# ithakis/Option-Replicating-Portfolio-with-Neural-Networks

Measured on AMD Instinct MI355X. Metric: MC paths/sec training 30-step hedge-MLP + terminal P&L std-dev, 1/2/4/8 MI355X, higher is better.
Workload: dtype fp32

## Files before the change

### csrc/hedge_mlp.hip

```cpp
#include "hedge_core.h"
#include "hedge_fit.h"
#include "hedge_lag.h"
#include "hedge_narrow.h"

#include <type_traits>

namespace rph {

template <int NIN, int H, int NO, int HEAD>
__global__ __launch_bounds__(256) void k_hedge_train_step(const TrainDesc d, const int step, const int epoch,
                                                          const Perm perm) {
  using B = NarrowBody<NIN, H, NO, HEAD>;
  constexpr int R = B::R;
  constexpr int P = B::P;
  prefetch_kernarg<sizeof(TrainDesc) + 2 * sizeof(int) + sizeof(Perm)>();
  __shared__ __attribute__((aligned(16))) float lds[B::SCRATCH_FLOATS];
  __shared__ __attribute__((aligned(16))) float wl[P + 4];
  __shared__ int s_last;

  RPH_DASSERT(d.batch > 0 && d.n_local >= d.batch && d.num_wgs == (int)gridDim.x);
  RPH_STAMP(0);
  const float stopped = d.fit->stopped;
  const float wv = threadIdx.x < P ? d.wts->w[0][threadIdx.x] : 0.f;
  UpdPre<P> up;
  if (d.fused_update) prefetch_update<P>(up, d.wts, d.opt, d.fit, d.lr_sched, epoch, step);
  const int lane = threadIdx.x & 63, wid = threadIdx.x >> 6;
  typename B::Pre pre;
  pre.valid = false;
  if (B::first(wid) < d.batch) B::load(d, step, perm, B::first(wid), lane, pre);

  if (stopped != 0.f) return;
  if (threadIdx.x < P) wl[threadIdx.x] = wv;
  if (d.fused_update) {
    asm volatile("" ::"v"(up.m[0]), "v"(up.v[0]), "v"(up.w[0]), "v"(up.wbest[0]), "s"(up.t), "s"(up.lr), "s"(up.loss_sum),
                 "s"(up.wait), "s"(up.best_loss), "s"(up.lr_sched_e));
  }
  __syncthreads();
  RPH_STAMP(1);
  float vv[1];
  B::partial(d, step, perm, wl, typename B::Frags{}, lds, pre, vv);
  float val = vv[0];
  float* red = lds;
  RPH_STAMP(3);

  if (gridDim.x > 1) {
    const int G = gridDim.x;
    if (threadIdx.x < R) {
      if (d.deterministic) st_agent(d.slab + (size_t)blockIdx.x * R + threadIdx.x, val);
      else __hip_atomic_fetch_add(d.acc + (blockIdx.x % ACC_REPLICAS) * R + threadIdx.x, val, __ATOMIC_RELAXED,
                                  __HIP_MEMORY_SCOPE_AGENT);
    }
    asm volatile("s_waitcnt vmcnt(0)" ::: "memory");
    __syncthreads();
    RPH_STAMP(4);
    if (threadIdx.x == 0) {
      const uint32_t ticket = __hip_atomic_fetch_add(d.counter, 1u, __ATOMIC_RELAXED, __HIP_MEMORY_SCOPE_AGENT);
      s_last = (ticket == (uint32_t)G - 1u) ? 1 : 0;
    }
    __syncthreads();
    RPH_STAMP(5);
    if (!s_last) return;
    if (d.deterministic) {
      constexpr int GROUPS = 256 / R;
      const int col = threadIdx.x % R;
      const int grp = threadIdx.x / R;
      float a = 0.f;
#pragma unroll 8
      for (int r = grp; r < G; r += GROUPS) a += ld_agent(d.slab + (size_t)r * R + col);
      lds[grp * R + col] = a;
      __syncthreads();
      if (threadIdx.x < R) {
        float s2 = 0.f;
        for (int gi = 0; gi < GROUPS; ++gi) s2 += lds[gi * R + threadIdx.x];
        val = s2;
      }
      __syncthreads();
    } else {
      if (threadIdx.x < R) {
        float* a = d.acc + threadIdx.x;
        float r0, r1, r2, r3, r4, r5, r6, r7;
        if (R == 128) {
          asm volatile(
              "global_load_dword %0, %8, off sc1\n\t"
              "global_load_dword %1, %8, off offset:512 sc1\n\t"
              "global_load_dword %2, %8, off offset:1024 sc1\n\t"
              "global_load_dword %3, %8, off offset:1536 sc1\n\t"
              "global_load_dword %4, %8, off offset:2048 sc1\n\t"
              "global_load_dword %5, %8, off offset:2560 sc1\n\t"
              "global_load_dword %6, %8, off offset:3072 sc1\n\t"
              "global_load_dword %7, %8, off offset:3584 sc1\n\t"
              "s_waitcnt vmcnt(0)"
              : "=&v"(r0), "=&v"(r1), "=&v"(r2), "=&v"(r3), "=&v"(r4), "=&v"(r5), "=&v"(r6), "=&v"(r7)
              : "v"(a)
              : "memory");
        } else {
          float* b = a + 4 * R;
          asm volatile(
              "global_load_dword %0, %8, off sc1\n\t"
              "global_load_dword %1, %8, off offset:1024 sc1\n\t"
              "global_load_dword %2, %8, off offset:2048 sc1\n\t"
              "global_load_dword %3, %8, off offset:3072 sc1\n\t"
              "global_load_dword %4, %9, off sc1\n\t"
              "global_load_dword %5, %9, off offset:1024 sc1\n\t"
              "global_load_dword %6, %9, off offset:2048 sc1\n\t"
              "global_load_dword %7, %9, off offset:3072 sc1\n\t"
              "s_waitcnt vmcnt(0)"
              : "=&v"(r0), "=&v"(r1), "=&v"(r2), "=&v"(r3), "=&v"(r4), "=&v"(r5), "=&v"(r6), "=&v"(r7)
              : "v"(a), "v"(b)
              : "memory");
        }
        val = ((r0 + r1) + (r2 + r3)) + ((r4 + r5) + (r6 + r7));
#pragma unroll
        for (int rp = 0; rp < ACC_REPLICAS; ++rp) st_agent(a + rp * R, 0.f);
      }
    }
    if (threadIdx.x == 0) __hip_atomic_store(d.counter, 0u, __ATOMIC_RELAXED, __HIP_MEMORY_SCOPE_AGENT);
  }
  if (threadIdx.x < R) red[threadIdx.x] = val;
  __syncthreads();
  RPH_STAMP(6);

  if (d.dp_world > 1) {
    dp_allreduce<R>(d, red);
    RPH_STAMP(7);
  }
  if (d.fused_update) {
    apply_update<P>(red, up, d.wts, d.opt, d.fit, epoch, step, d.steps_per_epoch);
  } else if (threadIdx.x < R) {
    d.grad_out[threadIdx.x] = red[threadIdx.x];
  }
  if (d.dp_world <= 1) RPH_STAMP(7);
}

template <int NIN, int H, int NO, int HEAD, bool PA, bool EX = false>
__global__ __launch_bounds__(256) void k_hedge_eval(const EvalDesc d) {
  using S = NetShape<NIN, H, NO, HEAD>;
  constexpr int NHOLD = S::NHOLD;
  static_assert(!PA || NIN >= NHOLD - 1, "price alias needs a feature per traded asset");
  prefetch_kernarg<sizeof(EvalDesc)>();
  RPH_DASSERT(d.n_local > 0 && d.num_wgs == (int)gridDim.x && d.wa != nullptr && d.stats != nullptr);
  __shared__ double sst[4][EVAL_NSTAT];
  constexpr int WBOFF = (S::P + 3) / 4 * 4;
  __shared__ __attribute__((aligned(16))) float wl[WBOFF + S::P + 4];
  const bool has_b = d.wb != nullptr;
  for (int i = threadIdx.x; i < S::P; i += 256) {
    wl[i] = d.wa->w[0][i];
    if (has_b) wl[WBOFF + i] = d.wb->w[0][i];
  }
  __syncthreads();
  if (blockIdx.x == 0) {
    for (int i = threadIdx.x; i < S::P; i += 256) {
      if (d.snap_a) d.snap_a->w[0][i] = wl[i];
      if (d.snap_b) d.snap_b->w[0][i] = has_b ? wl[WBOFF + i] : wl[i];
    }
  }
  const float* __restrict__ WA = wl;
  const float* __restrict__ WB = has_b ? wl + WBOFF : wl;
  const int lane = threadIdx.x & 63, wid = threadIdx.x >> 6;

  constexpr int NS = 64;
  float st[NS];
#pragma unroll
  for (int i = 0; i < NS; ++i) st[i] = 0.f;
  float rmin = INFINITY, rmax = -INFINITY;

  struct In {
    float x[NIN], pt[NHOLD], pt1[NHOLD], tgt, gb;
    int p;
    bool valid;
  };
  constexpr int EPF = 4;
  const int stride = (int)gridDim.x * 256;
  const bool has1 = d.price_t1[0] != nullptr;
  auto load_in = [&](int p, In& in) {
    in.p = p;
    in.valid = p < d.n_local;
    const int pp = in.valid ? p : 0;
#pragma unroll
    for (int f = 0; f < NIN; ++f) in.x[f] = d.feat[f][pp];
#pragma unroll
    for (int k = 0; k < NHOLD - 1; ++k) {
      if constexpr (PA) in.pt[k] = in.x[PA ? k : 0];
      else in.pt[k] = d.price_t[k][pp];
      in.pt1[k] = has1 ? d.price_t1[k][pp] : 0.f;
    }
    in.tgt = (has1 && d.target) ? d.target[pp] : 0.f;
    in.gb = d.g_base ? d.g_base[pp] : 0.f;
  };
  In q[EPF];
  const int p_first = blockIdx.x * 256 + threadIdx.x;
#pragma unroll
  for (int i = 0; i < EPF; ++i) load_in(p_first + i * stride, q[i]);

  for (int p0 = blockIdx.x * 256; p0 < d.n_local; p0 += stride) {
    const In cur = q[0];
#pragma unroll
    for (int i = 0; i + 1 < EPF; ++i) q[i] = q[i + 1];
    if (p0 + EPF * stride < d.n_local) load_in(cur.p + EPF * stride, q[EPF - 1]);
    const int p = cur.p;
    const bool valid = cur.valid;
    uint32_t zo = 0;
    asm volatile("" : "+v"(zo));
    const float* __restrict__ WAi = (const float*)__builtin_assume_aligned(WA + (zo & ~3u), 16);
    const float* __restrict__ WBi = (const float*)__builtin_assume_aligned(WB + (zo & ~3u), 16);
    float z1[H], a1[H], z2[H], a2[H], hold[NHOLD], holdv[NHOLD], xn[NIN];
#pragma unroll
    for (int f = 0; f < NIN; ++f) xn[f] = (cur.x[f] - d.fmu[f]) * d.fisd[f];
    net_forward<NIN, H, NO, HEAD>(WAi, xn, d.alpha, z1, a1, z2, a2, hold);
#pragma unroll
    for (int k = 0; k < NHOLD; ++k) holdv[k] = hold[k];
    if (has_b) {
      net_forward<NIN, H, NO, HEAD>(WBi, xn, d.alpha, z1, a1, z2, a2, holdv);
#pragma unroll
      for (int k = 0; k < NHOLD; ++k) hold[k] = hold[k] + d.hold_c * (holdv[k] - hold[k]);
    }
    float V = 0.f;
#pragma unroll
    for (int k = 0; k < NHOLD - 1; ++k) V = fmaf(holdv[k], cur.pt[k], V);
    V = fmaf(holdv[NHOLD - 1], d.bond_t, V);
    if (d.g_base) V = cur.gb + d.blend_c * (V - cur.gb);
    [[maybe_unused]] float cont = V, xval = 0.f;
    [[maybe_unused]] bool exer = false;
    if constexpr (EX) {
      xval = d.ex_kind == EX_PUT ? fmaxf(d.ex_strike - cur.pt[0], 0.f) : fmaxf(cur.pt[0] - d.ex_strike, 0.f);
      exer = xval > 0.f && xval >= cont;
      V = exer ? xval : cont;
    }
    float res = 0.f, pred1 = 0.f;
    const float tgt = cur.tgt;
    if (has1) {
#pragma unroll
      for (int k = 0; k < NHOLD - 1; ++k) pred1 = fmaf(hold[k], cur.pt1[k], pred1);
      pred1 = fmaf(hold[NHOLD - 1], d.bond_t1, pred1);
      if (d.target) res = tgt - pred1;
    }
    if (valid) {
      if (d.v_out) d.v_out[p] = V;
#pragma unroll
      for (int k = 0; k < NHOLD; ++k)
        if (d.hold_out[k]) d.hold_out[k][p] = hold[k];
      if (d.resid_out) d.resid_out[p] = res;
      if (d.pred1_out) d.pred1_out[p] = pred1;
      st[ES_V] += V;
      st[ES_V2] += V * V;
      st[ES_RES] += res;
      st[ES_RES2] += res * res;
      st[ES_ABSRES] += fabsf(res);
      st[ES_APE] += d.target ? fabsf(res) * __frcp_rn(fmaxf(fabsf(tgt), 1e-7f)) : 0.f;
      st[ES_PRED1] += pred1;
      st[ES_COUNT] += 1.f;
      if constexpr (EX) {
        st[ES_EXER] += exer ? 1.f : 0.f;
        st[ES_EXVAL] += exer ? xval : 0.f;
        st[ES_CONT] += cont;
      }
#pragma unroll
      for (int k = 0; k < NHOLD; ++k) {
        st[ES_HOLD + k] += hold[k];
        st[ES_HOLD2 + k] += hold[k] * hold[k];
      }
      rmin = fminf(rmin, res);
      rmax = fmaxf(rmax, res);
    }
  }
  wave_reduce_scatter<NS>(st, lane);
#pragma unroll
  for (int o = 1; o < 64; o <<= 1) {
    rmin = fminf(rmin, __shfl_xor(rmin, o, 64));
    rmax = fmaxf(rmax, __shfl_xor(rmax, o, 64));
  }
  if (lane < EVAL_NSTAT) sst[wid][lane] = (double)st[0];
  if (lane == 0) {
    sst[wid][ES_RESMIN] = rmin;
    sst[wid][ES_RESMAX] = rmax;
  }
  __syncthreads();
  if (threadIdx.x < EVAL_NSTAT) {
    const int i = threadIdx.x;
    double v;
    if (i == ES_RESMIN) v = fmin(fmin(sst[0][i], sst[1][i]), fmin(sst[2][i], sst[3][i]));
    else if (i == ES_RESMAX) v = fmax(fmax(sst[0][i], sst[1][i]), fmax(sst[2][i], sst[3][i]));
    else v = sst[0][i] + sst[1][i] + sst[2][i] + sst[3][i];
    d.stats[(size_t)blockIdx.x * EVAL_NSTAT + i] = v;
  }
}

constexpr int PNL_PPT = 4;

template <int NIN, int H, int NO, int HEAD, bool EX = false>
__global__ __launch_bounds__(256) void k_hedge_pnl(const PnlDesc d) {
  using S = NetShape<NIN, H, NO, HEAD>;
  constexpr int NHOLD = S::NHOLD;
  constexpr int NA = NHOLD - 1;
  constexpr int WBOFF = (S::P + 3) / 4 * 4;
  prefetch_kernarg<sizeof(PnlDesc)>();
  RPH_DASSERT(d.n_local > 0 && d.num_wgs == (int)gridDim.x && d.snap != nullptr && d.stats != nullptr);
  __shared__ __attribute__((aligned(16))) float wl[WBOFF + S::P + 4];
  __shared__ double sred[4][EX ? 12 : 8];
  const int tid = threadIdx.x, lane = tid & 63, wid = tid >> 6;
  const long long base = (long long)blockIdx.x * 256 * PNL_PPT + tid;
  const bool has_b = d.has_b != 0;
  float wealth[PNL_PPT], s_cur[PNL_PPT][NA > 0 ? NA : 1];
  long long pidx[PNL_PPT];
#pragma unroll
  for (int j = 0; j < PNL_PPT; ++j) {
    const long long p = base + (long long)j * 256;
    const bool ok = p < d.n_local;
    pidx[j] = ok ? p : 0;
    wealth[j] = ok ? (d.w0 ? d.w0[p] : d.wealth0) : 0.f;
#pragma unroll
    for (int a = 0; a < NA; ++a) s_cur[j][a] = d.price[a][pidx[j]];
  }
  float xr[PNL_PPT][NIN], s_nxt[PNL_PPT][NA > 0 ? NA : 1];
  auto load_date = [&](int t) {
#pragma unroll
    for (int j = 0; j < PNL_PPT; ++j) {
#pragma unroll
      for (int f = 0; f < NIN; ++f) xr[j][f] = d.feat[f][(long long)t * d.feat_ts[f] + pidx[j]];
#pragma unroll
      for (int a = 0; a < NA; ++a) s_nxt[j][a] = d.price[a][(long long)(t + 1) * d.price_ts[a] + pidx[j]];
    }
  };
  [[maybe_unused]] int tau[PNL_PPT];
  [[maybe_unused]] float pnl_ex[PNL_PPT];
  [[maybe_unused]] double paid[PNL_PPT];
  if constexpr (EX) {
#pragma unroll
    for (int j = 0; j < PNL_PPT; ++j) {
      tau[j] = d.n_dates;
      pnl_ex[j] = 0.f;
      paid[j] = 0.0;
    }
  }
  if (d.n_dates > 0) load_date(0);
  for (int t = 0; t < d.n_dates; ++t) {
    float xc[PNL_PPT][NIN], sc_nxt[PNL_PPT][NA > 0 ? NA : 1];
#pragma unroll
    for (int j = 0; j < PNL_PPT; ++j) {
#pragma unroll
      for (int f = 0; f < NIN; ++f) xc[j][f] = xr[j][f];
#pragma unroll
      for (int a = 0; a < NA; ++a) sc_nxt[j][a] = s_nxt[j][a];
    }
    if (t + 1 < d.n_dates) load_date(t + 1);
    __syncthreads();
    const NetWeights* wt = d.snap + (size_t)t * 2;
    for (int i = tid; i < S::P; i += 256) {
      wl[i] = wt[0].w[0][i];
      if (has_b) wl[WBOFF + i] = wt[1].w[0][i];
    }
    float mu[NIN], isd[NIN];
#pragma unroll
    for (int f = 0; f < NIN; ++f) {
      mu[f] = d.fmu[t * MAXIN + f];
      isd[f] = d.fisd[t * MAXIN + f];
    }
    const float grow = (float)(d.bond[t + 1] / d.bond[t]);
    [[maybe_unused]] bool ex_date = false;
    [[maybe_unused]] float bond_t = 0.f, to_end = 0.f;
    [[maybe_unused]] double disc = 0.0;
    if constexpr (EX) {
      ex_date = t % d.ex_every == 0;
      bond_t = (float)d.bond[t];
      to_end = (float)(d.bond[d.n_dates] / d.bond[t]);
      disc = d.bond[0] / d.bond[t];
    }
    __syncthreads();
#pragma unroll
    for (int j = 0; j < PNL_PPT; ++j) {
      uint32_t zo = 0;
      asm volatile("" : "+v"(zo));
      const float* __restrict__ WA = (const float*)__builtin_assume_aligned(wl + (zo & ~3u), 16);
      const float* __restrict__ WB = (const float*)__builtin_assume_aligned(wl + WBOFF + (zo & ~3u), 16);
      float x[NIN];
#pragma unroll
      for (int f = 0; f < NIN; ++f) x[f] = (xc[j][f] - mu[f]) * isd[f];
      float z1[H], a1[H], z2[H], a2[H], hold[NHOLD], hb[NHOLD];
      net_forward<NIN, H, NO, HEAD>(WA, x, d.alpha, z1, a1, z2, a2, hold);
      if (has_b) {
        net_forward<NIN, H, NO, HEAD>(WB, x, d.alpha, z1, a1, z2, a2, hb);
#pragma unroll
        for (int k = 0; k < NHOLD; ++k) hold[k] = hold[k] + d.hold_c * (hb[k] - hold[k]);
      }
      if constexpr (EX) {
        if (ex_date && tau[j] == d.n_dates) {
          float c = 0.f;
#pragma unroll
          for (int a = 0; a < NA; ++a) c = fmaf(hold[a], s_cur[j][a], c);
          c = fmaf(hold[NHOLD - 1], bond_t, c);
          const float s0 = s_cur[j][0];
          const float xv = d.ex_kind == EX_PUT ? fmaxf(d.ex_strike - s0, 0.f) : fmaxf(s0 - d.ex_strike, 0.f);
          if (xv > 0.f && xv >= c) {
            tau[j] = t;
            pnl_ex[j] = (wealth[j] - xv) * to_end;
            paid[j] = (double)xv * disc;
            wealth[j] = wealth[j] * to_end;
          }
        }
      }
      float w = wealth[j] * grow;
#pragma unroll
      for (int a = 0; a < NA; ++a) {
        w = fmaf(hold[a], sc_nxt[j][a] - s_cur[j][a] * grow, w);
        s_cur[j][a] = sc_nxt[j][a];
      }
      if constexpr (EX) wealth[j] = tau[j] == d.n_dates ? w : wealth[j];
      else wealth[j] = w;
    }
  }
  double sv = 0, sv2 = 0, sp = 0, sp2 = 0, sa = 0, cnt = 0;
  float pmin = INFINITY, pmax = -INFINITY;
  [[maybe_unused]] double sx = 0, sxv = 0, stau = 0;
#pragma unroll
  for (int j = 0; j < PNL_PPT; ++j) {
    const long long p = base + (long long)j * 256;
    if (p >= d.n_local) continue;
    float pnl = wealth[j] - d.payoff[p];
    if constexpr (EX) {
      const bool exd = tau[j] < d.n_dates;
      if (exd) pnl = pnl_ex[j];
      if (d.tau_out) d.tau_out[p] = tau[j];
      sx += exd ? 1.0 : 0.0;
      sxv += exd ? paid[j] : (double)d.payoff[p] * (d.bond[0] / d.bond[d.n_dates]);
      stau += (double)tau[j];
    }
    if (d.pnl_out) d.pnl_out[p] = pnl;
    sv += wealth[j];
    sv2 += (double)wealth[j] * wealth[j];
    sp += pnl;
    sp2 += (double)pnl * pnl;
    sa += fabsf(pnl);
    cnt += 1.0;
    pmin = fminf(pmin, pnl);
    pmax = fmaxf(pmax, pnl);
  }
#pragma unroll
  for (int o = 1; o < 64; o <<= 1) {
    sv += __shfl_xor(sv, o, 64);
    sv2 += __shfl_xor(sv2, o, 64);
    sp += __shfl_xor(sp, o, 64);
    sp2 += __shfl_xor(sp2, o, 64);
    sa += __shfl_xor(sa, o, 64);
    cnt += __shfl_xor(cnt, o, 64);
    pmin = fminf(pmin, __shfl_xor(pmin, o, 64));
    pmax = fmaxf(pmax, __shfl_xor(pmax, o, 64));
    if constexpr (EX) {
      sx += __shfl_xor(sx, o, 64);
      sxv += __shfl_xor(sxv, o, 64);
      stau += __shfl_xor(stau, o, 64);
    }
  }
  if constexpr (EX) {
    if (lane == 0) {
      sred[wid][8] = sx; sred[wid][9] = sxv; sred[wid][10] = stau;
    }
  }
  if (lane == 0) {
    sred[wid][0] = sv; sred[wid][1] = sv2; sred[wid][2] = sp; sred[wid][3] = sp2;
    sred[wid][4] = sa; sred[wid][5] = cnt; sred[wid][6] = pmin; sred[wid][7] = pmax;
  }
  __syncthreads();
  if (tid < EVAL_NSTAT) {
    double v = 0.0;
    auto sum4 = [&](int k) { return (sred[0][k] + sred[1][k]) + (sred[2][k] + sred[3][k]); };
    if (tid == ES_V) v = sum4(0);
    else if (tid == ES_V2) v = sum4(1);
    else if (tid == ES_RES) v = sum4(2);
    else if (tid == ES_RES2) v = sum4(3);
    else if (tid == ES_ABSRES) v = sum4(4);
    else if (tid == ES_COUNT) v = sum4(5);
    else if (tid == ES_RESMIN) v = fmin(fmin(sred[0][6], sred[1][6]), fmin(sred[2][6], sred[3][6]));
    else if (tid == ES_RESMAX) v = fmax(fmax(sred[0][7], sred[1][7]), fmax(sred[2][7], sred[3][7]));
    if constexpr (EX) {
      if (tid == ES_EXER) v = sum4(8);
      else if (tid == ES_EXVAL) v = sum4(9);
      else if (tid == ES_TAU) v = sum4(10);
    }
    d.stats[(size_t)blockIdx.x * EVAL_NSTAT + tid] = v;
  }
}

}

using namespace rph;

extern "C" int rph_net_nparams(int nin, int h, int nout, int head, int* p_out, int* r_out) {
  int rc = -1;
  match_shape(AllShapes{}, nin, h, nout, head, &rc, [&](auto t) {
    using S = typename decltype(t)::S;
    *p_out = S::P;
    *r_out = S::R;
    return 0;
  });
  return rc;
}

static Perm step_perm(const TrainDesc* d, int epoch) {
  const uint32_t n_chunks = (uint32_t)((d->n_local + (1 << d->chunk_log2) - 1) >> d->chunk_log2);
  return make_perm(n_chunks, d->seed, (uint32_t)epoch, d->shuffle != 0);
}

extern "C" int rph_train_step(const TrainDesc* d, int step, int epoch, void* stream) {
  if (int rc = validate_train(d, 0, "rph_train_step")) return rc;
  hipStream_t s = (hipStream_t)stream;
  const Perm perm = step_perm(d, epoch);
  int rc = 0;
  if (match_shape(NarrowShapes{}, d->nin, d->h, d->nout, d->head, &rc, [&](auto t) {
        using T = decltype(t);
        hipLaunchKernelGGL((k_hedge_train_step<T::NIN, T::H, T::NO, T::HEAD>), dim3(d->num_wgs), dim3(256), 0, s, *d,
                           step, epoch, perm);
        return (int)hipGetLastError();
      }))
    return rc;
  return launch_wide_step(d, step, epoch, perm, s);
}

extern "C" int rph_train_fit(const TrainDesc* d, int epochs, void* stream) {
  if (int rc = validate_train(d, 2, "rph_train_fit")) return rc;
  hipStream_t s = (hipStream_t)stream;
  int rc = 0;
  if (match_shape(NarrowShapes{}, d->nin, d->h, d->nout, d->head, &rc, [&](auto t) {
        using T = decltype(t);
        return launch_fit<NarrowBody<T::NIN, T::H, T::NO, T::HEAD>>(d, epochs, s);
      }))
    return rc;
  return launch_wide_fit(d, epochs, s);
}

extern "C" int rph_train_lag_step(const TrainDesc* d, int k, int epoch, void* stream) {
  if (int rc = validate_train(d, 1, "rph_train_lag_step")) return rc;
  hipStream_t s = (hipStream_t)stream;
  const Perm perm = step_perm(d, epoch);
  int rc = 0;
  if (match_shape(NarrowShapes{}, d->nin, d->h, d->nout, d->head, &rc, [&](auto t) {
        constexpr int A = decltype(t)::NIN, B = decltype(t)::H, C = decltype(t)::NO, E = decltype(t)::HEAD;
        switch (d->variant) {
          case 1: return launch_step_lag<NarrowBody<A, B, C, E, 2>>(d, k, epoch, perm, s);
          case 2: return launch_step_lag<NarrowBody<A, B, C, E, 1, 3>>(d, k, epoch, perm, s);
          case 3: return launch_step_lag<NarrowBody<A, B, C, E, 2, 3>>(d, k, epoch, perm, s);
          case 4: return launch_step_lag<NarrowBody<A, B, C, E, 1, 1, true>>(d, k, epoch, perm, s);
          case 5: return launch_step_lag<NarrowBody<A, B, C, E, 1, 1, false, true>>(d, k, epoch, perm, s);
          default: return launch_step_lag<NarrowBody<A, B, C, E>>(d, k, epoch, perm, s);
        }
      }))
    return rc;
  return launch_wide_lag_step(d, k, epoch, perm, s);
}

extern "C" int rph_train_lag_finalize(const TrainDesc* d, int K, void* stream) {
  if (int rc = validate_train(d, 1, "rph_train_lag_finalize")) return rc;
  hipStream_t s = (hipStream_t)stream;
  return with_shape(AllShapes{}, d->nin, d->h, d->nout, d->head, "rph_train_lag_finalize", [&](auto t) {
    using T = decltype(t);
    constexpr int NREP = T::H == 8 ? NARROW_NREP : WIDE_NREP;
    hipLaunchKernelGGL((k_hedge_lag_finalize<T::S::P, T::S::R, NREP>), dim3(1), dim3(256), 0, s, *d, K);
    return (int)hipGetLastError();
  });
}

extern "C" int rph_train_lag_fit(const TrainDesc* d, int epochs, void* stream) {
  if (int rc = validate_train(d, 1, "rph_train_lag_fit")) return rc;
  int k = 0;
  for (int e = 0; e < epochs; ++e)
    for (int s = 0; s < d->steps_per_epoch; ++s, ++k)
      if (int rc = rph_train_lag_step(d, k, e, stream)) return rc;
  return rph_train_lag_finalize(d, k, stream);
}

extern "C" int rph_train_ticket_fit(const TrainDesc* d, int epochs, void* stream) {
  if (int rc = validate_train(d, 0, "rph_train_ticket_fit")) return rc;
  if (!d->fused_update) return rph_report("rph_train_ticket_fit", "needs the fused (in-kernel) update");
  for (int e = 0; e < epochs; ++e)
    for (int s = 0; s < d->steps_per_epoch; ++s)
      if (int rc = rph_train_step(d, s, e, stream)) return rc;
  return 0;
}


extern "C" int rph_train_update(const TrainDesc* d, int step, int epoch, void* stream) {
  if (!d->grad_out || !d->wts || !d->opt || !d->fit) return rph_report("rph_train_update", "null pointer");
  hipStream_t s = (hipStream_t)stream;
  return with_shape(AllShapes{}, d->nin, d->h, d->nout, d->head, "rph_train_update", [&](auto t) {
    using S = typename decltype(t)::S;
    hipLaunchKernelGGL((k_hedge_update<S::P, S::R>), dim3(1), dim3(256), 0, s, *d, step, epoch);
    return (int)hipGetLastError();
  });
}

extern "C" int rph_eval(const EvalDesc* d, void* stream) {
  if (!d->wa || !d->stats || d->n_local < 1 || d->num_wgs < 1 || d->nin < 1 || d->nin > MAXIN)
    return rph_report("rph_eval", "bad eval descriptor");
  if (!(d->alpha >= 0.f && d->alpha <= 1.f)) return rph_report("rph_eval", "LeakyReLU slope must be in [0, 1]");
  for (int f = 0; f < d->nin; ++f)
    if (!(d->fisd[f] > 0.f && d->fisd[f] < 3.0e38f && d->fmu[f] == d->fmu[f]))
      return rph_report("rph_eval", "feature standardisation must be finite with fisd > 0");
  for (int f = 0; f < d->nin; ++f)
    if (!d->feat[f]) return rph_report("rph_eval", "null feature pointer");
  hipStream_t s = (hipStream_t)stream;
  const int nhold = d->head == HEAD_COMPLEMENT ? 2 : d->nout;
  bool alias = d->nin >= nhold - 1;
  for (int k = 0; alias && k < nhold - 1; ++k) alias = d->price_t[k] == d->feat[k];
  const bool ex = d->ex_kind != EX_NONE;
  if (ex) {
    if (d->ex_kind != EX_PUT && d->ex_kind != EX_CALL) return rph_report("rph_eval", "ex_kind must be 0, 1 (put) or 2 (call)");
    if (d->wb) return rph_report("rph_eval", "wb with ex_kind (early exercise takes one network)");
    if (d->g_base) return rph_report("rph_eval", "g_base with ex_kind (early exercise takes one network)");
    if (nhold < 2 || !d->price_t[0]) return rph_report("rph_eval", "price_t[0] is null with ex_kind");
    if (!(d->ex_strike == d->ex_strike) || d->ex_strike < 0.f || d->ex_strike > 3.0e38f)
      return rph_report("rph_eval", "ex_strike must be finite and >= 0");
  }
  return with_shape(AllShapes{}, d->nin, d->h, d->nout, d->head, "rph_eval", [&](auto t) {
    using T = decltype(t);
    auto launch = [&](auto pa, auto exv) {
      hipLaunchKernelGGL((k_hedge_eval<T::NIN, T::H, T::NO, T::HEAD, decltype(pa)::value, decltype(exv)::value>),
                         dim3(d->num_wgs), dim3(256), 0, s, *d);
      return (int)hipGetLastError();
    };
    if constexpr (T::NIN >= T::S::NHOLD - 1) {
      if (alias) return ex ? launch(std::true_type{}, std::true_type{}) : launch(std::true_type{}, std::false_type{});
    }
    return ex ? launch(std::false_type{}, std::true_type{}) : launch(std::false_type{}, std::false_type{});
  });
}

extern "C" int rph_pnl(const PnlDesc* d, void* stream) {
  const int nhold = d->head == HEAD_COMPLEMENT ? 2 : d->nout;
  if (!d->snap || !d->stats || !d->payoff || !d->fmu || !d->fisd || !d->bond || d->n_local < 1 || d->n_dates < 1 ||
      d->nin < 1 || d->nin > MAXIN || nhold < 2 || nhold > MAXHOLD)
    return rph_report("rph_pnl", "bad P&L descriptor");
  if (!(d->alpha >= 0.f && d->alpha <= 1.f)) return rph_report("rph_pnl", "LeakyReLU slope must be in [0, 1]");
  for (int f = 0; f < d->nin; ++f)
    if (!d->feat[f] || d->feat_ts[f] < 0) return rph_report("rph_pnl", "null feature pointer / negative stride");
  for (int k = 0; k < nhold - 1; ++k)
    if (!d->price[k] || d->price_ts[k] < d->n_local) return rph_report("rph_pnl", "null price pointer / bad stride");
  const long long per_wg = 256LL * PNL_PPT;
  if ((long long)d->num_wgs * per_wg < d->n_local || (long long)(d->num_wgs - 1) * per_wg >= d->n_local)
    return rph_report("rph_pnl", "num_wgs does not match n_local / (256 * PNL_PPT)");
  const bool ex = d->ex_kind != EX_NONE;
  if (ex) {
    if (d->ex_kind != EX_PUT && d->ex_kind != EX_CALL) return rph_report("rph_pnl", "ex_kind must be 0, 1 (put) or 2 (call)");
    if (d->has_b) return rph_report("rph_pnl", "has_b with ex_kind (early exercise takes one network)");
    if (d->ex_every < 1) return rph_report("rph_pnl", "ex_every must be >= 1 with ex_kind");
    if (!(d->ex_strike == d->ex_strike) || d->ex_strike < 0.f || d->ex_strike > 3.0e38f)
      return rph_report("rph_pnl", "ex_strike must be finite and >= 0");
  } else if (d->tau_out) {
    return rph_report("rph_pnl", "tau_out without ex_kind");
  }
  hipStream_t s = (hipStream_t)stream;
  return with_shape(AllShapes{}, d->nin, d->h, d->nout, d->head, "rph_pnl", [&](auto t) {
    using T = decltype(t);
    if (ex) hipLaunchKernelGGL((k_hedge_pnl<T::NIN, T::H, T::NO, T::HEAD, true>), dim3(d->num_wgs), dim3(256), 0, s, *d);
    else hipLaunchKernelGGL((k_hedge_pnl<T::NIN, T::H, T::NO, T::HEAD, false>), dim3(d->num_wgs), dim3(256), 0, s, *d);
    return (int)hipGetLastError();
  });
}
```

### csrc/paths.hip

```cpp
#include "rph_common.h"
#include "rph_types.h"

namespace rph {
int rph_report(const char* what, const char* msg);
}

namespace rph {

template <typename Real>
RPH_INLINE Real ndtri_u30(uint32_t x);
template <>
RPH_INLINE float ndtri_u30<float>(uint32_t x) {
  x = x == 0u ? 1u : x;
  return ndtri_u30_f32(x);
}
template <>
RPH_INLINE double ndtri_u30<double>(uint32_t x) {
  return ndtri_u30_f64(x);
}

template <typename Real, bool ALIGNED>
__global__ __launch_bounds__(256) void k_sobol_normal(Real* __restrict__ out, int n, int d,
                                                      const uint32_t* __restrict__ sv,
                                                      const uint32_t* __restrict__ shift,
                                                      long long offset, int raw) {
  const int i = blockIdx.x * 256 + threadIdx.x;
  if (ALIGNED == false && i >= n) return;
  const uint32_t g = gray_code((uint64_t)(offset + i));
  for (int j = 0; j < d; ++j) {
    const uint32_t x = sobol_point<ALIGNED>(sv + (size_t)j * 32, shift[j], g);
    Real v;
    if (raw) v = (Real)x * (Real)9.313225746154785e-10;
    else v = ndtri_u30<Real>(x);
    if (i < n) out[(size_t)i * d + j] = v;
  }
}

RPH_INLINE long long sim_gidx(const SimDesc& d, int p) {
  return d.map_blk > 0 ? d.path_offset + ((long long)p / d.map_blk) * d.map_stride + (long long)p % d.map_blk
                       : d.path_offset + p;
}

template <typename Real, bool ALIGNED, int MODEL, int STAT = 0>
__global__ __launch_bounds__(256) void k_sim_scan(const SimDesc d) {
  const int p = blockIdx.x * 256 + threadIdx.x;
  if (!ALIGNED && p >= d.n_local) return;
  const long long gp = sim_gidx(d, p);
  const uint32_t g = gray_code((uint64_t)gp);
  const Real dt = (Real)d.dt;
  const Real sdt = sqrt(dt);
  const Real mu = (Real)d.mu[0], sig = (Real)d.sigma[0];
  const float inv0 = (float)d.inv_norm[0];
  const size_t n = (size_t)d.n_local;

  if (MODEL == SIM_GBM_ARITH || MODEL == SIM_GBM_LOG) {
    Real y = (MODEL == SIM_GBM_LOG) ? log((Real)d.s0[0]) : (Real)d.s0[0];
    const Real drift = (MODEL == SIM_GBM_LOG) ? (mu - (Real)0.5 * sig * sig) * dt : mu * dt;
    const Real vol = sig * sdt;
    d.out[p] = (float)d.s0[0] * inv0;
    Real acc = (STAT == STAT_MEAN || STAT == STAT_GEOMEAN) ? (Real)0 : (Real)d.s0[0];
    Real stat = (Real)d.s0[0];
    Real sf = (Real)d.s0[0];
    if (STAT != STAT_NONE) d.out2[p] = (float)d.s0[0] * inv0;
    for (int t = 1; t < d.n_fine; ++t) {
      const Real z = ndtri_u30<Real>(sobol_point<ALIGNED>(d.sv1 + (size_t)t * 32, d.shift1[t], g));
      if (MODEL == SIM_GBM_LOG) y += drift + vol * z;
      else y = y + y * (drift + vol * z);
      if (STAT == STAT_GEOMEAN) {
        acc += y;
      } else if (STAT != STAT_NONE) {
        sf = (MODEL == SIM_GBM_LOG) ? exp(y) : y;
        if (STAT == STAT_MEAN) acc += sf;
        else if (STAT == STAT_MAX) acc = sf > acc ? sf : acc;
        else acc = sf < acc ? sf : acc;
      }
      if (t % d.reduction == 0 || (STAT != STAT_NONE && t == d.n_fine - 1)) {
        if (STAT == STAT_MEAN) stat = acc / (Real)t;
        else if (STAT == STAT_GEOMEAN) stat = exp(acc / (Real)t);
        else if (STAT != STAT_NONE) stat = acc;
      }
      if (t % d.reduction == 0) {
        const int c = t / d.reduction;
        const Real s = (STAT != STAT_NONE && STAT != STAT_GEOMEAN) ? sf : ((MODEL == SIM_GBM_LOG) ? exp(y) : y);
        if (c < d.n_coarse) {
          d.out[(size_t)c * n + p] = (float)s * inv0;
          if (STAT != STAT_NONE) d.out2[(size_t)c * n + p] = (float)stat * inv0;
        }
      }
    }
    const Real s = (STAT != STAT_NONE && STAT != STAT_GEOMEAN) ? sf : ((MODEL == SIM_GBM_LOG) ? exp(y) : y);
    if (d.final_out) d.final_out[p] = (float)s * inv0;
    if (STAT != STAT_NONE && d.final2_out) d.final2_out[p] = (float)stat * inv0;
  } else if (MODEL == SIM_SV_REF || MODEL == SIM_HESTON) {
    Real ly = log((Real)d.s0[0]);
    Real v = (Real)d.v0;
    d.out[p] = (float)d.s0[0] * inv0;
    if (d.out2) d.out2[p] = (float)v;
    const Real rho = (Real)d.rho, rhoc = sqrt((Real)1 - rho * rho);
    const Real kap = (Real)d.kappa, th = (Real)d.theta, xi = (Real)d.xi;
    const Real ekd = exp(-kap * dt);
    const Real qc1 = xi * xi * ekd * ((Real)1 - ekd) / kap;
    const Real qc2 = th * xi * xi * ((Real)1 - ekd) * ((Real)1 - ekd) / ((Real)2 * kap);
    const Real qK1 = (Real)0.5 * dt * (kap * rho / xi - (Real)0.5) - rho / xi;
    const Real qK2 = (Real)0.5 * dt * (kap * rho / xi - (Real)0.5) + rho / xi;
    const Real qK3 = (Real)0.5 * dt * ((Real)1 - rho * rho);
    const Real qA = qK2 + (Real)0.5 * qK3;
    const Real qK0u = -rho * kap * th * dt / xi;
    const bool qe = MODEL == SIM_HESTON && d.scheme == HESTON_QE;
    const Real tau = (Real)d.sv_tscale * dt;
    for (int t = 1; t < d.n_fine; ++t) {
      const Real z1 = ndtri_u30<Real>(sobol_point<ALIGNED>(d.sv1 + (size_t)t * 32, d.shift1[t], g));
      const uint32_t x2 = sobol_point<ALIGNED>(d.sv2 + (size_t)t * 32, d.shift2[t], g);
      if (MODEL == SIM_SV_REF) {
        const Real z2 = ndtri_u30<Real>(x2);
        if (d.sv_tscale > 0.0) {
          const Real vp = v > (Real)0 ? v : (Real)0;
          ly += (mu - (Real)0.5 * vp * vp) * dt + vp * sdt * z1;
          v = v + (Real)d.a * ((Real)d.b - vp) * tau + (Real)d.c * sqrt(vp * tau) * z2;
        } else {
          const Real arg = v * dt;
          const Real sq = d.parity ? sqrt(arg) : sqrt(arg > (Real)0 ? arg : (Real)0);
          v = v + (Real)d.a * ((Real)d.b - v) + (Real)d.c * sq * z2;
          ly += (mu - (Real)0.5 * v * v) * dt + v * sdt * z1;
        }
      } else if (qe) {
        const Real m = th + (v - th) * ekd;
        const Real s2 = v * qc1 + qc2;
        const Real psi = s2 / (m * m);
        Real vn, k0;
        if (psi <= (Real)1.5) {
          const Real z2 = ndtri_u30<Real>(x2);
          const Real ip = (Real)2 / psi;
          const Real b2 = ip - (Real)1 + sqrt(ip) * sqrt(ip - (Real)1);
          const Real qa = m / ((Real)1 + b2);
          const Real bz = sqrt(b2) + z2;
          vn = qa * bz * bz;
          const Real den = (Real)1 - (Real)2 * qA * qa;
          k0 = den > (Real)0 ? -qA * b2 * qa / den + (Real)0.5 * log(den) - (qK1 + (Real)0.5 * qK3) * v : qK0u;
        } else {
          const Real p = (psi - (Real)1) / (psi + (Real)1);
          const Real beta = ((Real)1 - p) / m;
          const Real u = (Real)x2 * (Real)9.313225746154785e-10;
          vn = u <= p ? (Real)0 : log(((Real)1 - p) / ((Real)1 - u)) / beta;
          k0 = beta > qA ? -log(p + beta * ((Real)1 - p) / (beta - qA)) - (qK1 + (Real)0.5 * qK3) * v : qK0u;
        }
        const Real var = qK3 * (v + vn);
        ly += mu * dt + k0 + qK1 * v + qK2 * vn + sqrt(var > (Real)0 ? var : (Real)0) * z1;
        v = vn;
      } else {
        const Real z2 = ndtri_u30<Real>(x2);
        const Real vp = v > (Real)0 ? v : (Real)0;
        const Real sv = sqrt(vp * dt);
        ly += (mu - (Real)0.5 * vp) * dt + sv * (rho * z2 + rhoc * z1);
        v = v + (Real)d.kappa * ((Real)d.theta - vp) * dt + (Real)d.xi * sv * z2;
      }
      if (t % d.reduction == 0) {
        const int c = t / d.reduction;
        if (c < d.n_coarse) {
          d.out[(size_t)c * n + p] = (float)exp(ly) * inv0;
          if (d.out2) d.out2[(size_t)c * n + p] = (float)v;
        }
      }
    }
    if (d.final_out) d.final_out[p] = (float)exp(ly) * inv0;
  } else if (MODEL == SIM_MORTALITY) {
    Real lam = (Real)d.l0;
    int N = d.n0;
    const float invn = 1.0f / (float)d.n0;
    d.out2[p] = 1.0f;
    if (d.out3) d.out3[p] = (float)lam;
    const Real lc = (Real)d.lc, eta_sdt = (Real)d.eta * sdt;
    for (int t = 1; t < d.n_fine; ++t) {
      const Real z = ndtri_u30<Real>(sobol_point<ALIGNED>(d.sv2 + (size_t)t * 32, d.shift2[t], g));
      lam = lam + (lc * lam * dt + eta_sdt * z);
      double q = 1.0 - exp(-(double)lam * (double)dt);
      q = q < 0.0 ? 0.0 : (q > 1.0 ? 1.0 : q);
      if (N > 0 && q > 0.0) {
        const u32x4 r = philox4x32_10({(uint32_t)gp, (uint32_t)(gp >> 32),
                                       (uint32_t)t, 0xB1A0u},
                                      d.seed, 0x1234u);
        const double u = u01d(r.x, r.y);
        const double mean = (double)N * q;
        int D;
        if (mean < 200.0 && q < 1.0) {
          double f = exp((double)N * log1p(-q));
          double F = f;
          const double ratio = q / (1.0 - q);
          D = 0;
          while (u > F && D < N) {
            f *= (double)(N - D) / (double)(D + 1) * ratio;
            ++D;
            F += f;
            if (f < 1e-300 && F < u) { break; }
          }
        } else {
          const double z2n = ndtri_u30<double>((uint32_t)(u * 1073741824.0) | 1u);
          double dd = mean + sqrt(mean * (1.0 - q)) * z2n + 0.5;
          dd = dd < 0.0 ? 0.0 : (dd > (double)N ? (double)N : dd);
          D = (int)dd;
        }
        N -= D;
      }
      if (d.parity) {
        if (t < d.n_coarse && d.out3) d.out3[(size_t)t * n + p] = (float)lam;
      }
      if (t % d.reduction == 0) {
        const int c = t / d.reduction;
        if (c < d.n_coarse) {
          d.out2[(size_t)c * n + p] = (float)N * invn;
          if (!d.parity && d.out3) d.out3[(size_t)c * n + p] = (float)lam;
        }
      }
    }
    if (d.final2_out) d.final2_out[p] = (float)N * invn;
  }
}

template <int NA, bool ALIGNED>
__global__ __launch_bounds__(256) void k_sim_basket(const SimDesc d) {
  const int p = blockIdx.x * 256 + threadIdx.x;
  if (!ALIGNED && p >= d.n_local) return;
  const uint32_t g = gray_code((uint64_t)sim_gidx(d, p));
  const float dt = (float)d.dt, sdt = sqrtf(dt);
  float ly[NA], drift[NA], vol[NA], inv[NA], ch[NA * (NA + 1) / 2];
  const size_t n = (size_t)d.n_local;
#pragma unroll
  for (int a = 0, i = 0; a < NA; ++a)
#pragma unroll
    for (int b = 0; b <= a; ++b, ++i) ch[i] = (float)d.chol[a * MAXIN + b];
#pragma unroll
  for (int a = 0; a < NA; ++a) {
    ly[a] = logf((float)d.s0[a]);
    drift[a] = (float)((d.mu[a] - 0.5 * d.sigma[a] * d.sigma[a]) * d.dt);
    vol[a] = (float)d.sigma[a] * sdt;
    inv[a] = (float)d.inv_norm[a];
    d.out[(size_t)a * n + p] = (float)d.s0[a] * inv[a];
  }
  for (int t = 1; t < d.n_fine; ++t) {
    float w[NA];
#pragma unroll
    for (int a = 0; a < NA; ++a) {
      const int dim = a * d.n_fine + t;
      w[a] = ndtri_u30<float>(sobol_point<ALIGNED>(d.sv1 + (size_t)dim * 32, d.shift1[dim], g));
    }
#pragma unroll
    for (int a = 0; a < NA; ++a) {
      float z = 0.f;
#pragma unroll
      for (int b = 0; b <= a; ++b) z = fmaf(ch[a * (a + 1) / 2 + b], w[b], z);
      ly[a] += drift[a] + vol[a] * z;
    }
    if (t % d.reduction == 0) {
      const int c = t / d.reduction;
      if (c < d.n_coarse) {
#pragma unroll
        for (int a = 0; a < NA; ++a) d.out[((size_t)c * NA + a) * n + p] = __expf(ly[a]) * inv[a];
      }
    }
  }
  if (d.final_out) {
#pragma unroll
    for (int a = 0; a < NA; ++a) d.final_out[(size_t)a * n + p] = __expf(ly[a]) * inv[a];
  }
}

__global__ __launch_bounds__(256) void k_payoff(int kind, int n, int na, const float* __restrict__ s,
                                                const float* __restrict__ nfrac, float strike,
                                                const float* __restrict__ wts, const float* __restrict__ x,
                                                float* __restrict__ out) {
  const int p = blockIdx.x * 256 + threadIdx.x;
  if (p >= n) return;
  float v;
  if (kind == 0) {
    const float y = s[p];
    v = (y > strike ? y : strike) * (nfrac ? nfrac[p] : 1.f);
  } else if (kind == 1) {
    v = fmaxf(s[p] - strike, 0.f);
  } else if (kind == 2) {
    v = fmaxf(strike - s[p], 0.f);
  } else if (kind == 4) {
    v = fmaxf(s[p] - x[p], 0.f);
  } else if (kind == 5) {
    v = fmaxf(x[p] - s[p], 0.f);
  } else {
    float b = 0.f;
    for (int a = 0; a < na; ++a) b = fmaf(wts[a], s[(size_t)a * n + p], b);
    v = fmaxf(b - strike, 0.f);
  }
  out[p] = v;
}

RPH_INLINE uint32_t fkey(float x) {
  const uint32_t b = __float_as_uint(x);
  return (b & 0x80000000u) ? ~b : (b | 0x80000000u);
}

__global__ __launch_bounds__(256) void k_radix_hist(const float* __restrict__ x, long long n, uint32_t pmask,
                                                    uint32_t prefix, int shift, int nbins,
                                                    unsigned int* __restrict__ hist) {
  extern __shared__ __attribute__((aligned(16))) unsigned int h[];
  for (int i = threadIdx.x; i < nbins; i += 256) h[i] = 0u;
  __syncthreads();
  for (long long i = (long long)blockIdx.x * 256 + threadIdx.x; i < n; i += (long long)gridDim.x * 256) {
    const uint32_t k = fkey(x[i]);
    if ((k & pmask) == prefix) atomicAdd(&h[(k >> shift) & (uint32_t)(nbins - 1)], 1u);
  }
  __syncthreads();
  for (int i = threadIdx.x; i < nbins; i += 256)
    if (h[i]) atomicAdd(&hist[i], h[i]);
}

}

using namespace rph;

static inline int grid_for(int n) { return (n + 255) / 256; }

extern "C" int rph_sobol_normal(void* out, int n, int d, const uint32_t* sv, const uint32_t* shift,
                                long long offset, int fp64, int raw, void* stream) {
  hipStream_t s = (hipStream_t)stream;
  const bool aligned = (n % 256 == 0) && (offset % 64 == 0);
  if (fp64) {
    if (aligned) hipLaunchKernelGGL((k_sobol_normal<double, true>), dim3(grid_for(n)), dim3(256), 0, s, (double*)out, n, d, sv, shift, offset, raw);
    else hipLaunchKernelGGL((k_sobol_normal<double, false>), dim3(grid_for(n)), dim3(256), 0, s, (double*)out, n, d, sv, shift, offset, raw);
  } else {
    if (aligned) hipLaunchKernelGGL((k_sobol_normal<float, true>), dim3(grid_for(n)), dim3(256), 0, s, (float*)out, n, d, sv, shift, offset, raw);
    else hipLaunchKernelGGL((k_sobol_normal<float, false>), dim3(grid_for(n)), dim3(256), 0, s, (float*)out, n, d, sv, shift, offset, raw);
  }
  return (int)hipGetLastError();
}

template <typename Real, bool AL, int MODEL>
static int launch_scan_stat(const SimDesc* d, hipStream_t s) {
  const dim3 grid(grid_for(d->n_local)), block(256);
  switch (d->path_stat) {
    case STAT_MEAN: hipLaunchKernelGGL((k_sim_scan<Real, AL, MODEL, STAT_MEAN>), grid, block, 0, s, *d); break;
    case STAT_GEOMEAN: hipLaunchKernelGGL((k_sim_scan<Real, AL, SIM_GBM_LOG, STAT_GEOMEAN>), grid, block, 0, s, *d); break;
    case STAT_MAX: hipLaunchKernelGGL((k_sim_scan<Real, AL, MODEL, STAT_MAX>), grid, block, 0, s, *d); break;
    case STAT_MIN: hipLaunchKernelGGL((k_sim_scan<Real, AL, MODEL, STAT_MIN>), grid, block, 0, s, *d); break;
    default: return -1;
  }
  return (int)hipGetLastError();
}

template <typename Real, bool AL>
static int launch_scan(const SimDesc* d, hipStream_t s) {
  const dim3 grid(grid_for(d->n_local)), block(256);
  if (d->path_stat != STAT_NONE)
    return d->model == SIM_GBM_LOG ? launch_scan_stat<Real, AL, SIM_GBM_LOG>(d, s)
                                   : launch_scan_stat<Real, AL, SIM_GBM_ARITH>(d, s);
  switch (d->model) {
    case SIM_GBM_ARITH: hipLaunchKernelGGL((k_sim_scan<Real, AL, SIM_GBM_ARITH>), grid, block, 0, s, *d); break;
    case SIM_GBM_LOG: hipLaunchKernelGGL((k_sim_scan<Real, AL, SIM_GBM_LOG>), grid, block, 0, s, *d); break;
    case SIM_SV_REF: hipLaunchKernelGGL((k_sim_scan<Real, AL, SIM_SV_REF>), grid, block, 0, s, *d); break;
    case SIM_HESTON: hipLaunchKernelGGL((k_sim_scan<Real, AL, SIM_HESTON>), grid, block, 0, s, *d); break;
    case SIM_MORTALITY: hipLaunchKernelGGL((k_sim_scan<Real, AL, SIM_MORTALITY>), grid, block, 0, s, *d); break;
    default: return -1;
  }
  return (int)hipGetLastError();
}

template <bool AL>
static int launch_basket(const SimDesc* d, hipStream_t s) {
  const dim3 grid(grid_for(d->n_local)), block(256);
  switch (d->na) {
    case 1: hipLaunchKernelGGL((k_sim_basket<1, AL>), grid, block, 0, s, *d); break;
    case 2: hipLaunchKernelGGL((k_sim_basket<2, AL>), grid, block, 0, s, *d); break;
    case 3: hipLaunchKernelGGL((k_sim_basket<3, AL>), grid, block, 0, s, *d); break;
    case 4: hipLaunchKernelGGL((k_sim_basket<4, AL>), grid, block, 0, s, *d); break;
    case 5: hipLaunchKernelGGL((k_sim_basket<5, AL>), grid, block, 0, s, *d); break;
    case 6: hipLaunchKernelGGL((k_sim_basket<6, AL>), grid, block, 0, s, *d); break;
    default: return -1;
  }
  return (int)hipGetLastError();
}

extern "C" int rph_simulate(const SimDesc* d, void* stream) {
  hipStream_t s = (hipStream_t)stream;
  if (d->map_blk < 0 || (d->map_blk > 0 && d->map_stride < d->map_blk)) return rph_report("rph_simulate", "bad path-index map");
  if (d->path_stat < STAT_NONE || d->path_stat > STAT_MIN) return rph_report("rph_simulate", "path_stat outside 0..4");
  if (d->path_stat != STAT_NONE) {
    if (d->model != SIM_GBM_ARITH && d->model != SIM_GBM_LOG)
      return rph_report("rph_simulate", "path statistics need a GBM model");
    if (!d->out2) return rph_report("rph_simulate", "path statistic without an out2 buffer");
    if (d->path_stat == STAT_GEOMEAN && d->model != SIM_GBM_LOG)
      return rph_report("rph_simulate", "geomean needs the log scheme (SIM_GBM_LOG)");
  }
  const bool aligned = (d->n_local % 256 == 0) && (d->path_offset % 64 == 0) &&
                       (d->map_blk == 0 || (d->map_blk % 64 == 0 && d->map_stride % 64 == 0));
  if (d->model == SIM_BASKET) return aligned ? launch_basket<true>(d, s) : launch_basket<false>(d, s);
  if (d->fp64) return aligned ? launch_scan<double, true>(d, s) : launch_scan<double, false>(d, s);
  return aligned ? launch_scan<float, true>(d, s) : launch_scan<float, false>(d, s);
}

extern "C" int rph_payoff(int kind, int n, int na, const float* s, const float* nfrac, float strike,
                          const float* wts, const float* x, float* out, void* stream) {
  if ((kind == 4 || kind == 5) && !x) return rph_report("rph_payoff", "floating-strike payoff without the x array");
  hipLaunchKernelGGL(k_payoff, dim3(grid_for(n)), dim3(256), 0, (hipStream_t)stream, kind, n, na, s, nfrac,
                     strike, wts, x, out);
  return (int)hipGetLastError();
}

extern "C" int rph_radix_hist(const float* x, long long n, uint32_t pmask, uint32_t prefix, int shift,
                              int nbins, unsigned int* hist, void* stream) {
  long long blocks = (n + 255) / 256;
  if (blocks > 2048) blocks = 2048;
  if (blocks < 1) blocks = 1;
  hipLaunchKernelGGL(k_radix_hist, dim3((unsigned)blocks), dim3(256), nbins * sizeof(unsigned int),
                     (hipStream_t)stream, x, n, pmask, prefix, shift, nbins, hist);
  return (int)hipGetLastError();
}
```

### csrc/rph_types.h

```cpp
#pragma once
#include <stdint.h>

namespace rph {

constexpr int PMAX = 2048;
constexpr int MAXIN = 8;
constexpr int MAXHOLD = 8;
constexpr int MAXHIST = 1024;
constexpr int EVAL_NSTAT = 32;
constexpr int LAG_SLOTS = 16;

enum Head : int { HEAD_FREE = 0, HEAD_COMPLEMENT = 1 };
enum Loss : int { LOSS_MSE = 0, LOSS_PINBALL = 1 };

struct NetWeights {
  float w[2][PMAX];
  float cur;
  float pad[3];
};

struct OptState {
  float m[PMAX];
  float v[PMAX];
  float t;
  float lr;
  float beta1, beta2, eps;
  float nan_steps;
  float pad0, pad1;
};

struct FitState {
  float w_best[PMAX];
  float best_loss;
  float wait;
  float stopped;
  float epoch;
  float patience;
  float max_epochs;
  float restore_best;
  float has_best;
  float loss_sum, loss_cnt, abs_sum, ape_sum;
  float last_loss, last_mae, last_mape;
  float restore_at_end;
  float hist[MAXHIST];
};

constexpr int NETW_FLOATS = (int)(sizeof(NetWeights) / 4);
constexpr int OPT_FLOATS = (int)(sizeof(OptState) / 4);
constexpr int FIT_FLOATS = (int)(sizeof(FitState) / 4);

struct TrainDesc {
  const float* feat[MAXIN];
  const float* price[MAXHOLD];
  const float* target;
  NetWeights* wts;
  OptState* opt;
  FitState* fit;
  const float* lr_sched;
  float* slab;
  uint32_t* counter;
  float* grad_out;
  float bond;
  float alpha;
  float quantile;
  float inv_batch;
  int loss;
  int n_local;
  int batch;
  int steps_per_epoch;
  int chunk_log2;
  int shuffle;
  uint32_t seed;
  int fused_update;
  int num_wgs;
  int nin, h, nout, head;
  float* acc;
  int deterministic;
  unsigned long long* stamps;
  int dp_world;
  int dp_rank;
  float* dp_mbox[8];
  uint32_t* dp_flags[8];
  uint32_t* dp_counter;
  uint32_t* dp_error;
  int mfma_fp32;
  float* lag;
  int variant;
  const FitState* fit_init;
  float fmu[MAXIN];
  float fisd[MAXIN];
};

constexpr int DP_SLOTS = 4;

struct EvalDesc {
  const float* feat[MAXIN];
  const float* price_t[MAXHOLD];
  const float* price_t1[MAXHOLD];
  const float* target;
  const NetWeights* wa;
  const NetWeights* wb;
  const float* g_base;
  float* v_out;
  float* hold_out[MAXHOLD];
  float* resid_out;
  float* pred1_out;
  double* stats;
  float bond_t, bond_t1;
  float alpha;
  float blend_c;
  float hold_c;
  int n_local;
  int num_wgs;
  int nin, h, nout, head;
  float fmu[MAXIN];
  float fisd[MAXIN];
  NetWeights* snap_a;
  NetWeights* snap_b;
  int ex_kind;
  float ex_strike;
};

struct PnlDesc {
  const float* feat[MAXIN];
  long long feat_ts[MAXIN];
  const float* price[MAXHOLD];
  long long price_ts[MAXHOLD];
  const NetWeights* snap;
  const float* fmu;
  const float* fisd;
  const double* bond;
  const float* w0;
  const float* payoff;
  float* pnl_out;
  double* stats;
  float alpha, hold_c, wealth0;
  int has_b;
  int n_local, n_dates, num_wgs;
  int nin, h, nout, head;
  int ex_kind;
  int ex_every;
  float ex_strike;
  int* tau_out;
};

constexpr int LM_NPMAX = 192;
constexpr int LM_TILE = 64;
constexpr int LM_GBLK_MAX = 21 * 1024;
constexpr int LM_OUTG = 64 * 65 / 2;
constexpr int LM_OUTG_TAIL = 1;
constexpr int LM_RED_OUTG = LM_GBLK_MAX + LM_NPMAX + 8;
constexpr int LM_RED = LM_RED_OUTG + LM_OUTG;
constexpr int LM_PASS_WGS_MAX = 512;
constexpr int LM_OG_MAX = 64;
constexpr int LM_SPEC = 4;
enum LmState : int {
  LMS_W = 0,
  LMS_RED = 2 * LM_NPMAX,
  LMS_BEST = LMS_RED + 2 * LM_RED,
  LMS_LAM,
  LMS_NACC,
  LMS_FAIL,
  LMS_LFIN,
  LMS_FAILTOT,
  LMS_SPEC_LAM = LMS_FAIL + 8,
  LMS_SPEC_PRED = LMS_SPEC_LAM + LM_SPEC,
  LMS_SPEC_OK = LMS_SPEC_PRED + LM_SPEC,
  LMS_SPEC_W = LMS_SPEC_OK + LM_SPEC,
  LMS_SLOTS = LMS_SPEC_W + LM_SPEC * LM_NPMAX,
  LMS_FLOATS = LMS_SLOTS + 16
};
constexpr int LM_SLOT = 8;
enum LmSlot : int {
  LSS_BEST = 0,
  LSS_LAM,
  LSS_NU,
  LSS_PRED,
  LSS_COPY,
  LSS_SPEC_IDX,
  LSS_LBEST,
  LSS_STOP,
};

constexpr int LM_DP_WGS = 16;
constexpr int LM_DP_FLAGS = 128;
constexpr int LM_DP_PITCH = LM_RED + LM_DP_FLAGS;
struct LmDpDesc {
  double* mbox[8];
  unsigned* counter;
  unsigned* error;
  int world, rank;
  int pitch;
  int fault;
};

struct LmDesc {
  double* state;
  float* slab_b;
  float* slab_g;
  int num_wgs;
  int gram_wgs;
  int red_wgs;
  int passes;
  int gram_blk;
  int gram_blk_stride;
  float inv_ns;
  float inv_n;
  float lam0, lam_up, lam_down, lam_min, lam_max, ridge;
  int bias_index;
  int weights_only;
  int damping;
  int stop_min;
  float stop_tol;
  int gram_skip;
  int inst;
  int explore;
  float lam_carry;
  float diag_floor;
  const float* w0;
  int renorm;
  int pad1;
  float ren_mu[MAXIN];
  float ren_isd[MAXIN];
  int out_n;
  float out_mu;
  int out_gram;
  float out_tr;
  float* slab_o;
  const float* gfeat[MAXIN];
  const float* gprice[MAXIN];
  int gram_side;
  float q_delta;
  float q_kappa;
  LmDpDesc dp;
  int dp_fused;
  int leaf_blocks;
  const float* gtarget;
  int gram_base;
  int pad4;
};

constexpr int LM_SEL_W = LM_NPMAX + 2;
constexpr int LM_SEL_MAX = 64;


enum EvalStat : int {
  ES_V = 0, ES_V2 = 1, ES_RES = 2, ES_RES2 = 3, ES_ABSRES = 4, ES_APE = 5, ES_PRED1 = 6,
  ES_COUNT = 7, ES_HOLD = 8 , ES_HOLD2 = 16 , ES_RESMIN = 24,
  ES_RESMAX = 25,
  ES_EXER = 26, ES_EXVAL = 27, ES_CONT = 28, ES_TAU = 29
};

enum ExKind : int { EX_NONE = 0, EX_PUT = 1, EX_CALL = 2 };

struct SimDesc {
  int model;
  int n_local;
  long long path_offset;
  int n_fine;
  int reduction;
  int n_coarse;
  int na;
  int fp64;
  int parity;
  const uint32_t* sv1; const uint32_t* shift1; int dims1;
  const uint32_t* sv2; const uint32_t* shift2; int dims2;
  double s0[MAXIN], mu[MAXIN], sigma[MAXIN];
  double chol[MAXIN * MAXIN];
  double dt;
  double inv_norm[MAXIN];
  double v0, a, b, c, kappa, theta, xi, rho;
  double l0, lc, eta; int n0; uint32_t seed;
  float* out;
// ... 32 lines not shown
```

### csrc/runtime.cpp

```cpp
#include <hip/hip_runtime.h>
#include <rccl/rccl.h>
#include <stddef.h>
#include <stdio.h>
#include <string.h>

#include "rph_types.h"

using namespace rph;

static thread_local char g_err[512];

static int set_err(const char* what, int code, const char* msg) {
  snprintf(g_err, sizeof(g_err), "%s failed (%d): %s", what, code, msg ? msg : "");
  return code == 0 ? -1 : code;
}

#define HIP_TRY(expr)                                                              \
  do {                                                                             \
    hipError_t _e = (expr);                                                        \
    if (_e != hipSuccess) return set_err(#expr, (int)_e, hipGetErrorString(_e));   \
  } while (0)

#define NCCL_TRY(expr)                                                             \
  do {                                                                             \
    ncclResult_t _r = (expr);                                                      \
    if (_r != ncclSuccess) return set_err(#expr, (int)_r, ncclGetErrorString(_r)); \
  } while (0)

extern "C" const char* rph_last_error() { return g_err; }

namespace rph {
int rph_report(const char* what, const char* msg) { return set_err(what, -22, msg); }
int rph_report_shape(const char* what, int nin, int h, int nout, int head) {
  char msg[128];
  snprintf(msg, sizeof(msg), "unsupported network shape (nin %d, h %d, nout %d, head %d)", nin, h, nout, head);
  return rph_report(what, msg);
}
}

#define OFF(T, f) (long long)offsetof(T, f)
extern "C" int rph_layout(long long* out, int cap) {
  long long v[] = {
      (long long)sizeof(NetWeights), (long long)sizeof(OptState), (long long)sizeof(FitState),
      OFF(NetWeights, cur), OFF(OptState, t), OFF(OptState, lr), OFF(OptState, nan_steps),
      OFF(FitState, best_loss), OFF(FitState, stopped), OFF(FitState, epoch), OFF(FitState, last_loss),
      OFF(FitState, restore_at_end), OFF(FitState, hist),
      (long long)sizeof(TrainDesc), OFF(TrainDesc, price), OFF(TrainDesc, target), OFF(TrainDesc, wts),
      OFF(TrainDesc, lr_sched), OFF(TrainDesc, slab), OFF(TrainDesc, counter), OFF(TrainDesc, grad_out),
      OFF(TrainDesc, bond), OFF(TrainDesc, inv_batch), OFF(TrainDesc, loss), OFF(TrainDesc, seed),
      OFF(TrainDesc, num_wgs), OFF(TrainDesc, head), OFF(TrainDesc, acc), OFF(TrainDesc, deterministic), OFF(TrainDesc, stamps),
      OFF(TrainDesc, dp_world), OFF(TrainDesc, dp_mbox), OFF(TrainDesc, dp_flags), OFF(TrainDesc, dp_counter), OFF(TrainDesc, dp_error),
      OFF(TrainDesc, fit_init), OFF(TrainDesc, fmu), OFF(TrainDesc, fisd),
      (long long)sizeof(EvalDesc), OFF(EvalDesc, price_t), OFF(EvalDesc, price_t1), OFF(EvalDesc, target),
      OFF(EvalDesc, wa), OFF(EvalDesc, g_base), OFF(EvalDesc, v_out), OFF(EvalDesc, hold_out),
      OFF(EvalDesc, resid_out), OFF(EvalDesc, pred1_out), OFF(EvalDesc, stats), OFF(EvalDesc, bond_t),
      OFF(EvalDesc, hold_c), OFF(EvalDesc, n_local), OFF(EvalDesc, head), OFF(EvalDesc, fmu), OFF(EvalDesc, fisd),
      OFF(EvalDesc, snap_a), OFF(EvalDesc, snap_b), OFF(EvalDesc, ex_kind), OFF(EvalDesc, ex_strike),
      (long long)sizeof(PnlDesc), OFF(PnlDesc, feat_ts), OFF(PnlDesc, price), OFF(PnlDesc, price_ts),
      OFF(PnlDesc, snap), OFF(PnlDesc, bond), OFF(PnlDesc, pnl_out), OFF(PnlDesc, stats), OFF(PnlDesc, alpha),
      OFF(PnlDesc, has_b), OFF(PnlDesc, n_dates), OFF(PnlDesc, head),
      OFF(PnlDesc, ex_kind), OFF(PnlDesc, ex_every), OFF(PnlDesc, ex_strike), OFF(PnlDesc, tau_out),
      (long long)ES_EXER, (long long)ES_EXVAL, (long long)ES_CONT, (long long)ES_TAU, (long long)EVAL_NSTAT,
      (long long)sizeof(LmDesc), OFF(LmDesc, slab_b), OFF(LmDesc, slab_g), OFF(LmDesc, num_wgs),
      OFF(LmDesc, passes), OFF(LmDesc, gram_blk), OFF(LmDesc, inv_ns), OFF(LmDesc, lam0), OFF(LmDesc, ridge), OFF(LmDesc, bias_index), OFF(LmDesc, weights_only), OFF(LmDesc, damping), OFF(LmDesc, stop_tol), OFF(LmDesc, gram_skip),
      OFF(LmDesc, inst), OFF(LmDesc, lam_carry), OFF(LmDesc, w0), OFF(LmDesc, renorm), OFF(LmDesc, ren_isd), OFF(LmDesc, out_n), OFF(LmDesc, gfeat), OFF(LmDesc, gprice), OFF(LmDesc, gram_side), OFF(LmDesc, q_delta), OFF(LmDesc, dp), OFF(LmDesc, dp_fused), OFF(LmDesc, gtarget), OFF(LmDesc, gram_base), (long long)sizeof(LmDesc), (long long)LMS_LFIN, (long long)LMS_FAILTOT, (long long)LM_SEL_W, (long long)LM_DP_PITCH,
      (long long)sizeof(LmDpDesc), OFF(LmDpDesc, counter), OFF(LmDpDesc, world), OFF(LmDpDesc, pitch),
      (long long)LM_NPMAX, (long long)LM_RED, (long long)LMS_BEST, (long long)LMS_FLOATS,
      (long long)LM_SPEC, (long long)LMS_SPEC_W, (long long)LMS_SLOTS, (long long)LM_SLOT, (long long)LSS_LBEST, (long long)LSS_STOP,
      (long long)sizeof(SimDesc), OFF(SimDesc, path_offset), OFF(SimDesc, sv1), OFF(SimDesc, dims1),
      OFF(SimDesc, sv2), OFF(SimDesc, dims2), OFF(SimDesc, s0), OFF(SimDesc, chol), OFF(SimDesc, dt),
      OFF(SimDesc, inv_norm), OFF(SimDesc, v0), OFF(SimDesc, rho), OFF(SimDesc, l0), OFF(SimDesc, n0),
      OFF(SimDesc, seed), OFF(SimDesc, out), OFF(SimDesc, final2_out), OFF(SimDesc, sv_tscale),
      OFF(SimDesc, scheme), OFF(SimDesc, path_stat), OFF(SimDesc, map_blk), OFF(SimDesc, map_stride),
      (long long)LAG_SLOTS,
  };
  const int n = (int)(sizeof(v) / sizeof(v[0]));
  for (int i = 0; i < n && i < cap; ++i) out[i] = v[i];
  return n;
}

extern "C" int rph_device_info(int dev, int* cus, int* lds_per_cu, long long* hbm_bytes, char* name, int name_cap) {
  hipDeviceProp_t p;
  HIP_TRY(hipGetDeviceProperties(&p, dev));
  *cus = p.multiProcessorCount;
  *lds_per_cu = (int)p.maxSharedMemoryPerMultiProcessor;
  *hbm_bytes = (long long)p.totalGlobalMem;
  snprintf(name, name_cap, "%s", p.gcnArchName);
  return 0;
}

extern "C" int rph_memset_async(void* ptr, int value, long long bytes, void* stream) {
  HIP_TRY(hipMemsetAsync(ptr, value, (size_t)bytes, (hipStream_t)stream));
  return 0;
}

extern "C" int rph_stream_sync(void* stream) {
  HIP_TRY(hipStreamSynchronize((hipStream_t)stream));
  return 0;
}

extern "C" int rph_graph_begin(void* stream) {
  HIP_TRY(hipStreamBeginCapture((hipStream_t)stream, hipStreamCaptureModeThreadLocal));
  return 0;
}

extern "C" int rph_graph_end(void* stream, void** exec_out, long long* num_nodes) {
  hipGraph_t g = nullptr;
  HIP_TRY(hipStreamEndCapture((hipStream_t)stream, &g));
  size_t nn = 0;
  HIP_TRY(hipGraphGetNodes(g, nullptr, &nn));
  *num_nodes = (long long)nn;
  hipGraphExec_t ex = nullptr;
  HIP_TRY(hipGraphInstantiate(&ex, g, nullptr, nullptr, 0));
  HIP_TRY(hipGraphDestroy(g));
  *exec_out = (void*)ex;
  return 0;
}

extern "C" int rph_graph_launch(void* exec, void* stream) {
  HIP_TRY(hipGraphLaunch((hipGraphExec_t)exec, (hipStream_t)stream));
  return 0;
}

extern "C" int rph_graph_destroy(void* exec) {
  HIP_TRY(hipGraphExecDestroy((hipGraphExec_t)exec));
  return 0;
}

extern "C" int rph_nccl_unique_id(char* out128) {
  ncclUniqueId id;
  NCCL_TRY(ncclGetUniqueId(&id));
  memcpy(out128, &id, sizeof(id));
  return (int)sizeof(id);
}

extern "C" int rph_nccl_init(const char* id128, int nranks, int rank, void** comm_out) {
  ncclUniqueId id;
  memcpy(&id, id128, sizeof(id));
  ncclComm_t c = nullptr;
  NCCL_TRY(ncclCommInitRank(&c, nranks, id, rank));
  *comm_out = (void*)c;
  return 0;
}

extern "C" int rph_nccl_allreduce_f32(void* comm, void* buf, long long count, void* stream) {
  NCCL_TRY(ncclAllReduce(buf, buf, (size_t)count, ncclFloat32, ncclSum, (ncclComm_t)comm, (hipStream_t)stream));
  return 0;
}

extern "C" int rph_nccl_allreduce_f64(void* comm, void* buf, long long count, void* stream) {
  NCCL_TRY(ncclAllReduce(buf, buf, (size_t)count, ncclFloat64, ncclSum, (ncclComm_t)comm, (hipStream_t)stream));
  return 0;
}

extern "C" int rph_nccl_allreduce_u32(void* comm, void* buf, long long count, void* stream) {
  NCCL_TRY(ncclAllReduce(buf, buf, (size_t)count, ncclUint32, ncclSum, (ncclComm_t)comm, (hipStream_t)stream));
  return 0;
}

extern "C" int rph_nccl_destroy(void* comm) {
  NCCL_TRY(ncclCommDestroy((ncclComm_t)comm));
  return 0;
}

static int g_ipc_finegrained = -1;

extern "C" int rph_ipc_alloc(long long bytes, void** ptr_out, char* handle_out ) {
  void* p = nullptr;
  hipIpcMemHandle_t h;
  bool done = false;
  if (g_ipc_finegrained != 0 && hipExtMallocWithFlags(&p, (size_t)bytes, hipDeviceMallocFinegrained) == hipSuccess) {
    if (hipIpcGetMemHandle(&h, p) == hipSuccess) {
      done = true;
      g_ipc_finegrained = 1;
    } else {
      (void)hipGetLastError();
      (void)hipFree(p);
      p = nullptr;
      g_ipc_finegrained = 0;
    }
  } else {
    (void)hipGetLastError();
  }
  if (!done) {
    HIP_TRY(hipMalloc(&p, (size_t)bytes));
    HIP_TRY(hipIpcGetMemHandle(&h, p));
  }
  HIP_TRY(hipMemset(p, 0, (size_t)bytes));
  HIP_TRY(hipDeviceSynchronize());
  memcpy(handle_out, &h, sizeof(h));
  *ptr_out = p;
  return 0;
}

extern "C" int rph_ipc_is_finegrained() { return g_ipc_finegrained; }

extern "C" int rph_ipc_open(const char* handle , void** ptr_out) {
  hipIpcMemHandle_t h;
  memcpy(&h, handle, sizeof(h));
  void* p = nullptr;
  HIP_TRY(hipIpcOpenMemHandle(&p, h, hipIpcMemLazyEnablePeerAccess));
  *ptr_out = p;
  return 0;
}

extern "C" int rph_ipc_close(void* p) {
  HIP_TRY(hipIpcCloseMemHandle(p));
  return 0;
}

// ... 7 lines not shown
```

### rphedge/api.py

```python
from __future__ import annotations

import math
import time
from dataclasses import dataclass, field

import numpy as np
import torch

from . import risk
from .config import RunConfig, parse_params
from .driver import BackwardInduction, InductionConfig, InductionResult, error_history, expected_value_trajectory
from .engine import Exercise, TrainConfig, gram_subsample, make_backend, set_weights
from .models import hedge_mlp as hm
from .ops import layout as L
from .ops import paths as P
from .parallel import dist as D
from .utils.logging import get_logger
from .utils.profiling import PhaseTimer


@dataclass
class RunResult:
    phi: float
    psi: float
    v0: float
    scale: float
    holdings0: np.ndarray
    induction: InductionResult
    errors: np.ndarray
    p_e_values: np.ndarray
    terminal_pnl: dict
    var: dict = field(default_factory=dict)
    summary: dict = field(default_factory=dict)
    timings: dict = field(default_factory=dict)
    config: dict = field(default_factory=dict)
    paths: object = None
    terminal_residual: dict = field(default_factory=dict)
    self_financing_pnl: dict | None = None
    exercise_share: float | None = None
    mean_exercise_date: float | None = None
    policy_value: float | None = None
    tree_price: float | None = None

    def as_tuple(self):
        return self.phi, self.psi


class HedgeRun:

    def __init__(self, cfg: RunConfig, dist_info: D.DistInfo | None = None, stream=None):
        self.cfg = cfg
        self.log = get_logger()
        if dist_info is None:
            dist_info = D.init(device=cfg.device) if D.env_world() > 1 else D.DistInfo(
                device=torch.device(cfg.device) if cfg.device else
                (torch.device("cuda", torch.cuda.current_device()) if torch.cuda.is_available() else
                 torch.device("cpu")))
        self.di = dist_info
        self.device = dist_info.device
        self.backend_kind = cfg.backend or ("hip" if self.device.type == "cuda" else "torch")
        if self.backend_kind == "hip" and self.device.type != "cuda":
            raise ValueError("hip backend needs a GPU device")
        self.stream = stream
        self.grid = P.Grid(cfg.T, cfg.dt, cfg.rebalancing)
        t_end = float(self.grid.times()[-1])
        if t_end - cfg.T > 1e-6 * max(cfg.T, 1.0):
            import warnings

            warnings.warn(f"time grid ends at {t_end:.10g}, beyond T={cfg.T:g} (dt={cfg.dt!r}, "
                          f"rebalancing={cfg.rebalancing!r}); pass dt / rebalancing at full precision", stacklevel=2)
        self.n_total = 2 ** int(cfg.n_paths)
        self.offset, self.n_local = D.shard(self.n_total, dist_info.world, dist_info.rank)
        self.timer = PhaseTimer(enabled=True, device=self.device)
        self.path_stat = None
        self.kind = self._kind()
        self.exercise = self._exercise()
        self.spec = self._spec()
        self.paths = None
        self.gpaths = None
        self.gv_terminal = None
        self.xpaths = None
        self.induction = None
        self.graph = None

    def _kind(self) -> str:
        c = self.cfg
        if c.payoff in ("call", "put"):
            return "european"
        if c.payoff in P.PATH_PAYOFFS:
            self.path_stat = P.PATH_PAYOFFS[c.payoff][0]
            bad = None
            if c.model in ("heston", "basket", "sv_ref"):
                bad = f"model {c.model!r} (path statistics run on the GBM models: gbm | gbm_log)"
            elif c.parity.complement_head:
                bad = "parity.complement_head (the psi = 1 - phi head takes one input)"
            elif c.mortality:
                bad = "mortality=True (a pension liability)"
            elif self.path_stat == "geomean" and c.model == "gbm":
                bad = "model 'gbm' (the arithmetic scheme; the geometric mean needs model='gbm_log')"
            if bad:
                raise ValueError(f"payoff {c.payoff!r} is not available with {bad}")
            return "european"
        if c.payoff == "basket_call" or c.model == "basket":
            return "basket"
        return "pension"

    def _exercise(self) -> Exercise | None:
        c = self.cfg
        mode = str(c.exercise).lower()
        if mode not in ("european", "bermudan", "american"):
            raise ValueError(f"exercise must be european | bermudan | american, got {c.exercise!r}")
        if mode == "european":
            return None
        every = int(c.exercise_every)
        if every < 1:
            raise ValueError(f"exercise_every must be >= 1, got {c.exercise_every!r}")
        if mode == "american" and every != 1:
            raise ValueError(f"exercise='american' is exercise='bermudan' with exercise_every=1, got {every}")
        what = f"exercise={mode!r}"
        if c.payoff in P.PATH_PAYOFFS:
            raise ValueError(f"{what} is not available with the path-dependent payoff {c.payoff!r} "
                             f"(the intrinsic value must depend on S_t alone: call | put)")
        if self.kind != "european" or c.mortality:
            raise ValueError(f"{what} is not available with a basket, pension or mortality liability (payoff "
                             f"{c.payoff!r}, model {c.model!r}, mortality={c.mortality}): call | put on one asset")
        if c.model not in ("gbm", "gbm_log", "heston"):
            raise ValueError(f"{what} is not available with model {c.model!r} (gbm | gbm_log | heston)")
        if c.train.q99:
            raise ValueError(f"{what} is not available with q99=True (a second network, wts_b / g_base: the exercise "
                             f"decision compares the intrinsic value with ONE network's continuation value)")
        if c.parity.complement_head or c.parity.local_residual_pnl or c.parity.raw_features:
            raise ValueError(f"{what} is not available with parity=True (the reference has no early exercise)")
        return Exercise(kind=c.option_type.lower(), strike=float(c.K) / float(c.Y), every=every)

    def _spec(self) -> hm.NetSpec:
        c = self.cfg
        alpha = c.train.leaky_alpha
        hid = int(c.train.hidden)
        if self.kind == "european":
            if self.path_stat is not None:
                return hm.NetSpec(nin=2 if c.path_feature else 1, hidden=hid, nout=2, head=L.HEAD_FREE, alpha=alpha)
            if c.model == "heston":
                return hm.NetSpec(nin=2, hidden=hid, nout=2, head=L.HEAD_FREE, alpha=alpha)
            if c.parity.complement_head:
                return hm.NetSpec(nin=1, hidden=hid, nout=1, head=L.HEAD_COMPLEMENT, alpha=alpha,
                                  layer_names=("LeakyReLU_1", "LeakyReLU_2", "Phi"))
            return hm.NetSpec(nin=1, hidden=hid, nout=2, head=L.HEAD_FREE, alpha=alpha)
        if self.kind == "basket":
            return hm.NetSpec(nin=c.n_assets, hidden=hid, nout=c.n_assets + 1, head=L.HEAD_FREE, alpha=alpha)
        if c.model in ("sv_ref", "heston") and not c.mortality:
            return hm.NetSpec(nin=2, hidden=hid, nout=2, head=L.HEAD_FREE, alpha=alpha)
        return hm.NetSpec(nin=3, hidden=hid, nout=2, head=L.HEAD_FREE, alpha=alpha)

    @property
    def scale(self) -> float:
        c = self.cfg
        return float(c.N * c.P) if self.kind == "pension" else float(c.Y)

    def simulate(self, into: P.Paths | None = None):
        c = self.cfg
        vt_out = self.v_terminal if into is not None else None
        with self.timer.phase("simulate"):
            p = self._simulate_paths(self.n_local, self.offset, None, into)
            v_t = self._payoff(p, vt_out)
            tr = c.train
            if str(tr.optimizer).lower() == "lm":
                ns, blk, stride = gram_subsample(self.n_total, tr.lm_gram_paths)
                self.gpaths = self._simulate_paths(ns, 0, (blk, stride), self.gpaths if into is not None else None)
                if self._q_lm():
                    self.gv_terminal = self._payoff(self.gpaths, self.gv_terminal if into is not None else None)
                if self.di.world > 1 and (int(tr.lm_starts) > 1 or bool(getattr(tr, "lm_explore_one", False))):
                    nx = min(1 << int(tr.lm_explore_log2), self.n_total)
                    xp = self._simulate_paths(nx, 0, None, self.xpaths[0] if into is not None else None)
                    xv = self._payoff(xp, self.xpaths[1] if into is not None else None)
                    self.xpaths = (xp, xv)
        self.paths, self.v_terminal = p, v_t
        return p, v_t

    def _q_lm(self) -> bool:
        tr, pf = self.cfg.train, self.cfg.parity
        return bool(tr.q99) and not pf.shared_q99_model and str(getattr(tr, "q99_optimizer", "adam")).lower() == "lm"

    def _payoff(self, p: P.Paths, out=None) -> torch.Tensor:
        c = self.cfg
        if self.path_stat is not None:
            return P.payoff(c.payoff, p, c.K / c.Y, stream=self.stream, out=out)
        if self.kind == "european":
            return P.payoff(c.option_type.lower(), p, c.K / c.Y, stream=self.stream, out=out)
        if self.kind == "basket":
            w = c.basket_weights or tuple([1.0 / c.n_assets] * c.n_assets)
            return P.payoff("basket_call", p, c.K / c.Y, weights=w, stream=self.stream, out=out)
        return P.payoff("guarantee", p, c.K, stream=self.stream, out=out)

    def _simulate_paths(self, n: int, offset: int, index_map, into: P.Paths | None) -> P.Paths:
        c, g, dev = self.cfg, self.grid, self.device
        fp64 = c.dtype == "fp64"
        kw = dict(device=dev, offset=offset, stream=self.stream, out=into, index_map=index_map)
        if self.kind == "european":
            if c.model == "heston":
                p = P.simulate_sv(g, n, c.Y, c.r, c.v0, model="heston", kappa=c.kappa, theta=c.theta, xi=c.xi,
                                  rho=c.rho, norm=c.Y, fp64=fp64, scheme=c.heston_scheme,
                                  joint=not c.parity.paired_sobol, **kw)
            else:
                scheme = "arith" if c.model == "gbm" else "log"
                p = P.simulate_gbm(g, n, c.Y, c.r, c.sigma, scheme=scheme, norm=c.Y, fp64=fp64,
                                   path_stat=self.path_stat, **kw)
                p.stat_feature = bool(c.path_feature)
            p.bond = g.bond(c.r, norm=c.Y if c.parity.complement_head else 1.0)
            return p
        if self.kind == "basket":
            na = c.n_assets
            corr = np.full((na, na), c.basket_corr) + np.eye(na) * (1 - c.basket_corr)
            s0 = [c.Y] * na
            p = P.simulate_basket(g, n, s0, [c.r] * na, [c.sigma] * na, corr, norm=s0, **kw)
            p.bond = g.bond(c.r)
            return p
        if c.model in ("sv_ref", "heston"):
            p = P.simulate_sv(g, n, c.Y, c.mu, c.s0, model=c.model, a=c.a, b=c.b, c=c.sv_c, kappa=c.kappa,
                              theta=c.theta, xi=c.xi, rho=c.rho, fp64=fp64, parity_nan=c.parity.sv_sqrt_nan,
                              scheme=c.heston_scheme,
                              sv_tscale=0.0 if c.parity.sv_reference_dynamics else c.sv_days_per_year,
                              joint=not c.parity.paired_sobol, **kw)
        else:
            p = P.simulate_gbm(g, n, c.Y, c.mu, c.sigma, scheme=("log" if c.model == "gbm_log" else "arith"),
                               fp64=fp64, **kw)
        if c.mortality:
            if into is not None and c.parity.numpy_binomial:
                raise NotImplementedError("numpy binomial (Q20 parity) runs on the host: not graph-safe")
            P.simulate_mortality(p, c.l0, c.c, c.ita, c.N, lambda_fine_index=c.parity.lambda_fine_index,
                                 fp64=fp64, numpy_binomial=c.parity.numpy_binomial, stream=self.stream)
        else:
            p.kind = "pension_nomort"
        p.bond = g.bond(c.r)
        if not c.parity.fine_terminal_payoff:
            if into is None:
                p.S_final = p.S[-1].clone()
            else:
                p.S_final.copy_(p.S[-1])
        if p.nfrac is not None:
            p.nfrac_final = p.nfrac[-1]
        return p

    def summary_stats(self) -> dict:
        c, p, w = self.cfg, self.paths, self.di.world
        n = float(self.n_total)
        yT = p.S_final if p.S_final.dim() == 1 else p.S_final[0]
        if self.kind == "pension":
            p_oom = D.all_reduce_scalar(float((yT < c.Y).double().sum()), device=self.device) / n if w > 1 else \
                float((yT < c.Y).double().mean())
        elif self.path_stat is not None:
            zero = self.v_terminal == 0
            p_oom = D.all_reduce_scalar(float(zero.double().sum()), device=self.device) / n if w > 1 else \
                float(zero.double().mean())
        else:
            strike = c.K / c.Y
            p_oom = D.all_reduce_scalar(float((yT < strike).double().sum()), device=self.device) / n if w > 1 else \
                float((yT < strike).double().mean())
        e_pay = float(self.v_terminal.double().sum())
        e_pay = (D.all_reduce_scalar(e_pay, device=self.device) if w > 1 else e_pay) / n
        out = {"p_oom": p_oom, "E_payoff": e_pay}
        if p.nfrac_final is not None:
            en = float(p.nfrac_final.double().sum())
            out["E_N_T"] = (D.all_reduce_scalar(en, device=self.device) if w > 1 else en) / n * c.N
        out["mean_Y_T"] = (D.all_reduce_scalar(float(yT.double().sum()), device=self.device) if w > 1
                           else float(yT.double().sum())) / n * (c.Y if self.kind != "pension" else 1.0)
        return out

    def init_align(self) -> tuple | None:
        c = self.cfg
        if str(getattr(c.train, "init", "reference")) != "aligned" or self.kind != "basket":
            return None
        return tuple(c.basket_weights or [1.0 / c.n_assets] * c.n_assets)

    def feature_centers(self) -> tuple | None:
        c = self.cfg
        if self.kind == "pension" or c.payoff not in ("call", "put", "basket_call"):
            return None
        k = float(c.K) / float(c.Y)
        nin = self.spec.nin
        return tuple([k] * nin) if self.kind == "basket" else (k,) + (None,) * (nin - 1)

    def init_weights(self, stats: dict) -> np.ndarray:
        c, spec = self.cfg, self.spec
        if self.kind == "pension":
            bias = [1.0 - stats["p_oom"], stats["p_oom"]]
        elif spec.head == L.HEAD_COMPLEMENT:
            bias = [stats["E_payoff"]]
        else:
            p_itm = 1.0 - stats["p_oom"]
            bias = [p_itm, stats["E_payoff"] - p_itm] + [0.0] * (spec.nout - 2)
            if self.kind == "basket":
                bias = [p_itm / c.n_assets] * c.n_assets + [stats["E_payoff"] - p_itm]
        return hm.init_weights(spec, bias[: spec.nout], seed=c.train.seed,
                               spread=str(getattr(c.train, "init", "reference")) in ("spread", "aligned"),
                               align=self.init_align(),
                               shared_stream=bool(c.parity.shared_initializer))

    def build(self, w0: np.ndarray | None = None):
        c = self.cfg
        if self.paths is None:
            self.simulate()
        self.stats0 = self.summary_stats()
        self.w0 = self.init_weights(self.stats0) if w0 is None else w0
        tr = c.train
        tcfg = TrainConfig(batch_size=tr.batch_size, shuffle=tr.shuffle, chunk_log2=tr.chunk_log2, seed=tr.seed,
                           lr=tr.lr, deterministic=tr.deterministic, max_wgs=tr.max_wgs,
                           mfma_fp32=str(tr.mfma_precision).lower() == "fp32", step_mode=tr.step_mode,
                           lm_gram_paths=int(tr.lm_gram_paths), lm_damping=str(tr.lm_damping),
                           lm_leaf_paths=int(getattr(tr, "lm_leaf_paths", -1)),
                           lm_lam0=float(tr.lm_lam0), lm_lam_up=float(tr.lm_lam_up),
                           lm_lam_down=float(tr.lm_lam_down), lm_out_fix=bool(tr.lm_out_fix),
                           lm_out_mu=float(tr.lm_out_mu), lm_out_tr=float(getattr(tr, "lm_out_tr", 0.0)),
                           lm_ridge=float(getattr(tr, "lm_ridge", 1e-10)),
                           lm_diag_floor=float(tr.lm_diag_floor))
        if int(tr.variant) >= 0:
            tcfg.variant = int(tr.variant)
        kw = {}
        if self.backend_kind == "hip" and self.di.world > 1:
            if self.di.probe is None and self.di.dp_mode == "xgmi":
                D.select_transport(self.di)
            self.mailbox = D.make_mailbox(self.di, self.spec.red_width)
            kw["mailbox"] = self.mailbox
            self.lm_mailbox = D.make_mailbox(self.di, L.LM_DP_PITCH, tag="rph_lmbox",
                                             mode=self.di.lm_dp_mode)
            kw["lm_mailbox"] = self.lm_mailbox
            kw["lm_comm"] = self.di.lm_comm
        self.backend = make_backend(self.backend_kind, self.spec, self.n_local, tcfg, device=self.device,
                                    comm=self.di.comm, world=self.di.world, rank=self.di.rank, stream=self.stream,
                                    **kw)
        pf = c.parity
        icfg = InductionConfig(epochs_first=tr.epochs_first, epochs_rest=tr.epochs_rest,
                               patience_first=tr.patience_first, patience_rest=tr.patience_rest,
                               early_stopping=tr.early_stopping,
                               lr_schedule_first=tr.lr_schedule_first and pf.lr_schedule_first_only,
                               lr=tr.lr, lr_rest=tr.lr_rest, lr_decay=tr.lr_decay,
                               q99=tr.q99, quantile=tr.quantile, cost_of_capital=tr.cost_of_capital,
                               shared_q99_model=pf.shared_q99_model,
                               holdings_blend_sign_rp=pf.holdings_blend_sign_rp, warm_start=pf.warm_start, carry_optimizer=pf.carry_optimizer,
                               restore_best_at_end=pf.restore_best_at_end, keep_paths=c.keep_paths,
                               poll_every=tr.poll_every, seed=tr.seed,
                               feature_norm="none" if pf.raw_features else tr.feature_norm,
                               feature_centers=self.feature_centers(),
                               feature_norm_floor=float(getattr(tr, "feature_norm_floor", 0.0)),
                               optimizer=str(tr.optimizer).lower(), lm_passes_first=int(tr.lm_passes_first),
                               q99_optimizer=str(getattr(tr, "q99_optimizer", "adam")).lower(),
                               lm_q_passes_first=int(getattr(tr, "lm_q_passes_first", 40)),
                               lm_q_passes_rest=int(getattr(tr, "lm_q_passes_rest", 4)),
                               lm_q_delta=float(getattr(tr, "lm_q_delta", 1e-4)),
                               lm_q_kappa=float(getattr(tr, "lm_q_kappa", 3.0)),
                               lm_q_start=str(getattr(tr, "lm_q_start", "mse")),
# ... 309 lines not shown
```

### rphedge/driver.py

```python
from __future__ import annotations

import math
from dataclasses import dataclass, field

import numpy as np
import torch

from .engine import (MAXIN, DateData, Exercise, FitConfig, PnlData, TrainConfig, fit_seed, fit_summary,
                     geometric_lr_schedule, keras_lr_schedule, reduce_stats)
from .models.hedge_mlp import NetSpec
from .ops import layout as L
from .ops.paths import Paths


@dataclass
class InductionConfig:
    epochs_first: int = 500
    epochs_rest: int = 100
    patience_first: int = 50
    patience_rest: int = 7
    early_stopping: bool = True
    lr_schedule_first: bool = True
    lr: float = 1e-3
    lr_rest: float = 0.0
    lr_decay: float = 1.0
    q99: bool = True
    quantile: float = 0.99
    cost_of_capital: float = 0.1
    shared_q99_model: bool = False
    holdings_blend_sign_rp: bool = False
    warm_start: bool = True
    carry_optimizer: bool = True
    restore_best_at_end: bool = False
    keep_paths: bool = True
    poll_every: int = 0
    seed: int = 1234
    feature_norm: str = "none"
    feature_centers: tuple | None = None
    feature_norm_floor: float = 0.0
    optimizer: str = "adam"
    q99_optimizer: str = "adam"
    lm_q_passes_first: int = 40
    lm_q_passes_rest: int = 4
    lm_q_delta: float = 1e-4
    lm_q_kappa: float = 3.0
    lm_q_start: str = "mse"
    lm_passes_first: int = 80
    lm_passes_rest: int = 3
    lm_stop_tol: float = 0.0
    lm_stop_min: int = 2
    lm_lam0_rest: float = 0.0
    lm_lam0_first: float = 0.0
    lm_lam_carry: float = 0.0
    lm_renorm: bool = False
    lm_starts: int = 1
    lm_explore_passes: int = 45
    lm_explore_log2: int = 16
    lm_explore_one: bool = False
    init_spread: bool = False
    init_align: tuple | None = None
    init_shared_stream: bool = False
    mean_refit: bool = False
    exercise: Exercise | None = None


@dataclass
class DateResult:
    index: int
    time: float
    fit_mse: dict | None = None
    fit_q99: dict | None = None
    stats: np.ndarray | None = None
    stats_mse: np.ndarray | None = None

    @property
    def count(self) -> float:
        return float(self.stats[L.ES_COUNT])

    def mean_holdings(self, nhold: int) -> np.ndarray:
        return self.stats[L.ES_HOLD:L.ES_HOLD + nhold] / self.count

    @property
    def mean_value(self) -> float:
        return float(self.stats[L.ES_V] / self.count)

    @property
    def residual_mean(self) -> float:
        return float(self.stats[L.ES_RES] / self.count)

    @property
    def residual_std(self) -> float:
        n = self.count
        m = self.stats[L.ES_RES] / n
        return float(math.sqrt(max(self.stats[L.ES_RES2] / n - m * m, 0.0) * n / max(n - 1, 1)))

    @property
    def exercise_share(self) -> float:
        return float(self.stats[L.ES_EXER] / self.count)

    @property
    def mean_continuation(self) -> float:
        return float(self.stats[L.ES_CONT] / self.count)

    @property
    def mean_exercise_value(self) -> float:
        n = self.stats[L.ES_EXER]
        return float(self.stats[L.ES_EXVAL] / n) if n > 0 else 0.0

    @property
    def policy_value(self) -> float:
        return float(self.stats[L.ES_EXVAL] / self.count)

    @property
    def errors(self) -> tuple[float, float]:
        s = self.stats_mse if self.stats_mse is not None else self.stats
        n = s[L.ES_COUNT]
        return float(s[L.ES_ABSRES] / n), float(100.0 * s[L.ES_APE] / n)


@dataclass
class InductionResult:
    dates: list = field(default_factory=list)
    values: torch.Tensor | None = None
    holdings: torch.Tensor | None = None
    residuals: torch.Tensor | None = None
    weights_snapshots: torch.Tensor | None = None
    v0: float = float("nan")
    holdings0: np.ndarray | None = None
    terminal: DateResult | None = None
    pnl: DateResult | None = None
    pnl_paths: torch.Tensor | None = None
    tau: torch.Tensor | None = None


class BackwardInduction:

    def __init__(self, paths: Paths, v_terminal: torch.Tensor, spec: NetSpec, w0: np.ndarray, backend,
                 icfg: InductionConfig, world: int = 1, rank: int = 0, backend_q=None, gram_paths: Paths | None = None,
                 explore_paths: tuple | None = None, gram_terminal: torch.Tensor | None = None):
        self.paths, self.spec, self.backend, self.cfg = paths, spec, backend, icfg
        self.gram_paths = gram_paths
        self.explore_paths = explore_paths
        self.backend_q = backend_q if (backend_q is not None and icfg.q99 and not icfg.shared_q99_model) else None
        self._side = None
        self.world, self.rank = world, rank
        n, nc = paths.n_local, paths.n_coarse
        dev = paths.S.device
        self.n_dates = nc - 1
        self.values = torch.empty(nc, n, dtype=torch.float32, device=dev)
        self.values[nc - 1].copy_(v_terminal)
        self.v_terminal = v_terminal
        self.gbuf = torch.empty(n, dtype=torch.float32, device=dev)
        keep = icfg.keep_paths
        self.holdings = torch.empty(nc - 1, spec.nhold, n, dtype=torch.float32, device=dev) if keep else None
        self.residuals = torch.empty(nc - 1, n, dtype=torch.float32, device=dev) if keep else None
        self.w_mse = backend.new_weights(w0)
        self.opt_mse = backend.new_opt()
        if icfg.q99:
            self.w_q = self.w_mse if icfg.shared_q99_model else backend.new_weights(w0)
            self.opt_q = backend.new_opt()
        self.w_init = backend.new_weights(w0)
        self.lm_w0s = None
        if icfg.optimizer == "lm" and (icfg.lm_starts > 1 or icfg.lm_explore_one):
            from .models import hedge_mlp as hm
            o = spec.offsets
            b3 = np.asarray(w0, np.float32)[o["b3"]:o["P"]]
            rows = [np.asarray(w0, np.float32)] + [hm.init_weights(spec, b3, seed=icfg.seed + 1000 * c,
                                                                   spread=icfg.init_spread, align=icfg.init_align,
                                                                   shared_stream=icfg.init_shared_stream)
                                                   for c in range(1, icfg.lm_starts)]
            self.lm_w0s = np.stack(rows)
        self.opt_init = backend.new_opt()
        self.fits = [[backend.new_fit(), backend.new_fit()] for _ in range(self.n_dates)]
        self.stats = [[backend.new_stats(), backend.new_stats()] for _ in range(self.n_dates)]
        self.snap = torch.zeros(self.n_dates, 2, L.NETW_FLOATS, dtype=torch.float32, device=dev)
        if icfg.lr_schedule_first:
            self.lr_first = tuple(keras_lr_schedule(icfg.epochs_first))
        else:
            self.lr_first = geometric_lr_schedule(icfg.lr, icfg.epochs_first, icfg.lr_decay) \
                if icfg.lr_decay != 1.0 else None
        self.lr_rest = geometric_lr_schedule(icfg.lr_rest or icfg.lr, icfg.epochs_rest, icfg.lr_decay) \
            if (icfg.lr_rest > 0 or icfg.lr_decay != 1.0) else None
        self.norms = feature_norms(paths, icfg.feature_norm, world, centers=icfg.feature_centers,
                                   floor=icfg.feature_norm_floor)
        self.gvalues = None
        q_lm_side = (icfg.q99 and not icfg.shared_q99_model and str(icfg.q99_optimizer).lower() == "lm"
                     and gram_paths is not None and gram_terminal is not None)
        if q_lm_side:
            ns = gram_terminal.numel()
            self.gvalues = torch.full((nc, ns), float("nan"), dtype=torch.float32, device=dev)
            self.gvalues[nc - 1].copy_(gram_terminal)
            self.g_terminal = gram_terminal
            self.ggbuf = torch.empty(ns, dtype=torch.float32, device=dev)
            self.gstats = [backend.new_stats(), backend.new_stats()]
        self.q_lm = icfg.q99 and not icfg.shared_q99_model and str(icfg.q99_optimizer).lower() == "lm"
        self.q_delta = 0.0
        if self.q_lm:
            vs = torch.stack([v_terminal.double().abs().sum(),
                              torch.tensor(float(v_terminal.numel()), dtype=torch.float64, device=dev)])
            if world > 1:
                from .parallel import dist as D

                D.all_reduce_(vs)
            vs = vs.cpu().numpy()
            self.q_delta = float(icfg.lm_q_delta) * float(vs[0] / max(vs[1], 1.0))
        nd, nin = self.n_dates, spec.nin
        fmu = np.zeros((nd, MAXIN), np.float32)
        fisd = np.ones((nd, MAXIN), np.float32)
        for t, (mu, isd) in enumerate(self.norms):
            fmu[t, :nin], fisd[t, :nin] = mu, isd
        self.pnl_data = PnlData(n_dates=nd, features=paths.features, prices=paths.prices,
                                bond=torch.tensor(np.asarray(paths.bond, np.float64), device=dev),
                                fmu=torch.from_numpy(fmu).to(dev), fisd=torch.from_numpy(fisd).to(dev),
                                w0=self.values[0], payoff=self.values[nc - 1])
        self.pnl_stats = backend.new_pnl_stats()
        self.pnl_paths = torch.empty(n, dtype=torch.float32, device=dev) if keep else None
        self.pnl_done = False
        ex = icfg.exercise
        if ex is not None and icfg.q99:
            raise ValueError("early exercise takes one network per date: q99=True (wts_b / g_base) is not available")
        self.tau = torch.full((n,), self.n_dates, dtype=torch.int32, device=dev) if ex is not None else None

    def exercise_at(self, t: int) -> Exercise | None:
        ex = self.cfg.exercise
        return ex if (ex is not None and t % int(ex.every) == 0) else None

    @property
    def hold_c(self) -> float:
        c = self.cfg
        return -c.cost_of_capital if c.holdings_blend_sign_rp else c.cost_of_capital

    def _fcfg(self, first: bool, loss: int, t: int | None = None) -> FitConfig:
        c = self.cfg
        if loss == L.LOSS_PINBALL and self.q_lm:
            return FitConfig(epochs=c.lm_q_passes_first if first else c.lm_q_passes_rest, loss=loss,
                             quantile=c.quantile, optimizer="lm", early_stopping=False,
                             lm_lam0=(c.lm_lam0_first if (first and c.lm_lam0_first > 0) else None),
                             lm_lam_carry=0.0 if first else c.lm_lam_carry, lm_q_delta=self.q_delta,
                             lm_q_kappa=c.lm_q_kappa)
        if c.optimizer == "lm" and loss == L.LOSS_MSE:
            ms = first and (c.lm_starts > 1 or c.lm_explore_one)
            ren = (self.norms[t + 1] if (c.lm_renorm and not first and c.warm_start and t is not None and self.norms
                                         and t + 1 < len(self.norms)) else None)
            return FitConfig(epochs=c.lm_passes_first if first else c.lm_passes_rest, loss=loss,
                             optimizer="lm", early_stopping=False, lm_stop_tol=0.0 if first else c.lm_stop_tol,
                             lm_stop_min=c.lm_stop_min,
                             lm_lam0=((c.lm_lam0_first if c.lm_lam0_first > 0 else None) if first else
                                      (c.lm_lam0_rest if c.lm_lam0_rest > 0 else None)),
                             lm_lam_carry=0.0 if first else c.lm_lam_carry,
                             lm_starts=c.lm_starts if ms else 1,
                             lm_explore_passes=c.lm_explore_passes if ms else 0,
                             lm_explore_paths=(1 << int(c.lm_explore_log2)) if ms else 0,
                             lm_w0s=self.lm_w0s if ms else None, lm_renorm=ren,
                             lm_explore_data=self.explore_data(t) if (ms and t is not None) else None)
        return FitConfig(epochs=c.epochs_first if first else c.epochs_rest,
                         patience=c.patience_first if first else c.patience_rest,
                         loss=loss, quantile=c.quantile, lr_schedule=self.lr_first if first else self.lr_rest,
                         restore_best=True, restore_at_end=c.restore_best_at_end, early_stopping=c.early_stopping)

    def explore_data(self, t: int) -> DateData | None:
        if self.explore_paths is None:
            return None
        if t != self.paths.n_coarse - 2:
            raise ValueError(f"explore_data(t={t}): the exploration prefix holds the terminal payoff, the target of "
                             f"the first fitted date t = {self.paths.n_coarse - 2} only")
        xp, xv = self.explore_paths
        mu, isd = self.norms[t] if self.norms else ((), ())
        return DateData(feats=xp.features(t), prices_next=xp.prices(t + 1), bond_next=float(xp.bond[t + 1]),
                        target=xv, prices_now=xp.prices(t), bond_now=float(xp.bond[t]), fmu=mu, fisd=isd)

    def date_data(self, t: int) -> DateData:
        p = self.paths
        mu, isd = self.norms[t] if self.norms else ((), ())
        gp = self.gram_paths
        return DateData(feats=p.features(t), prices_next=p.prices(t + 1), bond_next=float(p.bond[t + 1]),
                        target=self.values[t + 1], prices_now=p.prices(t), bond_now=float(p.bond[t]),
                        fmu=mu, fisd=isd, gram_feats=gp.features(t) if gp is not None else None,
                        gram_prices_next=gp.prices(t + 1) if gp is not None else None,
                        gram_target=self.gvalues[t + 1] if self.gvalues is not None else None)

    def gram_date_data(self, t: int) -> DateData:
        gp = self.gram_paths
        mu, isd = self.norms[t] if self.norms else ((), ())
        return DateData(feats=gp.features(t), prices_next=gp.prices(t + 1), bond_next=float(gp.bond[t + 1]),
                        target=self.gvalues[t + 1], prices_now=gp.prices(t), bond_now=float(gp.bond[t]),
                        fmu=mu, fisd=isd)

    def eval_gram_values(self, t: int, with_target: bool = True):
        c, be = self.cfg, self.backend
        gd = self.gram_date_data(t)
        if not with_target:
            gd.target = None
        ns = self.ggbuf.numel()
        be.eval(self.w_mse, gd, self.gstats[0], v_out=self.ggbuf, n_local=ns)
        be.eval(self.w_mse, gd, self.gstats[1], wts_b=self.w_q, g_base=self.ggbuf,
                blend_c=c.cost_of_capital, hold_c=self.hold_c, v_out=self.gvalues[t], n_local=ns)

    def restore_gram_values(self, date: int):
        if self.gvalues is None:
            return
        if date >= self.paths.n_coarse - 1:
            self.gvalues[date].copy_(self.g_terminal)
        else:
            self.eval_gram_values(date, with_target=False)

    def enqueue(self, start: int | None = None):
        c, be = self.cfg, self.backend
        nc = self.paths.n_coarse
        start = nc - 2 if start is None else int(start)
        self.ran = list(range(start, -1, -1))
        for t in self.ran:
            first = t == nc - 2
            data = self.date_data(t)
            if not c.carry_optimizer and c.warm_start and not first:
                self.opt_mse.copy_(self.opt_init)
                if c.q99:
                    self.opt_q.copy_(self.opt_init)
            if not c.warm_start and not first:
                self.w_mse.copy_(self.w_init)
                self.opt_mse.copy_(self.opt_init)
                if c.q99:
                    if not c.shared_q99_model:
                        self.w_q.copy_(self.w_init)
                    self.opt_q.copy_(self.opt_init)
            f_m, f_q = self.fits[t]
            s_m, s_q = self.stats[t]
            join = None
            q_from_mse = self.q_lm and str(c.lm_q_start).lower() == "mse"
            if self.backend_q is not None and not q_from_mse:
                main = torch.cuda.current_stream(self.values.device)
                if self._side is None:
                    self._side = torch.cuda.Stream(self.values.device)
                fork = torch.cuda.Event()
                fork.record(main)
                self._side.wait_event(fork)
                with torch.cuda.stream(self._side):
                    self.backend_q.fit(self.w_q, self.opt_q, f_q, data, self._fcfg(first, L.LOSS_PINBALL),
                                       seed=fit_seed(c.seed, t, 1), poll_every=0)
                    join = torch.cuda.Event()
                    join.record(self._side)
            be.fit(self.w_mse, self.opt_mse, f_m, data, self._fcfg(first, L.LOSS_MSE, t),
                   seed=fit_seed(c.seed, t, 0), poll_every=c.poll_every)
            if c.mean_refit and c.optimizer != "lm":
                be.bias_refit(self.w_mse, self.opt_mse, f_m, data, self._fcfg(first, L.LOSS_MSE))
            hold_out = [self.holdings[t, k] for k in range(self.spec.nhold)] if self.holdings is not None else None
            resid_out = self.residuals[t] if self.residuals is not None else None
            if c.q99:
                be.eval(self.w_mse, data, s_m, v_out=self.gbuf)
                if join is not None:
                    torch.cuda.current_stream(self.values.device).wait_event(join)
                else:
                    if q_from_mse:
                        self.w_q.copy_(self.w_mse)
                    be.fit(self.w_q, self.opt_q, f_q, data, self._fcfg(first, L.LOSS_PINBALL),
                           seed=fit_seed(c.seed, t, 1), poll_every=c.poll_every)
                be.eval(self.w_mse, data, s_q, wts_b=self.w_q, g_base=self.gbuf, blend_c=c.cost_of_capital,
                        hold_c=self.hold_c, v_out=self.values[t], hold_out=hold_out, resid_out=resid_out,
                        snap_a=self.snap[t, 0], snap_b=self.snap[t, 1])
                if self.gvalues is not None:
                    self.eval_gram_values(t)
            else:
                be.eval(self.w_mse, data, s_q, v_out=self.values[t], hold_out=hold_out, resid_out=resid_out,
                        snap_a=self.snap[t, 0], exercise=self.exercise_at(t))
        self.pnl_done = start == nc - 2
        if self.pnl_done:
            be.pnl(self.snap, self.pnl_data, self.pnl_stats, has_b=c.q99, hold_c=self.hold_c,
                   pnl_out=self.pnl_paths, exercise=c.exercise, tau_out=self.tau)

    def collect(self) -> InductionResult:
        c = self.cfg
        nc = self.paths.n_coarse
        dtc = self.paths.grid.dt_coarse
        res = InductionResult(values=self.values, holdings=self.holdings, residuals=self.residuals,
                              weights_snapshots=self.snap)
        for t in getattr(self, "ran", range(nc - 2, -1, -1)):
            f_m, f_q = self.fits[t]
            s_m, s_q = self.stats[t]
            d = DateResult(index=t, time=t * dtc, fit_mse=fit_summary(f_m),
                           fit_q99=fit_summary(f_q) if c.q99 else None,
                           stats=reduce_stats(s_q, self.world),
                           stats_mse=reduce_stats(s_m, self.world) if c.q99 else None)
            res.dates.append(d)
        d0 = res.dates[-1]
        res.terminal = res.dates[0]
        res.v0 = d0.mean_value
        res.holdings0 = d0.mean_holdings(self.spec.nhold)
        if self.pnl_done:
            res.pnl = DateResult(index=-1, time=float(self.paths.grid.times()[-1]),
                                 stats=reduce_stats(self.pnl_stats, self.world))
            res.pnl_paths = self.pnl_paths
            res.tau = self.tau
        return res


def price_features(paths: Paths) -> list:
    nin = len(paths.features(0))
    return list(range(nin)) if paths.kind not in ("pension", "heston", "sv", "gbm_stat") else [0]


def feature_norms(paths: Paths, mode: str, world: int = 1, centers=None, floor: float = 0.0) -> list:
    mode = (mode or "none").lower()
    if mode == "none":
        return []
    if mode not in ("global", "date", "horizon"):
        raise ValueError(f"feature_norm must be none | global | date | horizon, got {mode!r}")
    nd = paths.n_coarse - 1
    nin = len(paths.features(0))
    s1, s2 = [], []
    for t in range(nd):
        for x in paths.features(t):
            s1.append(x.sum(dtype=torch.float64))
            s2.append((x * x).sum(dtype=torch.float64))
    cnt = float(paths.features(0)[0].numel())
    mom = torch.stack([torch.stack(s1).view(nd, nin), torch.stack(s2).double().view(nd, nin),
                       torch.full((nd, nin), cnt, dtype=torch.float64, device=paths.S.device)], dim=-1)
    if world > 1:
        from .parallel import dist as D

        D.all_reduce_(mom)
    m = mom.cpu().numpy()
    if mode == "global":
        m = np.broadcast_to(m.sum(axis=0, keepdims=True), m.shape)
    out = []
    for t in range(nd):
        cnt = np.maximum(m[t, :, 2], 1.0)
        mu = m[t, :, 0] / cnt
        var = np.maximum(m[t, :, 1] / cnt - mu * mu, 0.0)
        sd = np.sqrt(var)
        ok = sd > 1e-6 * (np.abs(mu) + 1.0)
        isd = np.where(ok, 1.0 / np.where(ok, sd, 1.0), 1.0)
        out.append([mu, isd, sd])
    if mode == "horizon":
        _horizon_norms(paths, out, world, centers, floor)
    return [(tuple(float(v) for v in mu), tuple(float(v) for v in isd)) for mu, isd, _ in out]


def _horizon_norms(paths: Paths, out: list, world: int, centers, floor: float):
    nd = paths.n_coarse - 1
    pf = price_features(paths)
    nin = len(paths.features(0))
    last = paths.features(nd)
    lT = [torch.log(last[i].double()) for i in pf]
    s = []
    q = float(2 ** 32)
    for t in range(nd):
        ft = paths.features(t)
        for k, i in enumerate(pf):
            r = lT[k] - torch.log(ft[i].double())
            s.append(torch.round(r * q).to(torch.int64).sum())
            s.append(torch.round(r * r * q).to(torch.int64).sum())
    mom = torch.stack(s).view(nd, len(pf), 2)
    if world > 1:
        from .parallel import dist as D

        D.all_reduce_(mom)
    m = mom.cpu().numpy().astype(np.float64) / q
    cnt = float(paths.features(0)[0].numel()) * world
    for t in range(nd):
        mu, isd, sd = out[t]
        mu, isd = np.array(mu, dtype=np.float64), np.array(isd, dtype=np.float64)
        for k, i in enumerate(pf):
            rm = m[t, k, 0] / cnt
            rsd = math.sqrt(max(m[t, k, 1] / cnt - rm * rm, 0.0))
            scale = max(abs(mu[i]) * rsd, float(floor) * float(sd[i]))
            if scale > 1e-12 * (abs(mu[i]) + 1.0):
                c = centers[i] if (centers is not None and i < len(centers) and centers[i] is not None) else mu[i]
                mu[i], isd[i] = float(c), 1.0 / scale
        out[t] = [mu, isd, sd]
    assert len(out) == nd and all(len(o[0]) == nin for o in out)


def expected_value_trajectory(result: InductionResult, e_payoff: float, mu: float, r: float, dt: float) -> np.ndarray:
    rows = [[e_payoff, e_payoff, e_payoff]]
    for its, d in enumerate(result.dates, start=1):
        rows.append([d.mean_value, e_payoff * math.exp(-mu * dt * its), e_payoff * math.exp(-r * dt * its)])
    return np.asarray(rows)


def error_history(result: InductionResult) -> np.ndarray:
    rows = [[0.0, 0.0]] + [list(d.errors) for d in result.dates]
    return np.asarray(rows)
```

### rphedge/engine/__init__.py

```python
from ..models.hedge_mlp import NetSpec
from ..ops.native import MAXIN
from .config import (DateData, Exercise, FitConfig, PnlData, TrainConfig, fit_seed, geometric_lr_schedule,
                     keras_lr_schedule)
from .lm_geometry import (GRAM_BLOCKS, _lm_bias_index, _lm_out_n, gram_subsample, lm_gram_geometry,
                          lm_og_wgs, lm_out_gram, lm_out_nu, lm_pass_schedule, lm_pass_wgs, lm_tpack_image, lm_tpack_len)
from .state import (_normalise, current_weights, fit_summary, fit_template, make_opt, make_weights,
                    reduce_stats, set_weights)
from .torch_ref import TorchBackend


def __getattr__(name):
    if name in ("HipBackend", "PERSISTENT_MAX_WGS", "PNL_PPT"):
        from . import hip
        return getattr(hip, name)
    raise AttributeError(f"module {__name__!r} has no attribute {name!r}")


def make_backend(kind: str, spec: NetSpec, n_local: int, tcfg: TrainConfig, **kw):
    if kind == "hip":
        from .hip import HipBackend
        return HipBackend(spec, n_local, tcfg, **kw)
    for k in ("stream", "mailbox", "lm_mailbox", "lm_comm"):
        kw.pop(k, None)
    return TorchBackend(spec, n_local, tcfg, **kw)
```

### rphedge/engine/config.py

```python
from __future__ import annotations

from dataclasses import dataclass, field

import torch

from ..ops import layout as L


def keras_lr_schedule(epochs: int) -> list:
    return [1e-2 if e < 100 else 1e-3 if e < 200 else 5e-4 if e < 400 else float("nan") for e in range(epochs)]


def geometric_lr_schedule(lr0: float, epochs: int, decay: float = 1.0) -> tuple:
    n = max(int(epochs), 1)
    if n == 1 or decay == 1.0:
        return tuple([float(lr0)] * n)
    return tuple(float(lr0) * decay ** (e / (n - 1)) for e in range(n))


@dataclass
class FitConfig:
    epochs: int = 100
    patience: int = 7
    loss: int = L.LOSS_MSE
    quantile: float = 0.99
    lr_schedule: tuple | None = None
    restore_best: bool = True
    restore_at_end: bool = False
    early_stopping: bool = True
    optimizer: str = "adam"
    lm_stop_tol: float = 0.0
    lm_stop_min: int = 2
    lm_lam0: float | None = None
    lm_lam_carry: float = 0.0
    lm_renorm: tuple | None = None
    lm_starts: int = 1
    lm_explore_passes: int = 0
    lm_explore_paths: int = 0
    lm_w0s: object = None
    lm_explore_data: object = None
    lm_q_delta: float = 0.0
    lm_q_kappa: float = 3.0

    def key(self):
        return (self.epochs, self.patience if self.early_stopping else 1 << 30, self.restore_best,
                self.restore_at_end, tuple(self.lr_schedule) if self.lr_schedule is not None else None)


@dataclass
class TrainConfig:
    batch_size: int = 512
    shuffle: bool = True
    chunk_log2: int = 0
    seed: int = 1234
    lr: float = 1e-3
    beta1: float = 0.9
    beta2: float = 0.999
    eps: float = 1e-7
    max_wgs: int = 0
    paths_per_thread: int = 1
    deterministic: bool = False
    split_update: bool = False
    mfma_fp32: bool = False
    lm_gram_paths: int = 4096
    lm_lam0: float = 1e-3
    lm_lam_up: float = 4.0
    lm_lam_down: float = 1.0 / 3.0
    lm_lam_min: float = 1e-9
    lm_lam_max: float = 1e10
    lm_ridge: float = 1e-10
    lm_diag_floor: float = 0.0
    lm_damping: str = "simple"
    lm_bias_fix: bool = True
    lm_gram_skip: int = 3
    lm_leaf_paths: int = -1
    lm_gram_overlap: bool | None = None
    lm_out_fix: bool = False
    lm_out_mu: float = 1e-5
    lm_out_tr: float = 0.0
    lm_split: bool = False
    expose_packet: bool = False
    step_mode: str = "auto"
    variant: int = -1


@dataclass
class DateData:

    feats: list
    prices_next: list
    bond_next: float
    target: torch.Tensor
    prices_now: list = field(default_factory=list)
    bond_now: float = 1.0
    fmu: tuple = ()
    fisd: tuple = ()
    gram_feats: list | None = None
    gram_prices_next: list | None = None
    gram_target: torch.Tensor | None = None


@dataclass
class PnlData:

    n_dates: int
    features: object
    prices: object
    bond: torch.Tensor
    fmu: torch.Tensor
    fisd: torch.Tensor
    w0: torch.Tensor
    payoff: torch.Tensor


@dataclass(frozen=True)
class Exercise:

    kind: str
    strike: float
    every: int = 1

    def __post_init__(self):
        if self.kind not in ("put", "call"):
            raise ValueError(f"exercise kind must be 'put' or 'call', got {self.kind!r}")
        if int(self.every) < 1:
            raise ValueError(f"exercise_every must be >= 1, got {self.every!r}")

    def intrinsic(self, s: torch.Tensor) -> torch.Tensor:
        k = torch.tensor(float(self.strike), dtype=s.dtype, device=s.device)
        return torch.clamp(k - s, min=0) if self.kind == "put" else torch.clamp(s - k, min=0)


def fit_seed(seed: int, date: int, net: int) -> int:
    return (int(seed) * 1000003 + int(date) * 7919 + int(net) * 104729) & 0xFFFFFFFF
```

### rphedge/engine/hip.py

```python
from __future__ import annotations

import os
from dataclasses import replace

import numpy as np
import torch

from ..models.hedge_mlp import NetSpec
from ..ops import layout as L
from .config import DateData, Exercise, FitConfig, PnlData, TrainConfig
from .lm_geometry import (_lm_bias_index, _lm_out_n, gram_subsample, lm_explore_nsub, lm_gram_geometry, lm_og_wgs,
                          lm_out_nu, lm_pass_schedule, lm_shard_gram_wgs, lm_tpack_len)
from .state import StateBlocks, _Cache, _check_eval_data, _set_norm, _steps, fit_template

PNL_PPT = 4
PERSISTENT_MAX_WGS = 64


def _env(name: str, default) -> int:
    return int(os.environ.get("RPH_" + name, default))


_clone = lambda desc: type(desc).from_buffer_copy(desc)

# ... 334 lines not shown
                raise RuntimeError("multi-start start points changed inside a graph capture")
            w0 = torch.zeros(K, L.LM_NPMAX, dtype=torch.float32)
            w0[:, :P] = torch.from_numpy(rows)
            if self.device.type == "cuda" and self.stream is not None:
                with torch.cuda.stream(self.stream):
                    x["w0"].copy_(w0)
            else:
                x["w0"].copy_(w0)
            x["w0_rows"] = rows.tobytes()
        n, main_state = self.native, self._lm_buffers()["state"]
        n.lm_fit(d, lm, x["red"], self.stream)
        n.lm_select(d, lm, x["sel"], main_state, 1, 0, P, 0, self.stream)
        n.lm_select(d, lm, x["sel"], main_state, 1, 0, P, 1, self.stream)
        self.lm_explore_last = x

    def _lm_allreduce(self, red: torch.Tensor, gram: bool = True, og: bool = False):
        P, _, nblk = self._lm_shape
        if self.lm_mailbox is not None:
            x = self._cache.get(("lm_dp",), self.lm_mailbox.lm_desc)
            if gram:
                self.native.lm_dp_exchange(x, red, nblk * 1024 + lm_tpack_len(P, nblk), P, self.stream)
            else:
                self.native.lm_dp_exchange(x, red, 0, self._lm_greg(og), self.stream)
            return
        if gram:
            self._lm_comm().allreduce_(red, self.stream)
        else:
            self._lm_comm().allreduce_(red[L.LM_GBLK_MAX:L.LM_GBLK_MAX + self._lm_greg(og)], self.stream)

    def bias_refit(self, wts, opt, fit, data: DateData, fcfg: FitConfig):
        bi = _lm_bias_index(self.spec, self.tcfg)
        if bi < 0:
            return
        if not self.lm_supported():
            c = self._cache.get(("refit",), self._refit_buffers)
            st, red = c["stats"], c["red"]
            G, S = L.LM_GBLK_MAX, L.LM_GBLK_MAX + L.LM_NPMAX
            self.eval(wts, data, st)
            torch.sum(st[:, L.ES_RES], dim=0, out=red[G])
            torch.sum(st[:, L.ES_COUNT], dim=0, out=red[S])
            if self.world > 1:
                if self.lm_mailbox is not None:
                    x = self._cache.get(("lm_dp",), self.lm_mailbox.lm_desc)
                    self.native.lm_dp_exchange(x, red, 0, L.LM_RED_OUTG - L.LM_GBLK_MAX, self.stream)
                else:
                    self._lm_comm().allreduce_(red[G:S + 1], self.stream)
            torch.clamp_min(red[S:S + 1], 1.0, out=c["cnt"])
            torch.div(red[G:G + 1], c["cnt"], out=c["delta"])
            c["delta"].mul_(1.0 / float(data.bond_next))
            wts[bi:bi + 1].add_(c["delta"])
            fit[L.F_WBEST + bi:L.F_WBEST + bi + 1].copy_(wts[bi:bi + 1])
            return
        d, lm = self._lm_refit_prepare(wts, opt, fit, data, fcfg)
        self._lm_launch(d, lm, self._lm_buffers()["red"], self.world <= 1, True)

    def _lm_refit_prepare(self, wts, opt, fit, data: DateData, fcfg: FitConfig):
        def make():
            lm = _clone(self._lm_buffers()["base"])
            lm.weights_only, lm.gram_wgs, lm.out_n, lm.out_gram = 1, 1, 0, 0
            lm.gram_blk, lm.gram_blk_stride = lm_gram_geometry(self.n_local, L.LM_TILE, self.world)
            lm.inv_ns = 1.0 / float(L.LM_TILE * max(self.world, 1))
            return lm
        return self._full_batch_desc(wts, opt, fit, data, fcfg, L.LOSS_MSE), self._cache.get(("lm_refit",), make)

    def _refit_buffers(self) -> dict:
        dev = self.device
        return {"stats": self.new_stats(), "red": torch.zeros(L.LM_RED, dtype=torch.float64, device=dev),
                "cnt": torch.zeros(1, dtype=torch.float64, device=dev),
                "delta": torch.zeros(1, dtype=torch.float64, device=dev)}

    def _lm_comm(self):
        if self._lm_nccl is not None:
            return self._lm_nccl
        if self.comm is not None:
            return self.comm
        raise RuntimeError("LM reduced-block exchange without an xGMI mailbox or an RCCL communicator: build "
                           "data-parallel backends through rphedge.parallel.dist.select_transport (or pass lm_comm)")

    def lm_state(self) -> dict:
        st = self._lm_buffers()["state"].cpu().numpy()
        return {"accepted": int(st[L.LMS_NACC]), "chol_failures": int(st[L.LMS_FAIL]), "lam": float(st[L.LMS_LAM]),
                "chol_failures_total": int(st[L.LMS_FAILTOT])}

    def step_mode(self, poll_every: int = 0) -> str:
        t = self.tcfg
        atomic = not t.deterministic and not t.split_update
        dp_fused = self.mailbox is not None and self.comm is None
        if (t.step_mode == "persistent" and atomic and not poll_every and (self.world == 1 or dp_fused)
                and self.persistent_supported()):
            return "persistent"
        shared = dp_fused and getattr(self.mailbox, "shared_device", False)
        if t.step_mode == "lag" and atomic and (self.world == 1 or dp_fused):
            return "lag"
        if (t.step_mode == "auto" and atomic and self.world == 1 and not poll_every
                and self.spec.hidden == 8 and self.num_wgs <= PERSISTENT_MAX_WGS):
            return "persistent"
        if t.step_mode == "persistent" and atomic and (self.world == 1 or dp_fused):
            return "lag"
        if t.step_mode == "auto" and atomic and (self.world == 1 or (dp_fused and not shared)):
            return "lag"
        return "ticket"

    def concurrent_with(self, other: "HipBackend") -> bool:
        a, b = self.step_mode(), other.step_mode()
        cus = 256
        try:
            cus = int(torch.cuda.get_device_properties(self.device).multi_processor_count)
        except Exception:
            pass
        need = (self.num_wgs if a == "persistent" else 0) + (other.num_wgs if b == "persistent" else 0)
        if ("persistent" in (a, b)) and need > cus:
            return False
        return self.world == 1 and other.world == 1

    def persistent_supported(self) -> bool:
        return self.spec.hidden == 8 or self.spec.nin <= 3

    def check(self):
        if int(self.fit_ctl[1].item()) != 0:
            raise RuntimeError("persistent fit kernel: workgroups not co-resident (wait timed out); "
                               "use TrainConfig.step_mode='lag' or 'ticket'")

    def pnl_wgs(self) -> int:
        return (self.n_local + 256 * PNL_PPT - 1) // (256 * PNL_PPT)

    def pnl(self, snap, data: PnlData, stats, has_b: bool = False, hold_c: float = 0.0, pnl_out=None,
            exercise: Exercise | None = None, tau_out=None):
        n = self.native
        d = n.PnlDesc()
        f0, p0, p1 = data.features(0), data.prices(0), data.prices(1)
        f1 = data.features(1) if data.n_dates >= 1 else f0
        n.fill_ptrs(d.feat, f0)
        n.fill_ptrs(d.price, p0)
        for i, (a, b) in enumerate(zip(f0, f1)):
            d.feat_ts[i] = (b.data_ptr() - a.data_ptr()) // 4
        for k, (a, b) in enumerate(zip(p0, p1)):
            d.price_ts[k] = (b.data_ptr() - a.data_ptr()) // 4
        d.snap = snap.data_ptr()
        d.fmu, d.fisd, d.bond = data.fmu.data_ptr(), data.fisd.data_ptr(), data.bond.data_ptr()
        d.w0, d.payoff = data.w0.data_ptr(), data.payoff.data_ptr()
        d.pnl_out = n.ptr(pnl_out)
        d.stats = stats.data_ptr()
        d.alpha, d.hold_c, d.wealth0, d.has_b = float(self.spec.alpha), float(hold_c), 0.0, 1 if has_b else 0
        d.n_local, d.n_dates, d.num_wgs = self.n_local, int(data.n_dates), self.pnl_wgs()
        d.nin, d.h, d.nout, d.head = self.shape
        if exercise is not None:
            d.ex_kind, d.ex_every, d.ex_strike = L.EX_KINDS[exercise.kind], int(exercise.every), float(exercise.strike)
        if tau_out is not None:
            assert tau_out.dtype == torch.int32 and tau_out.numel() == self.n_local
            d.tau_out = tau_out.data_ptr()
        assert stats.shape[0] == d.num_wgs and snap.shape[0] >= data.n_dates
        n.pnl(d, self.stream)

    def eval(self, wts, data: DateData, stats, wts_b=None, g_base=None, blend_c=0.0, hold_c=0.0,
             v_out=None, hold_out=None, resid_out=None, pred1_out=None, snap_a=None, snap_b=None,
             n_local: int | None = None, exercise: Exercise | None = None):
        _check_eval_data(self.spec, data)
        n = self.native
        d = n.EvalDesc()
        d.snap_a, d.snap_b = n.ptr(snap_a), n.ptr(snap_b)
        n.fill_ptrs(d.feat, data.feats)
        n.fill_ptrs(d.price_t, data.prices_now)
        n.fill_ptrs(d.price_t1, data.prices_next)
        d.target = n.ptr(data.target)
        d.wa, d.wb, d.g_base, d.v_out = wts.data_ptr(), n.ptr(wts_b), n.ptr(g_base), n.ptr(v_out)
        if hold_out is not None:
            n.fill_ptrs(d.hold_out, hold_out)
        d.resid_out, d.pred1_out = n.ptr(resid_out), n.ptr(pred1_out)
        d.stats = stats.data_ptr()
        d.bond_t, d.bond_t1 = float(data.bond_now), float(data.bond_next)
        d.alpha = float(self.spec.alpha)
        d.blend_c, d.hold_c = float(blend_c), float(hold_c)
        d.n_local = self.n_local if n_local is None else int(n_local)
        if d.n_local != int(data.feats[0].numel()):
            raise ValueError(f"eval over {data.feats[0].numel()} paths with n_local {d.n_local}")
        d.num_wgs = self.eval_wgs
        d.nin, d.h, d.nout, d.head = self.shape
        _set_norm(d, data)
        if exercise is not None:
            d.ex_kind, d.ex_strike = L.EX_KINDS[exercise.kind], float(exercise.strike)
        n.eval_(d, self.stream)
```

### rphedge/ops/native.py

```python
from __future__ import annotations

import ctypes as C
import os
from pathlib import Path

import torch

from . import layout as L

_LIB_ENV = os.environ.get("RPH_NATIVE_LIB", "")
_LIB_PATH = Path(_LIB_ENV).resolve() if _LIB_ENV.endswith(".so") else Path(__file__).resolve().parent.parent / "_lib" / (
    {"debug": "librphedge_debug.so", "asan": "librphedge_asan.so"}.get(_LIB_ENV, "librphedge.so"))
_lib = None
_load_error: str | None = None

MAXIN, MAXHOLD = 8, 8
VP = C.c_void_p


class TrainDesc(C.Structure):
    _fields_ = [
        ("feat", VP * MAXIN), ("price", VP * MAXHOLD), ("target", VP),
        ("wts", VP), ("opt", VP), ("fit", VP), ("lr_sched", VP),
        ("slab", VP), ("counter", VP), ("grad_out", VP),
        ("bond", C.c_float), ("alpha", C.c_float), ("quantile", C.c_float), ("inv_batch", C.c_float),
        ("loss", C.c_int), ("n_local", C.c_int), ("batch", C.c_int), ("steps_per_epoch", C.c_int),
        ("chunk_log2", C.c_int), ("shuffle", C.c_int), ("seed", C.c_uint32), ("fused_update", C.c_int),
        ("num_wgs", C.c_int), ("nin", C.c_int), ("h", C.c_int), ("nout", C.c_int), ("head", C.c_int),
        ("acc", VP), ("deterministic", C.c_int), ("stamps", VP),
        ("dp_world", C.c_int), ("dp_rank", C.c_int), ("dp_mbox", VP * 8), ("dp_flags", VP * 8),
        ("dp_counter", VP), ("dp_error", VP), ("mfma_fp32", C.c_int), ("lag", VP), ("variant", C.c_int),
        ("fit_init", VP), ("fmu", C.c_float * MAXIN), ("fisd", C.c_float * MAXIN),
    ]

    def __init__(self, *a, **kw):
        super().__init__(*a, **kw)
        for f in range(MAXIN):
            self.fisd[f] = 1.0


class EvalDesc(C.Structure):
    _fields_ = [
        ("feat", VP * MAXIN), ("price_t", VP * MAXHOLD), ("price_t1", VP * MAXHOLD), ("target", VP),
        ("wa", VP), ("wb", VP), ("g_base", VP), ("v_out", VP), ("hold_out", VP * MAXHOLD),
        ("resid_out", VP), ("pred1_out", VP), ("stats", VP),
        ("bond_t", C.c_float), ("bond_t1", C.c_float), ("alpha", C.c_float), ("blend_c", C.c_float),
        ("hold_c", C.c_float),
        ("n_local", C.c_int), ("num_wgs", C.c_int), ("nin", C.c_int), ("h", C.c_int), ("nout", C.c_int),
        ("head", C.c_int), ("fmu", C.c_float * MAXIN), ("fisd", C.c_float * MAXIN),
        ("snap_a", VP), ("snap_b", VP), ("ex_kind", C.c_int), ("ex_strike", C.c_float),
    ]

    def __init__(self, *a, **kw):
        super().__init__(*a, **kw)
        for f in range(MAXIN):
            self.fisd[f] = 1.0


class PnlDesc(C.Structure):
    _fields_ = [
        ("feat", VP * MAXIN), ("feat_ts", C.c_longlong * MAXIN), ("price", VP * MAXHOLD),
        ("price_ts", C.c_longlong * MAXHOLD), ("snap", VP), ("fmu", VP), ("fisd", VP), ("bond", VP),
        ("w0", VP), ("payoff", VP), ("pnl_out", VP), ("stats", VP),
        ("alpha", C.c_float), ("hold_c", C.c_float), ("wealth0", C.c_float), ("has_b", C.c_int),
        ("n_local", C.c_int), ("n_dates", C.c_int), ("num_wgs", C.c_int),
        ("nin", C.c_int), ("h", C.c_int), ("nout", C.c_int), ("head", C.c_int),
        ("ex_kind", C.c_int), ("ex_every", C.c_int), ("ex_strike", C.c_float), ("tau_out", VP),
    ]


class LmDpDesc(C.Structure):
    _fields_ = [
        ("mbox", VP * 8), ("counter", VP), ("error", VP),
        ("world", C.c_int), ("rank", C.c_int), ("pitch", C.c_int), ("fault", C.c_int),
    ]


class LmDesc(C.Structure):
    _fields_ = [
        ("state", VP), ("slab_b", VP), ("slab_g", VP),
        ("num_wgs", C.c_int), ("gram_wgs", C.c_int), ("red_wgs", C.c_int), ("passes", C.c_int),
        ("gram_blk", C.c_int), ("gram_blk_stride", C.c_int), ("inv_ns", C.c_float), ("inv_n", C.c_float),
        ("lam0", C.c_float), ("lam_up", C.c_float), ("lam_down", C.c_float), ("lam_min", C.c_float),
        ("lam_max", C.c_float), ("ridge", C.c_float), ("bias_index", C.c_int), ("weights_only", C.c_int),
        ("damping", C.c_int), ("stop_min", C.c_int), ("stop_tol", C.c_float), ("gram_skip", C.c_int),
        ("inst", C.c_int), ("explore", C.c_int), ("lam_carry", C.c_float), ("diag_floor", C.c_float), ("w0", VP),
        ("renorm", C.c_int), ("pad1", C.c_int), ("ren_mu", C.c_float * MAXIN), ("ren_isd", C.c_float * MAXIN),
        ("out_n", C.c_int), ("out_mu", C.c_float), ("out_gram", C.c_int), ("out_tr", C.c_float),
        ("slab_o", VP),
        ("gfeat", VP * MAXIN), ("gprice", VP * MAXIN), ("gram_side", C.c_int), ("q_delta", C.c_float), ("q_kappa", C.c_float),
        ("dp", LmDpDesc), ("dp_fused", C.c_int), ("leaf_blocks", C.c_int), ("gtarget", VP),
        ("gram_base", C.c_int), ("pad4", C.c_int),
    ]

    def __init__(self, *a, **kw):
        super().__init__(*a, **kw)
        self.inst = 1


class SimDesc(C.Structure):
    _fields_ = [
        ("model", C.c_int), ("n_local", C.c_int), ("path_offset", C.c_longlong),
        ("n_fine", C.c_int), ("reduction", C.c_int), ("n_coarse", C.c_int), ("na", C.c_int),
        ("fp64", C.c_int), ("parity", C.c_int),
        ("sv1", VP), ("shift1", VP), ("dims1", C.c_int),
        ("sv2", VP), ("shift2", VP), ("dims2", C.c_int),
        ("s0", C.c_double * MAXIN), ("mu", C.c_double * MAXIN), ("sigma", C.c_double * MAXIN),
        ("chol", C.c_double * (MAXIN * MAXIN)), ("dt", C.c_double), ("inv_norm", C.c_double * MAXIN),
        ("v0", C.c_double), ("a", C.c_double), ("b", C.c_double), ("c", C.c_double),
        ("kappa", C.c_double), ("theta", C.c_double), ("xi", C.c_double), ("rho", C.c_double),
        ("l0", C.c_double), ("lc", C.c_double), ("eta", C.c_double), ("n0", C.c_int), ("seed", C.c_uint32),
        ("out", VP), ("out2", VP), ("out3", VP), ("final_out", VP), ("final2_out", VP),
        ("sv_tscale", C.c_double), ("scheme", C.c_int), ("path_stat", C.c_int),
        ("map_blk", C.c_longlong), ("map_stride", C.c_longlong),
    ]


def _expected_layout() -> list[int]:
    f = 4
    T, E, S = TrainDesc, EvalDesc, SimDesc
    return [
        L.NETW_FLOATS * f, L.OPT_FLOATS * f, L.FIT_FLOATS * f,
        L.W_CUR * f, L.O_T * f, L.O_LR * f, L.O_NAN * f,
        L.F_BEST * f, L.F_STOPPED * f, L.F_EPOCH * f, L.F_LAST_LOSS * f, L.F_RESTORE_END * f, L.F_HIST * f,
        C.sizeof(T), T.price.offset, T.target.offset, T.wts.offset, T.lr_sched.offset, T.slab.offset,
        T.counter.offset, T.grad_out.offset, T.bond.offset, T.inv_batch.offset, T.loss.offset, T.seed.offset,
        T.num_wgs.offset, T.head.offset, T.acc.offset, T.deterministic.offset, T.stamps.offset,
        T.dp_world.offset, T.dp_mbox.offset, T.dp_flags.offset, T.dp_counter.offset, T.dp_error.offset,
        T.fit_init.offset, T.fmu.offset, T.fisd.offset,
        C.sizeof(E), E.price_t.offset, E.price_t1.offset, E.target.offset, E.wa.offset, E.g_base.offset,
        E.v_out.offset, E.hold_out.offset, E.resid_out.offset, E.pred1_out.offset, E.stats.offset,
        E.bond_t.offset, E.hold_c.offset, E.n_local.offset, E.head.offset, E.fmu.offset, E.fisd.offset,
        E.snap_a.offset, E.snap_b.offset, E.ex_kind.offset, E.ex_strike.offset,
        C.sizeof(PnlDesc), PnlDesc.feat_ts.offset, PnlDesc.price.offset, PnlDesc.price_ts.offset,
        PnlDesc.snap.offset, PnlDesc.bond.offset, PnlDesc.pnl_out.offset, PnlDesc.stats.offset,
        PnlDesc.alpha.offset, PnlDesc.has_b.offset, PnlDesc.n_dates.offset, PnlDesc.head.offset,
        PnlDesc.ex_kind.offset, PnlDesc.ex_every.offset, PnlDesc.ex_strike.offset, PnlDesc.tau_out.offset,
        L.ES_EXER, L.ES_EXVAL, L.ES_CONT, L.ES_TAU, L.EVAL_NSTAT,
        C.sizeof(LmDesc), LmDesc.slab_b.offset, LmDesc.slab_g.offset, LmDesc.num_wgs.offset,
        LmDesc.passes.offset, LmDesc.gram_blk.offset, LmDesc.inv_ns.offset, LmDesc.lam0.offset,
        LmDesc.ridge.offset, LmDesc.bias_index.offset, LmDesc.weights_only.offset, LmDesc.damping.offset, LmDesc.stop_tol.offset, LmDesc.gram_skip.offset,
        LmDesc.inst.offset, LmDesc.lam_carry.offset, LmDesc.w0.offset, LmDesc.renorm.offset,
        LmDesc.ren_isd.offset, LmDesc.out_n.offset, LmDesc.gfeat.offset, LmDesc.gprice.offset,
        LmDesc.gram_side.offset, LmDesc.q_delta.offset, LmDesc.dp.offset, LmDesc.dp_fused.offset, LmDesc.gtarget.offset, LmDesc.gram_base.offset, C.sizeof(LmDesc),
        L.LMS_LFIN, L.LMS_FAILTOT, L.LM_SEL_W, L.LM_DP_PITCH,
        C.sizeof(LmDpDesc), LmDpDesc.counter.offset, LmDpDesc.world.offset, LmDpDesc.pitch.offset,
        L.LM_NPMAX, L.LM_RED, L.LMS_BEST, L.LMS_FLOATS,
        L.LM_SPEC, L.LMS_SPEC_W, L.LMS_SLOTS, L.LM_SLOT, L.LSS_LBEST, L.LSS_STOP,
        C.sizeof(S), S.path_offset.offset, S.sv1.offset, S.dims1.offset, S.sv2.offset, S.dims2.offset,
        S.s0.offset, S.chol.offset, S.dt.offset, S.inv_norm.offset, S.v0.offset, S.rho.offset, S.l0.offset,
        S.n0.offset, S.seed.offset, S.out.offset, S.final2_out.offset, S.sv_tscale.offset, S.scheme.offset, S.path_stat.offset,
        S.map_blk.offset, S.map_stride.offset,
        L.LAG_SLOTS,
    ]


def _bind(lib):
    sig = {
        "rph_last_error": (C.c_char_p, []),
        "rph_layout": (C.c_int, [C.POINTER(C.c_longlong), C.c_int]),
        "rph_device_info": (C.c_int, [C.c_int, C.POINTER(C.c_int), C.POINTER(C.c_int), C.POINTER(C.c_longlong),
                                      C.c_char_p, C.c_int]),
        "rph_memset_async": (C.c_int, [VP, C.c_int, C.c_longlong, VP]),
        "rph_stream_sync": (C.c_int, [VP]),
        "rph_graph_begin": (C.c_int, [VP]),
        "rph_graph_end": (C.c_int, [VP, C.POINTER(VP), C.POINTER(C.c_longlong)]),
        "rph_graph_launch": (C.c_int, [VP, VP]),
        "rph_graph_destroy": (C.c_int, [VP]),
        "rph_nccl_unique_id": (C.c_int, [C.c_char_p]),
        "rph_nccl_init": (C.c_int, [C.c_char_p, C.c_int, C.c_int, C.POINTER(VP)]),
        "rph_nccl_allreduce_f32": (C.c_int, [VP, VP, C.c_longlong, VP]),
        "rph_nccl_allreduce_f64": (C.c_int, [VP, VP, C.c_longlong, VP]),
        "rph_nccl_allreduce_u32": (C.c_int, [VP, VP, C.c_longlong, VP]),
        "rph_nccl_destroy": (C.c_int, [VP]),
        "rph_net_nparams": (C.c_int, [C.c_int] * 4 + [C.POINTER(C.c_int), C.POINTER(C.c_int)]),
        "rph_train_step": (C.c_int, [C.POINTER(TrainDesc), C.c_int, C.c_int, VP]),
        "rph_train_update": (C.c_int, [C.POINTER(TrainDesc), C.c_int, C.c_int, VP]),
        "rph_train_fit": (C.c_int, [C.POINTER(TrainDesc), C.c_int, VP]),
        "rph_train_lag_step": (C.c_int, [C.POINTER(TrainDesc), C.c_int, C.c_int, VP]),
        "rph_train_lag_finalize": (C.c_int, [C.POINTER(TrainDesc), C.c_int, VP]),
        "rph_train_lag_fit": (C.c_int, [C.POINTER(TrainDesc), C.c_int, VP]),
        "rph_train_ticket_fit": (C.c_int, [C.POINTER(TrainDesc), C.c_int, VP]),
        "rph_eval": (C.c_int, [C.POINTER(EvalDesc), VP]),
        "rph_pnl": (C.c_int, [C.POINTER(PnlDesc), VP]),
        "rph_lm_shape": (C.c_int, [C.c_int] * 4 + [C.POINTER(C.c_int)] * 3),
        "rph_lm_pass_wps": (C.c_int, [C.c_int] * 4),
        "rph_lm_eval": (C.c_int, [C.POINTER(TrainDesc), C.POINTER(LmDesc), VP, C.c_int, VP]),
        "rph_lm_solve": (C.c_int, [C.POINTER(TrainDesc), C.POINTER(LmDesc), VP, C.c_int, VP]),
        "rph_lm_fit": (C.c_int, [C.POINTER(TrainDesc), C.POINTER(LmDesc), VP, VP]),
        "rph_lm_dp_exchange": (C.c_int, [C.POINTER(LmDpDesc), VP, C.c_int, C.c_int, VP]),
        "rph_lm_select": (C.c_int, [C.POINTER(TrainDesc), C.POINTER(LmDesc), VP, VP, C.c_int, C.c_int, C.c_int,
                                    C.c_int, VP]),
        "rph_sobol_normal": (C.c_int, [VP, C.c_int, C.c_int, VP, VP, C.c_longlong, C.c_int, C.c_int, VP]),
        "rph_simulate": (C.c_int, [C.POINTER(SimDesc), VP]),
        "rph_payoff": (C.c_int, [C.c_int, C.c_int, C.c_int, VP, VP, C.c_float, VP, VP, VP, VP]),
        "rph_radix_hist": (C.c_int, [VP, C.c_longlong, C.c_uint32, C.c_uint32, C.c_int, C.c_int, VP, VP]),
        "rph_ipc_alloc": (C.c_int, [C.c_longlong, C.POINTER(VP), C.c_char_p]),
        "rph_ipc_open": (C.c_int, [C.c_char_p, C.POINTER(VP)]),
        "rph_ipc_close": (C.c_int, [VP]),
        "rph_free": (C.c_int, [VP]),
        "rph_ipc_handle_size": (C.c_int, []),
        "rph_ipc_is_finegrained": (C.c_int, []),
    }
    for name, (res, args) in sig.items():
        fn = getattr(lib, name)
        fn.restype = res
        fn.argtypes = args


def load(required: bool | None = None):
    global _lib, _load_error
    if _lib is not None:
        return _lib
    if required is None:
        required = torch.cuda.is_available()
    try:
        if _LIB_ENV.endswith(".so") and not _LIB_PATH.exists():
            raise FileNotFoundError(f"RPH_NATIVE_LIB={_LIB_ENV} does not exist (it is never built implicitly)")
        if not _LIB_PATH.exists() or os.environ.get("RPH_REBUILD"):
            from .. import build as _build

            v = os.environ.get("RPH_NATIVE_LIB", "")
            _build.build(debug=v == "debug", asan=v == "asan")
        lib = C.CDLL(str(_LIB_PATH), mode=C.RTLD_GLOBAL)
        _bind(lib)
        cap = 256
        buf = (C.c_longlong * cap)()
        n = lib.rph_layout(buf, cap)
        got = list(buf[:n])
        exp = _expected_layout()
        if got != exp:
            raise RuntimeError(f"native/ctypes layout mismatch:\n native={got}\n python={exp}")
        _lib = lib
        return lib
    except Exception as e:
        _load_error = f"{type(e).__name__}: {e}"
        if required:
            raise RuntimeError(f"rphedge native library unavailable on a GPU machine: {_load_error}") from e
        return None


def available() -> bool:
    return load(required=False) is not None


def _check(rc: int, what: str):
    if rc != 0:
        msg = _lib.rph_last_error().decode() if _lib is not None else ""
        raise RuntimeError(f"{what} failed with code {rc}: {msg}")


def ptr(t) -> int | None:
    if t is None:
        return None
    return t.data_ptr()


def fill_ptrs(arr, tensors):
    for i, t in enumerate(tensors):
        arr[i] = ptr(t)


def stream_handle(stream=None) -> int:
    if isinstance(stream, int):
        return stream
    s = stream if stream is not None else torch.cuda.current_stream()
    return s.cuda_stream


def net_nparams(nin: int, h: int, nout: int, head: int) -> tuple[int, int]:
    lib = load(required=True)
    p, r = C.c_int(), C.c_int()
    if lib.rph_net_nparams(nin, h, nout, head, C.byref(p), C.byref(r)) != 0:
        raise ValueError(f"unsupported hedge network shape nin={nin} h={h} nout={nout} head={head}")
    return p.value, r.value


def sobol_normal(out: torch.Tensor, table, offset: int = 0, raw: bool = False, stream=None):
    lib = load(required=True)
    sv, sh, dims = table
    n, d = out.shape
    assert d <= dims
    fp64 = 1 if out.dtype == torch.float64 else 0
    _check(lib.rph_sobol_normal(ptr(out), n, d, ptr(sv), ptr(sh), int(offset), fp64, int(raw),
                                stream_handle(stream)), "rph_sobol_normal")


def simulate(desc: SimDesc, stream=None):
    lib = load(required=True)
    _check(lib.rph_simulate(C.byref(desc), stream_handle(stream)), "rph_simulate")


def train_step(desc: TrainDesc, step: int, epoch: int, stream=None):
    _check(_lib.rph_train_step(C.byref(desc), int(step), int(epoch), stream_handle(stream)), "rph_train_step")


def train_fit(desc: TrainDesc, epochs: int, stream=None):
    _check(_lib.rph_train_fit(C.byref(desc), int(epochs), stream_handle(stream)), "rph_train_fit")


def train_lag_step(desc: TrainDesc, k: int, epoch: int, stream=None):
    _check(_lib.rph_train_lag_step(C.byref(desc), int(k), int(epoch), stream_handle(stream)), "rph_train_lag_step")


def train_lag_fit(desc: TrainDesc, epochs: int, stream=None):
    load(required=True)
    _check(_lib.rph_train_lag_fit(C.byref(desc), int(epochs), stream_handle(stream)), "rph_train_lag_fit")


def train_ticket_fit(desc: TrainDesc, epochs: int, stream=None):
    load(required=True)
    _check(_lib.rph_train_ticket_fit(C.byref(desc), int(epochs), stream_handle(stream)), "rph_train_ticket_fit")


def train_lag_finalize(desc: TrainDesc, K: int, stream=None):
    _check(_lib.rph_train_lag_finalize(C.byref(desc), int(K), stream_handle(stream)), "rph_train_lag_finalize")


def train_update(desc: TrainDesc, step: int, epoch: int, stream=None):
    _check(_lib.rph_train_update(C.byref(desc), int(step), int(epoch), stream_handle(stream)), "rph_train_update")


def eval_(desc: EvalDesc, stream=None):
    _check(_lib.rph_eval(C.byref(desc), stream_handle(stream)), "rph_eval")


def lm_shape(nin: int, h: int, nout: int, head: int):
    lib = load(required=True)
    v = [C.c_int() for _ in range(3)]
    if lib.rph_lm_shape(nin, h, nout, head, *[C.byref(x) for x in v]) != 0:
        return None
    return tuple(int(x.value) for x in v)


def lm_pass_wps(nin: int, h: int, nout: int, head: int) -> int:
    return int(load(required=True).rph_lm_pass_wps(nin, h, nout, head))


def lm_eval(desc: TrainDesc, lm: LmDesc, red_new: torch.Tensor, pass_: int, stream=None):
    _check(_lib.rph_lm_eval(C.byref(desc), C.byref(lm), ptr(red_new), int(pass_), stream_handle(stream)),
           "rph_lm_eval")


def lm_solve(desc: TrainDesc, lm: LmDesc, red_new: torch.Tensor, pass_: int, stream=None):
    _check(_lib.rph_lm_solve(C.byref(desc), C.byref(lm), ptr(red_new), int(pass_), stream_handle(stream)),
           "rph_lm_solve")


def lm_fit(desc: TrainDesc, lm: LmDesc, red_new: torch.Tensor, stream=None):
    load(required=True)
    _check(_lib.rph_lm_fit(C.byref(desc), C.byref(lm), ptr(red_new), stream_handle(stream)), "rph_lm_fit")


def lm_select(desc: TrainDesc, lm: LmDesc, sel: torch.Tensor, main_state: torch.Tensor, world: int, rank: int,
              p: int, phase: int, stream=None):
    _check(_lib.rph_lm_select(C.byref(desc), C.byref(lm), ptr(sel), ptr(main_state), int(world), int(rank), int(p),
                              int(phase), stream_handle(stream)), "rph_lm_select")


def lm_dp_exchange(x: LmDpDesc, red: torch.Tensor, ng: int, p: int, stream=None):
    load(required=True)
    _check(_lib.rph_lm_dp_exchange(C.byref(x), ptr(red), int(ng), int(p), stream_handle(stream)),
           "rph_lm_dp_exchange")


def pnl(desc: PnlDesc, stream=None):
    load(required=True)
    _check(_lib.rph_pnl(C.byref(desc), stream_handle(stream)), "rph_pnl")


def payoff(kind: int, s: torch.Tensor, out: torch.Tensor, strike: float, nfrac=None, wts=None, na: int = 1,
           stream=None, x=None):
    lib = load(required=True)
    n = out.numel()
    _check(lib.rph_payoff(kind, n, na, ptr(s), ptr(nfrac), float(strike), ptr(wts), ptr(x), ptr(out),
                          stream_handle(stream)), "rph_payoff")


def radix_hist(x: torch.Tensor, pmask: int, prefix: int, shift: int, nbins: int, hist: torch.Tensor, stream=None):
    lib = load(required=True)
    _check(lib.rph_radix_hist(ptr(x), x.numel(), pmask & 0xFFFFFFFF, prefix & 0xFFFFFFFF, shift, nbins, ptr(hist),
                              stream_handle(stream)), "rph_radix_hist")


def memset_async(t: torch.Tensor, value: int = 0, stream=None):
    lib = load(required=True)
    _check(lib.rph_memset_async(ptr(t), value, t.numel() * t.element_size(), stream_handle(stream)),
           "rph_memset_async")


def device_info(dev: int = 0) -> dict:
    lib = load(required=True)
    cus, lds = C.c_int(), C.c_int()
    hbm = C.c_longlong()
    name = C.create_string_buffer(128)
    _check(lib.rph_device_info(dev, C.byref(cus), C.byref(lds), C.byref(hbm), name, 128), "rph_device_info")
    return {"cus": cus.value, "lds_per_cu": lds.value, "hbm_bytes": hbm.value, "arch": name.value.decode()}


class Graph:

    def __init__(self):
        self.exec = None
        self.num_nodes = 0

    def capture_begin(self, stream=None):
        lib = load(required=True)
        self._stream = stream_handle(stream)
        _check(lib.rph_graph_begin(self._stream), "rph_graph_begin")

    def capture_end(self):
        ex = VP()
        nn = C.c_longlong()
        _check(_lib.rph_graph_end(self._stream, C.byref(ex), C.byref(nn)), "rph_graph_end")
        self.exec = ex.value
        self.num_nodes = nn.value

    def replay(self, stream=None):
        _check(_lib.rph_graph_launch(self.exec, stream_handle(stream)), "rph_graph_launch")

    def __del__(self):
        if self.exec is not None and _lib is not None:
            try:
                _lib.rph_graph_destroy(self.exec)
            except Exception:
                pass
            self.exec = None


class NcclComm:

    def __init__(self, rank: int, world: int, store, tag: str = "rph_nccl"):
        lib = load(required=True)
        key = f"{tag}_uid"
        if rank == 0:
            buf = C.create_string_buffer(128)
            n = lib.rph_nccl_unique_id(buf)
            if n <= 0:
                _check(-1, "rph_nccl_unique_id")
            store.set(key, bytes(buf.raw[:128]))
        uid = store.get(key)
        comm = VP()
        _check(lib.rph_nccl_init(uid, world, rank, C.byref(comm)), "rph_nccl_init")
        self.comm = comm.value
        self.rank, self.world = rank, world

    def allreduce_(self, t: torch.Tensor, stream=None):
        fn = {torch.float32: _lib.rph_nccl_allreduce_f32, torch.float64: _lib.rph_nccl_allreduce_f64,
              torch.int32: _lib.rph_nccl_allreduce_u32}[t.dtype]
        _check(fn(self.comm, ptr(t), t.numel(), stream_handle(stream)), "rph_nccl_allreduce")

    def close(self):
        if self.comm is not None:
            _lib.rph_nccl_destroy(self.comm)
            self.comm = None


DP_SLOTS = 4


class IpcMailbox:

    def __init__(self, rank: int, world: int, R: int, store, device, tag: str = "rph_mbox"):
        lib = load(required=True)
        if world > 8:
            raise ValueError("fused xGMI all-reduce supports up to 8 ranks (one node)")
        self.rank, self.world, self.R = rank, world, R
        data_bytes = DP_SLOTS * world * R * 8
        self.flag_off = (data_bytes + 255) // 256 * 256
        nbytes = self.flag_off + DP_SLOTS * world * 4 + 256
        hs = lib.rph_ipc_handle_size()
        buf = C.create_string_buffer(hs)
        p = VP()
        _check(lib.rph_ipc_alloc(nbytes, C.byref(p), buf), "rph_ipc_alloc")
        self.own = p.value
        self.finegrained = lib.rph_ipc_is_finegrained() == 1
        store.set(f"{tag}_{rank}", bytes(buf.raw[:hs]))
        self.ptrs, self.opened = [], []
        for q in range(world):
            if q == rank:
                self.ptrs.append(self.own)
                continue
            h = store.get(f"{tag}_{q}")
            pq = VP()
            _check(lib.rph_ipc_open(h, C.byref(pq)), "rph_ipc_open")
            self.ptrs.append(pq.value)
            self.opened.append(pq.value)
        self.counter = torch.zeros(4, dtype=torch.int32, device=device)
        self.error = torch.zeros(4, dtype=torch.int32, device=device)

    def fill(self, d: TrainDesc):
        d.dp_world, d.dp_rank = self.world, self.rank
        for q in range(self.world):
            d.dp_mbox[q] = self.ptrs[q]
            d.dp_flags[q] = self.ptrs[q] + self.flag_off
        d.dp_counter = self.counter.data_ptr()
        d.dp_error = self.error.data_ptr()

    def lm_desc(self) -> "LmDpDesc":
        x = LmDpDesc()
        for q in range(self.world):
            x.mbox[q] = self.ptrs[q]
        x.counter, x.error = self.counter.data_ptr(), self.error.data_ptr()
        x.world, x.rank, x.pitch = self.world, self.rank, self.R
        return x

    def check(self):
        if int(self.error[0].item()) != 0:
            raise RuntimeError("fused xGMI all-reduce: a peer rank did not arrive (timeout)")

    def close(self):
        for p in self.opened:
            _lib.rph_ipc_close(p)
        self.opened = []
        if self.own is not None:
            _lib.rph_free(self.own)
            self.own = None
```

### rphedge/ops/paths.py

```python
from __future__ import annotations

import math
from dataclasses import dataclass, field

import numpy as np
import torch

from . import layout as L
from .sobol import sobol_table, device_table
from .ndtri import ndtri_u30_f64, ndtri_u30_f32
from .philox import philox4x32_10, u01d

SEED_W1 = 1235
SEED_W2 = 1234


@dataclass
class Grid:
    T: float
    dt: float
    rebalancing: float

    @property
    def n_fine(self) -> int:
        return int(math.ceil(self.T / self.dt) + 1)

    @property
    def reduction(self) -> int:
        return max(1, int(math.floor((self.n_fine - 1) / (self.T / self.rebalancing))))

    @property
    def n_coarse(self) -> int:
        return int(math.ceil(self.n_fine / self.reduction))

    @property
    def dt_coarse(self) -> float:
        return self.dt * self.reduction

    def times(self) -> np.ndarray:
        return np.arange(self.n_coarse) * self.dt * self.reduction

    def bond(self, r: float, norm: float = 1.0) -> np.ndarray:
        fine = np.exp(r * np.linspace(0, self.T, self.n_fine))
        return (fine[:: self.reduction] / norm).astype(np.float64)


@dataclass
class Paths:
    kind: str
    grid: Grid
    n_local: int
    path_offset: int
    S: torch.Tensor
    bond: np.ndarray
    S_final: torch.Tensor
    vol: torch.Tensor | None = None
    nfrac: torch.Tensor | None = None
    lam: torch.Tensor | None = None
    nfrac_final: torch.Tensor | None = None
    stat: torch.Tensor | None = None
    stat_final: torch.Tensor | None = None
    stat_kind: str | None = None
    stat_feature: bool = True
    norm: float = 1.0
    na: int = 1
    meta: dict = field(default_factory=dict)

    @property
    def n_coarse(self) -> int:
        return self.S.shape[0]

    def asset(self, t: int, a: int = 0) -> torch.Tensor:
        return self.S[t, a] if self.S.dim() == 3 else self.S[t]

    def prices(self, t: int) -> list:
        return [self.asset(t, a) for a in range(self.na)]

    def features(self, t: int) -> list:
        if self.kind == "pension":
            return [self.S[t], self.nfrac[t], self.lam[t]]
        if self.kind in ("heston", "sv"):
            return [self.S[t], self.vol[t]]
        if self.kind == "gbm_stat" and self.stat_feature:
            return [self.S[t], self.stat[t]]
        return self.prices(t)


def _dev_is_gpu(device) -> bool:
    return torch.device(device).type == "cuda"


def path_indices(n_local: int, offset: int, index_map=None) -> np.ndarray:
    p = np.arange(int(n_local), dtype=np.uint64)
    if index_map is None:
        return p + np.uint64(offset)
    blk, stride = (int(v) for v in index_map)
    return np.uint64(offset) + (p // np.uint64(blk)) * np.uint64(stride) + p % np.uint64(blk)


def _desc(model, n_local, offset, grid: Grid, fp64, parity, index_map=None):
    from . import native

    d = native.SimDesc()
    d.model = model
    d.n_local = int(n_local)
    d.path_offset = int(offset)
    if index_map is not None:
        d.map_blk, d.map_stride = (int(v) for v in index_map)
    d.n_fine = grid.n_fine
    d.reduction = grid.reduction
    d.n_coarse = grid.n_coarse
    d.na = 1
    d.fp64 = 1 if fp64 else 0
    d.parity = 1 if parity else 0
    d.dt = float(grid.dt)
    return d


def simulate_gbm(grid: Grid, n_local: int, s0: float, mu: float, sigma: float, scheme: str = "arith",
                 norm: float = 1.0, device="cuda", offset: int = 0, fp64: bool = False, seed: int = SEED_W1,
                 stream=None, out: Paths | None = None, index_map=None, path_stat: str | None = None) -> Paths:
    if path_stat not in L.PATH_STATS:
        raise ValueError(f"path_stat must be one of mean | geomean | max | min, got {path_stat!r}")
    if path_stat == "geomean" and scheme != "log":
        raise ValueError("path_stat='geomean' needs the log scheme")
    if out is not None and out.stat_kind != path_stat:
        raise ValueError(f"out= holds path_stat {out.stat_kind!r}, asked for {path_stat!r}")
    dev = torch.device(device)
    S = out.S if out is not None else torch.empty(grid.n_coarse, n_local, dtype=torch.float32, device=dev)
    fin = out.S_final if out is not None else torch.empty(n_local, dtype=torch.float32, device=dev)
    A = afin = None
    if path_stat is not None:
        A = out.stat if out is not None else torch.empty(grid.n_coarse, n_local, dtype=torch.float32, device=dev)
        afin = out.stat_final if out is not None else torch.empty(n_local, dtype=torch.float32, device=dev)
    if _dev_is_gpu(dev):
        from . import native

        sv, sh, dims = device_table(grid.n_fine, seed, dev)
        d = _desc(L.SIM_GBM_LOG if scheme == "log" else L.SIM_GBM_ARITH, n_local, offset, grid, fp64, False,
                  index_map)
        d.sv1, d.shift1, d.dims1 = sv.data_ptr(), sh.data_ptr(), dims
        d.s0[0], d.mu[0], d.sigma[0], d.inv_norm[0] = s0, mu, sigma, 1.0 / norm
        d.out, d.final_out = S.data_ptr(), fin.data_ptr()
        if path_stat is not None:
            d.path_stat = L.PATH_STATS[path_stat]
            d.out2, d.final2_out = A.data_ptr(), afin.data_ptr()
        native.simulate(d, stream)
    elif path_stat is None:
        s_np, f_np = _cpu_gbm(grid, n_local, s0, mu, sigma, scheme, offset, seed, index_map)
        S.copy_(torch.from_numpy((s_np / norm).astype(np.float32)))
        fin.copy_(torch.from_numpy((f_np / norm).astype(np.float32)))
    else:
        s_np, f_np, a_np, af_np = _cpu_gbm(grid, n_local, s0, mu, sigma, scheme, offset, seed, index_map,
                                           path_stat=path_stat)
        S.copy_(torch.from_numpy((s_np / norm).astype(np.float32)))
        fin.copy_(torch.from_numpy((f_np / norm).astype(np.float32)))
        A.copy_(torch.from_numpy((a_np / norm).astype(np.float32)))
        afin.copy_(torch.from_numpy((af_np / norm).astype(np.float32)))
    if out is not None:
        return out
    p = Paths(kind="gbm" if path_stat is None else "gbm_stat", grid=grid, n_local=n_local, path_offset=offset, S=S,
              bond=grid.bond(0.0), S_final=fin, norm=norm, stat=A, stat_final=afin, stat_kind=path_stat)
    p.meta["index_map"] = index_map
    return p


def simulate_sv(grid: Grid, n_local: int, s0: float, mu: float, v0: float, model: str = "sv_ref",
                a=0.0, b=0.0, c=0.0, kappa=0.0, theta=0.0, xi=0.0, rho=0.0, norm: float = 1.0,
                device="cuda", offset: int = 0, fp64: bool = False, parity_nan: bool = False,
                seed1: int = SEED_W1, seed2: int = SEED_W2, stream=None, out: Paths | None = None,
                scheme: str = "qe", sv_tscale: float = 0.0, joint: bool | None = None, index_map=None) -> Paths:
    if scheme not in ("qe", "euler"):
        raise ValueError(f"heston scheme must be qe | euler, got {scheme!r}")
    if model == "heston" and scheme == "qe" and not (kappa > 0 and xi > 0):
        scheme = "euler"
    if joint is None:
        joint = model == "heston" or (model == "sv_ref" and sv_tscale > 0)
    dev = torch.device(device)
    S = out.S if out is not None else torch.empty(grid.n_coarse, n_local, dtype=torch.float32, device=dev)
    V = out.vol if out is not None else torch.empty(grid.n_coarse, n_local, dtype=torch.float32, device=dev)
    fin = out.S_final if out is not None else torch.empty(n_local, dtype=torch.float32, device=dev)
    mcode = L.SIM_SV_REF if model == "sv_ref" else L.SIM_HESTON
    if _dev_is_gpu(dev):
        from . import native

        d = _desc(mcode, n_local, offset, grid, fp64, parity_nan, index_map)
        nf = grid.n_fine
        if joint:
            sv, sh, dd = device_table(2 * nf, seed1, dev)
            d.sv1, d.shift1, d.dims1 = sv.data_ptr(), sh.data_ptr(), nf
            d.sv2, d.shift2, d.dims2 = sv.data_ptr() + nf * 32 * 4, sh.data_ptr() + nf * 4, nf
        else:
            sv1, sh1, d1 = device_table(nf, seed1, dev)
            sv2, sh2, d2 = device_table(nf, seed2, dev)
            d.sv1, d.shift1, d.dims1 = sv1.data_ptr(), sh1.data_ptr(), d1
            d.sv2, d.shift2, d.dims2 = sv2.data_ptr(), sh2.data_ptr(), d2
        d.s0[0], d.mu[0], d.inv_norm[0] = s0, mu, 1.0 / norm
        d.v0, d.a, d.b, d.c = v0, a, b, c
        d.kappa, d.theta, d.xi, d.rho = kappa, theta, xi, rho
        d.sv_tscale = float(sv_tscale) if model == "sv_ref" else 0.0
        d.scheme = L.HESTON_QE if scheme == "qe" else L.HESTON_EULER
        d.out, d.out2, d.final_out = S.data_ptr(), V.data_ptr(), fin.data_ptr()
        native.simulate(d, stream)
    else:
        s_np, v_np, f_np = _cpu_sv(grid, n_local, s0, mu, v0, model, a, b, c, kappa, theta, xi, rho, offset,
                                   parity_nan, seed1, seed2, scheme=scheme,
                                   sv_tscale=float(sv_tscale) if model == "sv_ref" else 0.0, joint=joint,
                                   index_map=index_map)
        S.copy_(torch.from_numpy((s_np / norm).astype(np.float32)))
        V.copy_(torch.from_numpy(v_np.astype(np.float32)))
        fin.copy_(torch.from_numpy((f_np / norm).astype(np.float32)))
    if out is not None:
        return out
    p = Paths(kind="heston" if model == "heston" else "sv", grid=grid, n_local=n_local, path_offset=offset,
              S=S, vol=V, bond=grid.bond(0.0), S_final=fin, norm=norm)
    p.meta["index_map"] = index_map
    return p


def simulate_basket(grid: Grid, n_local: int, s0, mu, sigma, corr, norm=None, device="cuda", offset: int = 0,
                    seed: int = SEED_W1, stream=None, out: Paths | None = None, index_map=None) -> Paths:
    na = len(s0)
    norm = np.asarray(norm if norm is not None else s0, dtype=np.float64)
    C = np.asarray(corr, dtype=np.float64)
    chol = np.linalg.cholesky(C)
    dev = torch.device(device)
    S = out.S if out is not None else torch.empty(grid.n_coarse, na, n_local, dtype=torch.float32, device=dev)
    fin = out.S_final if out is not None else torch.empty(na, n_local, dtype=torch.float32, device=dev)
    if _dev_is_gpu(dev):
        from . import native

        sv, sh, dims = device_table(na * grid.n_fine, seed, dev)
        d = _desc(L.SIM_BASKET, n_local, offset, grid, False, False, index_map)
        d.na = na
        d.sv1, d.shift1, d.dims1 = sv.data_ptr(), sh.data_ptr(), dims
        for i in range(na):
            d.s0[i], d.mu[i], d.sigma[i], d.inv_norm[i] = float(s0[i]), float(mu[i]), float(sigma[i]), 1.0 / norm[i]
        for i in range(na):
            for j in range(na):
                d.chol[i * 8 + j] = float(chol[i, j])
        d.out, d.final_out = S.data_ptr(), fin.data_ptr()
        native.simulate(d, stream)
    else:
        s_np, f_np = _cpu_basket(grid, n_local, s0, mu, sigma, chol, offset, seed, index_map)
        S.copy_(torch.from_numpy((s_np / norm[None, :, None]).astype(np.float32)))
        fin.copy_(torch.from_numpy((f_np / norm[:, None]).astype(np.float32)))
    if out is not None:
        return out
    p = Paths(kind="basket", grid=grid, n_local=n_local, path_offset=offset, S=S, bond=grid.bond(0.0),
              S_final=fin, norm=float(norm[0]), na=na)
    p.meta["norms"] = norm
    p.meta["index_map"] = index_map
    return p


def simulate_mortality(paths: Paths, l0: float, c: float, eta: float, n0: int, lambda_fine_index: bool = False,
                       device=None, fp64: bool = False, seed: int = SEED_W2, philox_seed: int = 1234,
                       numpy_binomial: bool = False, stream=None) -> Paths:
    grid, n_local, offset = paths.grid, paths.n_local, paths.path_offset
    dev = paths.S.device if device is None else torch.device(device)
    reuse = paths.nfrac is not None and paths.lam is not None and paths.meta.get("nfrac_final_buf") is not None
    NF = paths.nfrac if reuse else torch.empty(grid.n_coarse, n_local, dtype=torch.float32, device=dev)
    LM = paths.lam if reuse else torch.empty(grid.n_coarse, n_local, dtype=torch.float32, device=dev)
    NT = paths.meta["nfrac_final_buf"] if reuse else torch.empty(n_local, dtype=torch.float32, device=dev)
    if _dev_is_gpu(dev):
        from . import native

        sv, sh, dims = device_table(grid.n_fine, seed, dev)
        d = _desc(L.SIM_MORTALITY, n_local, offset, grid, fp64, lambda_fine_index, paths.meta.get("index_map"))
        d.sv2, d.shift2, d.dims2 = sv.data_ptr(), sh.data_ptr(), dims
        d.l0, d.lc, d.eta, d.n0, d.seed = l0, c, eta, int(n0), int(philox_seed)
        d.out2, d.out3, d.final2_out = NF.data_ptr(), LM.data_ptr(), NT.data_ptr()
        native.simulate(d, stream)
    else:
        nf, lm, nt = _cpu_mortality(grid, n_local, l0, c, eta, n0, lambda_fine_index, offset, seed, philox_seed,
                                    numpy_binomial, paths.meta.get("index_map"))
        NF.copy_(torch.from_numpy(nf.astype(np.float32)))
        LM.copy_(torch.from_numpy(lm.astype(np.float32)))
        NT.copy_(torch.from_numpy(nt.astype(np.float32)))
    paths.kind = "pension"
    paths.nfrac, paths.lam, paths.nfrac_final = NF, LM, NT
    paths.meta["nfrac_final_buf"] = NT
    return paths


PATH_PAYOFFS = {
    "asian_call": ("mean", 1), "asian_put": ("mean", 2),
    "geo_asian_call": ("geomean", 1), "geo_asian_put": ("geomean", 2),
    "lookback_call": ("max", 1),
    "lookback_put": ("min", 2),
    "asian_strike_call": ("mean", 4),
    "asian_strike_put": ("mean", 5),
    "lookback_float_call": ("min", 4),
    "lookback_float_put": ("max", 5),
}


def payoff(kind: str, paths: Paths, strike: float, weights=None, stream=None, out: torch.Tensor | None = None
           ) -> torch.Tensor:
    S = paths.S_final
    n = paths.n_local
    if out is None:
        out = torch.empty(n, dtype=torch.float32, device=S.device)
    x = None
    if kind in PATH_PAYOFFS:
        want, code = PATH_PAYOFFS[kind]
        if paths.stat_kind != want:
            raise ValueError(f"payoff {kind!r} needs paths simulated with path_stat={want!r}, "
                             f"got {paths.stat_kind!r}")
        if code in (1, 2):
            S = paths.stat_final
        else:
            x = paths.stat_final
    else:
        code = {"guarantee": 0, "call": 1, "put": 2, "basket_call": 3}[kind]
    if S.is_cuda:
        from . import native

        w = None
        if code == 3:
            key = ("basket_w", tuple(float(x) for x in weights))
            w = paths.meta.get(key)
            if w is None:
                w = paths.meta[key] = torch.tensor(np.asarray(weights, np.float32), device=S.device)
        native.payoff(code, S, out, strike, nfrac=paths.nfrac_final if code == 0 else None, wts=w, na=paths.na,
                      stream=stream, x=x)
        return out
    if code == 0:
        y = S
        out.copy_(torch.where(y > strike, y, torch.full_like(y, strike)) *
                  (paths.nfrac_final if paths.nfrac_final is not None else 1.0))
    elif code == 1:
        out.copy_((S - strike).clamp_min(0))
    elif code == 2:
        out.copy_((strike - S).clamp_min(0))
    elif code == 4:
        out.copy_((S - x).clamp_min(0))
    elif code == 5:
        out.copy_((x - S).clamp_min(0))
    else:
        w = torch.tensor(np.asarray(weights, np.float32))
        out.copy_(((S * w[:, None]).sum(0) - strike).clamp_min(0))
    return out


def _normals(table_dims, seed, n_local, offset, dims, f32=False, index_map=None):
    tab = sobol_table(table_dims, seed)
    x = tab.points_u30(path_indices(n_local, offset, index_map), dims=dims).astype(np.int64)
    return ndtri_u30_f32(np.maximum(x, 1)).astype(np.float64) if f32 else ndtri_u30_f64(x)


def _cpu_gbm(grid, n, s0, mu, sigma, scheme, offset, seed, index_map=None, path_stat=None):
    W = _normals(grid.n_fine, seed, n, offset, grid.n_fine, index_map=index_map)
    dt = grid.dt
    y = np.full(n, math.log(s0) if scheme == "log" else s0, dtype=np.float64)
    out = np.empty((grid.n_coarse, n))
# ... 174 lines not shown
```

Before: 202.6 million.

## Fuse P&L accumulation into eval kernel and merge paired path simulations

Adds an in-place P&L accumulator to the per-date eval kernel, so each date's hedge gain is folded into a running buffer while holdings are already in registers. A new finish kernel then combines the accumulator with initial wealth and payoff and reduces the terminal P&L statistics. The intent is to avoid a separate full P&L pass that re-reads features and prices and re-runs the network. Separately, the main and Gram-subsample path simulations for LM training are launched as one merged kernel to save a launch and fill the device better. This adds an extra read and write of the accumulator on every date's eval, plus more API surface.

```diff
diff --git a/csrc/hedge_mlp.hip b/csrc/hedge_mlp.hip
--- a/csrc/hedge_mlp.hip
+++ b/csrc/hedge_mlp.hip
@@ -172,6 +172,8 @@
   constexpr int EPF = 4;
   const int stride = (int)gridDim.x * 256;
   const bool has1 = d.price_t1[0] != nullptr;
+  const bool pnl_on = !EX && d.pnl_acc != nullptr;
+  const bool pnl_read = pnl_on && !d.pnl_first;
   auto load_in = [&](int p, In& in) {
     in.p = p;
     in.valid = p < d.n_local;
@@ -199,6 +201,7 @@
     if (p0 + EPF * stride < d.n_local) load_in(cur.p + EPF * stride, q[EPF - 1]);
     const int p = cur.p;
     const bool valid = cur.valid;
+    const float racc = pnl_read ? d.pnl_acc[valid ? p : 0] : 0.f;
     uint32_t zo = 0;
     asm volatile("" : "+v"(zo));
     const float* __restrict__ WAi = (const float*)__builtin_assume_aligned(WA + (zo & ~3u), 16);
@@ -241,6 +244,14 @@
         if (d.hold_out[k]) d.hold_out[k][p] = hold[k];
       if (d.resid_out) d.resid_out[p] = res;
       if (d.pred1_out) d.pred1_out[p] = pred1;
+      if constexpr (!EX) {
+        if (pnl_on) {
+          float gain = 0.f;
+#pragma unroll
+          for (int k = 0; k < NHOLD - 1; ++k) gain = fmaf(hold[k], cur.pt1[k] - cur.pt[k] * d.pnl_grow, gain);
+          d.pnl_acc[p] = fmaf(d.pnl_carry, gain, racc);
+        }
+      }
       st[ES_V] += V;
       st[ES_V2] += V * V;
       st[ES_RES] += res;
@@ -476,6 +487,60 @@
       else if (tid == ES_EXVAL) v = sum4(9);
       else if (tid == ES_TAU) v = sum4(10);
     }
+    d.stats[(size_t)blockIdx.x * EVAL_NSTAT + tid] = v;
+  }
+}
+
+__global__ __launch_bounds__(256) void k_pnl_finish(const PnlFinishDesc d) {
+  RPH_DASSERT(d.n_local > 0 && d.num_wgs == (int)gridDim.x && d.acc != nullptr && d.stats != nullptr);
+  __shared__ double sred[4][8];
+  const int tid = threadIdx.x, lane = tid & 63, wid = tid >> 6;
+  const long long base = (long long)blockIdx.x * 256 * PNL_PPT + tid;
+  double sv = 0, sv2 = 0, sp = 0, sp2 = 0, sa = 0, cnt = 0;
+  float pmin = INFINITY, pmax = -INFINITY;
+#pragma unroll
+  for (int j = 0; j < PNL_PPT; ++j) {
+    const long long p = base + (long long)j * 256;
+    if (p >= d.n_local) continue;
+    const float w = fmaf(d.w0[p], d.carry, d.acc[p]);
+    const float pnl = w - d.payoff[p];
+    if (d.pnl_out) d.pnl_out[p] = pnl;
+    sv += w;
+    sv2 += (double)w * w;
+    sp += pnl;
+    sp2 += (double)pnl * pnl;
+    sa += fabsf(pnl);
+    cnt += 1.0;
+    pmin = fminf(pmin, pnl);
+    pmax = fmaxf(pmax, pnl);
+  }
+#pragma unroll
+  for (int o = 1; o < 64; o <<= 1) {
+    sv += __shfl_xor(sv, o, 64);
+    sv2 += __shfl_xor(sv2, o, 64);
+    sp += __shfl_xor(sp, o, 64);
+    sp2 += __shfl_xor(sp2, o, 64);
+    sa += __shfl_xor(sa, o, 64);
+    cnt += __shfl_xor(cnt, o, 64);
+    pmin = fminf(pmin, __shfl_xor(pmin, o, 64));
+    pmax = fmaxf(pmax, __shfl_xor(pmax, o, 64));
+  }
+  if (lane == 0) {
+    sred[wid][0] = sv; sred[wid][1] = sv2; sred[wid][2] = sp; sred[wid][3] = sp2;
+    sred[wid][4] = sa; sred[wid][5] = cnt; sred[wid][6] = pmin; sred[wid][7] = pmax;
+  }
+  __syncthreads();
+  if (tid < EVAL_NSTAT) {
+    double v = 0.0;
+    auto sum4 = [&](int k) { return (sred[0][k] + sred[1][k]) + (sred[2][k] + sred[3][k]); };
+    if (tid == ES_V) v = sum4(0);
+    else if (tid == ES_V2) v = sum4(1);
+    else if (tid == ES_RES) v = sum4(2);
+    else if (tid == ES_RES2) v = sum4(3);
+    else if (tid == ES_ABSRES) v = sum4(4);
+    else if (tid == ES_COUNT) v = sum4(5);
+    else if (tid == ES_RESMIN) v = fmin(fmin(sred[0][6], sred[1][6]), fmin(sred[2][6], sred[3][6]));
+    else if (tid == ES_RESMAX) v = fmax(fmax(sred[0][7], sred[1][7]), fmax(sred[2][7], sred[3][7]));
     d.stats[(size_t)blockIdx.x * EVAL_NSTAT + tid] = v;
   }
 }
@@ -608,6 +673,13 @@
     if (nhold < 2 || !d->price_t[0]) return rph_report("rph_eval", "price_t[0] is null with ex_kind");
     if (!(d->ex_strike == d->ex_strike) || d->ex_strike < 0.f || d->ex_strike > 3.0e38f)
       return rph_report("rph_eval", "ex_strike must be finite and >= 0");
+  }
+  if (d->pnl_acc) {
+    if (ex) return rph_report("rph_eval", "pnl_acc with ex_kind (the early-exercise P&L is the forward scan)");
+    for (int k = 0; k < nhold - 1; ++k)
+      if (!d->price_t[k] || !d->price_t1[k]) return rph_report("rph_eval", "pnl_acc needs price_t and price_t1");
+    if (!(fabsf(d->pnl_grow) <= 3.0e38f) || !(fabsf(d->pnl_carry) <= 3.0e38f))
+      return rph_report("rph_eval", "pnl_grow / pnl_carry must be finite");
   }
   return with_shape(AllShapes{}, d->nin, d->h, d->nout, d->head, "rph_eval", [&](auto t) {
     using T = decltype(t);
@@ -654,3 +726,17 @@
     return (int)hipGetLastError();
   });
 }
+
+extern "C" int rph_pnl_finish(const PnlFinishDesc* d, void* stream) {
+  if (!d->acc || !d->w0 || !d->payoff || !d->stats || d->n_local < 1)
+    return rph_report("rph_pnl_finish", "bad P&L finish descriptor");
+  if (!(fabsf(d->carry) <= 3.0e38f)) return rph_report("rph_pnl_finish", "carry must be finite");
+  const long long per_wg = 256LL * PNL_PPT;
+  if ((long long)d->num_wgs * per_wg < d->n_local || (long long)(d->num_wgs - 1) * per_wg >= d->n_local)
+    return rph_report("rph_pnl_finish", "num_wgs does not match n_local / (256 * PNL_PPT)");
+  hipStream_t s = (hipStream_t)stream;
+  return with_shape(AllShapes{}, d->nin, d->h, d->nout, d->head, "rph_pnl_finish", [&](auto) {
+    hipLaunchKernelGGL(k_pnl_finish, dim3(d->num_wgs), dim3(256), 0, s, *d);
+    return (int)hipGetLastError();
+  });
+}
diff --git a/csrc/paths.hip b/csrc/paths.hip
--- a/csrc/paths.hip
+++ b/csrc/paths.hip
@@ -41,9 +41,9 @@
                        : d.path_offset + p;
 }
 
-template <typename Real, bool ALIGNED, int MODEL, int STAT = 0>
-__global__ __launch_bounds__(256) void k_sim_scan(const SimDesc d) {
-  const int p = blockIdx.x * 256 + threadIdx.x;
+template <typename Real, bool ALIGNED, int MODEL, int STAT>
+RPH_INLINE void sim_scan_block(const SimDesc& d, const int blk) {
+  const int p = blk * 256 + threadIdx.x;
   if (!ALIGNED && p >= d.n_local) return;
   const long long gp = sim_gidx(d, p);
   const uint32_t g = gray_code((uint64_t)gp);
@@ -216,6 +216,17 @@
   }
 }
 
+template <typename Real, bool ALIGNED, int MODEL, int STAT = 0>
+__global__ __launch_bounds__(256) void k_sim_scan(const SimDesc d) {
+  sim_scan_block<Real, ALIGNED, MODEL, STAT>(d, (int)blockIdx.x);
+}
+
+template <typename Real, bool ALIGNED, int MODEL, int STAT = 0>
+__global__ __launch_bounds__(256) void k_sim_scan_pair(const SimDesc a, const SimDesc b, const int split) {
+  if ((int)blockIdx.x < split) sim_scan_block<Real, ALIGNED, MODEL, STAT>(a, (int)blockIdx.x);
+  else sim_scan_block<Real, ALIGNED, MODEL, STAT>(b, (int)blockIdx.x - split);
+}
+
 template <int NA, bool ALIGNED>
 __global__ __launch_bounds__(256) void k_sim_basket(const SimDesc d) {
   const int p = blockIdx.x * 256 + threadIdx.x;
@@ -330,31 +341,42 @@
   return (int)hipGetLastError();
 }
 
+template <typename Real, bool AL, int MODEL, int STAT = 0>
+static void launch_scan_kernel(const SimDesc* d, const SimDesc* d2, hipStream_t s) {
+  const int split = grid_for(d->n_local);
+  if constexpr (MODEL != SIM_MORTALITY) {
+    if (d2) {
+      hipLaunchKernelGGL((k_sim_scan_pair<Real, AL, MODEL, STAT>), dim3(split + grid_for(d2->n_local)), dim3(256), 0, s,
+                         *d, *d2, split);
+      return;
+    }
+  }
+  hipLaunchKernelGGL((k_sim_scan<Real, AL, MODEL, STAT>), dim3(split), dim3(256), 0, s, *d);
+}
+
 template <typename Real, bool AL, int MODEL>
-static int launch_scan_stat(const SimDesc* d, hipStream_t s) {
-  const dim3 grid(grid_for(d->n_local)), block(256);
+static int launch_scan_stat(const SimDesc* d, const SimDesc* d2, hipStream_t s) {
   switch (d->path_stat) {
-    case STAT_MEAN: hipLaunchKernelGGL((k_sim_scan<Real, AL, MODEL, STAT_MEAN>), grid, block, 0, s, *d); break;
-    case STAT_GEOMEAN: hipLaunchKernelGGL((k_sim_scan<Real, AL, SIM_GBM_LOG, STAT_GEOMEAN>), grid, block, 0, s, *d); break;
-    case STAT_MAX: hipLaunchKernelGGL((k_sim_scan<Real, AL, MODEL, STAT_MAX>), grid, block, 0, s, *d); break;
-    case STAT_MIN: hipLaunchKernelGGL((k_sim_scan<Real, AL, MODEL, STAT_MIN>), grid, block, 0, s, *d); break;
+    case STAT_MEAN: launch_scan_kernel<Real, AL, MODEL, STAT_MEAN>(d, d2, s); break;
+    case STAT_GEOMEAN: launch_scan_kernel<Real, AL, SIM_GBM_LOG, STAT_GEOMEAN>(d, d2, s); break;
+    case STAT_MAX: launch_scan_kernel<Real, AL, MODEL, STAT_MAX>(d, d2, s); break;
+    case STAT_MIN: launch_scan_kernel<Real, AL, MODEL, STAT_MIN>(d, d2, s); break;
     default: return -1;
   }
   return (int)hipGetLastError();
 }
 
 template <typename Real, bool AL>
-static int launch_scan(const SimDesc* d, hipStream_t s) {
-  const dim3 grid(grid_for(d->n_local)), block(256);
+static int launch_scan(const SimDesc* d, hipStream_t s, const SimDesc* d2 = nullptr) {
   if (d->path_stat != STAT_NONE)
-    return d->model == SIM_GBM_LOG ? launch_scan_stat<Real, AL, SIM_GBM_LOG>(d, s)
-                                   : launch_scan_stat<Real, AL, SIM_GBM_ARITH>(d, s);
+    return d->model == SIM_GBM_LOG ? launch_scan_stat<Real, AL, SIM_GBM_LOG>(d, d2, s)
+                                   : launch_scan_stat<Real, AL, SIM_GBM_ARITH>(d, d2, s);
   switch (d->model) {
-    case SIM_GBM_ARITH: hipLaunchKernelGGL((k_sim_scan<Real, AL, SIM_GBM_ARITH>), grid, block, 0, s, *d); break;
-    case SIM_GBM_LOG: hipLaunchKernelGGL((k_sim_scan<Real, AL, SIM_GBM_LOG>), grid, block, 0, s, *d); break;
-    case SIM_SV_REF: hipLaunchKernelGGL((k_sim_scan<Real, AL, SIM_SV_REF>), grid, block, 0, s, *d); break;
-    case SIM_HESTON: hipLaunchKernelGGL((k_sim_scan<Real, AL, SIM_HESTON>), grid, block, 0, s, *d); break;
-    case SIM_MORTALITY: hipLaunchKernelGGL((k_sim_scan<Real, AL, SIM_MORTALITY>), grid, block, 0, s, *d); break;
+    case SIM_GBM_ARITH: launch_scan_kernel<Real, AL, SIM_GBM_ARITH>(d, d2, s); break;
+    case SIM_GBM_LOG: launch_scan_kernel<Real, AL, SIM_GBM_LOG>(d, d2, s); break;
+    case SIM_SV_REF: launch_scan_kernel<Real, AL, SIM_SV_REF>(d, d2, s); break;
+    case SIM_HESTON: launch_scan_kernel<Real, AL, SIM_HESTON>(d, d2, s); break;
+    case SIM_MORTALITY: launch_scan_kernel<Real, AL, SIM_MORTALITY>(d, nullptr, s); break;
     default: return -1;
   }
   return (int)hipGetLastError();
@@ -375,22 +397,48 @@
   return (int)hipGetLastError();
 }
 
+static int validate_sim(const SimDesc* d, const char* who) {
+  if (d->map_blk < 0 || (d->map_blk > 0 && d->map_stride < d->map_blk)) return rph_report(who, "bad path-index map");
+  if (d->path_stat < STAT_NONE || d->path_stat > STAT_MIN) return rph_report(who, "path_stat outside 0..4");
+  if (d->path_stat != STAT_NONE) {
+    if (d->model != SIM_GBM_ARITH && d->model != SIM_GBM_LOG) return rph_report(who, "path statistics need a GBM model");
+    if (!d->out2) return rph_report(who, "path statistic without an out2 buffer");
+    if (d->path_stat == STAT_GEOMEAN && d->model != SIM_GBM_LOG)
+      return rph_report(who, "geomean needs the log scheme (SIM_GBM_LOG)");
+  }
+  return 0;
+}
+
+static bool sim_aligned(const SimDesc* d) {
+  return (d->n_local % 256 == 0) && (d->path_offset % 64 == 0) &&
+         (d->map_blk == 0 || (d->map_blk % 64 == 0 && d->map_stride % 64 == 0));
+}
+
 extern "C" int rph_simulate(const SimDesc* d, void* stream) {
   hipStream_t s = (hipStream_t)stream;
-  if (d->map_blk < 0 || (d->map_blk > 0 && d->map_stride < d->map_blk)) return rph_report("rph_simulate", "bad path-index map");
-  if (d->path_stat < STAT_NONE || d->path_stat > STAT_MIN) return rph_report("rph_simulate", "path_stat outside 0..4");
-  if (d->path_stat != STAT_NONE) {
-    if (d->model != SIM_GBM_ARITH && d->model != SIM_GBM_LOG)
-      return rph_report("rph_simulate", "path statistics need a GBM model");
-    if (!d->out2) return rph_report("rph_simulate", "path statistic without an out2 buffer");
-    if (d->path_stat == STAT_GEOMEAN && d->model != SIM_GBM_LOG)
-      return rph_report("rph_simulate", "geomean needs the log scheme (SIM_GBM_LOG)");
-  }
-  const bool aligned = (d->n_local % 256 == 0) && (d->path_offset % 64 == 0) &&
-                       (d->map_blk == 0 || (d->map_blk % 64 == 0 && d->map_stride % 64 == 0));
+  if (int rc = validate_sim(d, "rph_simulate")) return rc;
+  const bool aligned = sim_aligned(d);
   if (d->model == SIM_BASKET) return aligned ? launch_basket<true>(d, s) : launch_basket<false>(d, s);
   if (d->fp64) return aligned ? launch_scan<double, true>(d, s) : launch_scan<double, false>(d, s);
   return aligned ? launch_scan<float, true>(d, s) : launch_scan<float, false>(d, s);
+}
+
+extern "C" int rph_simulate_pair(const SimDesc* a, const SimDesc* b, int* merged, void* stream) {
+  hipStream_t s = (hipStream_t)stream;
+  if (merged) *merged = 0;
+  if (int rc = validate_sim(a, "rph_simulate_pair")) return rc;
+  if (int rc = validate_sim(b, "rph_simulate_pair")) return rc;
+  const bool aligned = sim_aligned(a);
+  const bool same = a->model == b->model && (a->fp64 != 0) == (b->fp64 != 0) && a->path_stat == b->path_stat &&
+                    aligned == sim_aligned(b) && a->model != SIM_BASKET && a->model != SIM_MORTALITY &&
+                    (long long)grid_for(a->n_local) + grid_for(b->n_local) <= 0x7fffffffLL;
+  if (!same) {
+    if (int rc = rph_simulate(a, stream)) return rc;
+    return rph_simulate(b, stream);
+  }
+  if (merged) *merged = 1;
+  if (a->fp64) return aligned ? launch_scan<double, true>(a, s, b) : launch_scan<double, false>(a, s, b);
+  return aligned ? launch_scan<float, true>(a, s, b) : launch_scan<float, false>(a, s, b);
 }
 
 extern "C" int rph_payoff(int kind, int n, int na, const float* s, const float* nfrac, float strike,
diff --git a/csrc/rph_types.h b/csrc/rph_types.h
--- a/csrc/rph_types.h
+++ b/csrc/rph_types.h
@@ -119,6 +119,23 @@
   NetWeights* snap_b;
   int ex_kind;
   float ex_strike;
+  float* pnl_acc;
+  float pnl_grow;
+  float pnl_carry;
+  int pnl_first;
+  int pad_pnl;
+};
+
+struct PnlFinishDesc {
+  const float* acc;
+  const float* w0;
+  const float* payoff;
+  float* pnl_out;
+  double* stats;
+  float carry;
+  int n_local, num_wgs;
+  int nin, h, nout, head;
+  int pad0;
 };
 
 struct PnlDesc {
diff --git a/csrc/runtime.cpp b/csrc/runtime.cpp
--- a/csrc/runtime.cpp
+++ b/csrc/runtime.cpp
@@ -56,6 +56,10 @@
       OFF(EvalDesc, resid_out), OFF(EvalDesc, pred1_out), OFF(EvalDesc, stats), OFF(EvalDesc, bond_t),
       OFF(EvalDesc, hold_c), OFF(EvalDesc, n_local), OFF(EvalDesc, head), OFF(EvalDesc, fmu), OFF(EvalDesc, fisd),
       OFF(EvalDesc, snap_a), OFF(EvalDesc, snap_b), OFF(EvalDesc, ex_kind), OFF(EvalDesc, ex_strike),
+      OFF(EvalDesc, pnl_acc), OFF(EvalDesc, pnl_grow), OFF(EvalDesc, pnl_carry), OFF(EvalDesc, pnl_first),
+      (long long)sizeof(PnlFinishDesc), OFF(PnlFinishDesc, w0), OFF(PnlFinishDesc, payoff), OFF(PnlFinishDesc, pnl_out),
+      OFF(PnlFinishDesc, stats), OFF(PnlFinishDesc, carry), OFF(PnlFinishDesc, n_local), OFF(PnlFinishDesc, num_wgs),
+      OFF(PnlFinishDesc, nin), OFF(PnlFinishDesc, head),
       (long long)sizeof(PnlDesc), OFF(PnlDesc, feat_ts), OFF(PnlDesc, price), OFF(PnlDesc, price_ts),
       OFF(PnlDesc, snap), OFF(PnlDesc, bond), OFF(PnlDesc, pnl_out), OFF(PnlDesc, stats), OFF(PnlDesc, alpha),
       OFF(PnlDesc, has_b), OFF(PnlDesc, n_dates), OFF(PnlDesc, head),
diff --git a/rphedge/api.py b/rphedge/api.py
--- a/rphedge/api.py
+++ b/rphedge/api.py
@@ -160,13 +160,20 @@
     def simulate(self, into: P.Paths | None = None):
         c = self.cfg
         vt_out = self.v_terminal if into is not None else None
+        tr = c.train
+        lm = str(tr.optimizer).lower() == "lm"
+        pair = [] if (lm and self.kind == "european" and self.device.type == "cuda") else None
         with self.timer.phase("simulate"):
-            p = self._simulate_paths(self.n_local, self.offset, None, into)
+            p = self._simulate_paths(self.n_local, self.offset, None, into, defer=pair)
+            if lm:
+                ns, blk, stride = gram_subsample(self.n_total, tr.lm_gram_paths)
+                self.gpaths = self._simulate_paths(ns, 0, (blk, stride), self.gpaths if into is not None else None,
+                                                   defer=pair)
+            if pair is not None:
+                from .ops import native
+                native.simulate_pair(pair[0], pair[1], self.stream)
             v_t = self._payoff(p, vt_out)
-            tr = c.train
-            if str(tr.optimizer).lower() == "lm":
-                ns, blk, stride = gram_subsample(self.n_total, tr.lm_gram_paths)
-                self.gpaths = self._simulate_paths(ns, 0, (blk, stride), self.gpaths if into is not None else None)
+            if lm:
                 if self._q_lm():
                     self.gv_terminal = self._payoff(self.gpaths, self.gv_terminal if into is not None else None)
                 if self.di.world > 1 and (int(tr.lm_starts) > 1 or bool(getattr(tr, "lm_explore_one", False))):
@@ -192,10 +199,14 @@
             return P.payoff("basket_call", p, c.K / c.Y, weights=w, stream=self.stream, out=out)
         return P.payoff("guarantee", p, c.K, stream=self.stream, out=out)
 
-    def _simulate_paths(self, n: int, offset: int, index_map, into: P.Paths | None) -> P.Paths:
+    def _simulate_paths(self, n: int, offset: int, index_map, into: P.Paths | None, defer: list | None = None
+                        ) -> P.Paths:
         c, g, dev = self.cfg, self.grid, self.device
         fp64 = c.dtype == "fp64"
         kw = dict(device=dev, offset=offset, stream=self.stream, out=into, index_map=index_map)
+        if defer is not None:
+            assert self.kind == "european"
+            kw["defer"] = defer
         if self.kind == "european":
             if c.model == "heston":
                 p = P.simulate_sv(g, n, c.Y, c.r, c.v0, model="heston", kappa=c.kappa, theta=c.theta, xi=c.xi,
diff --git a/rphedge/driver.py b/rphedge/driver.py
--- a/rphedge/driver.py
+++ b/rphedge/driver.py
@@ -7,7 +7,7 @@
 import torch
 
 from .engine import (MAXIN, DateData, Exercise, FitConfig, PnlData, TrainConfig, fit_seed, fit_summary,
-                     geometric_lr_schedule, keras_lr_schedule, reduce_stats)
+                     geometric_lr_schedule, keras_lr_schedule, pnl_fold_factors, reduce_stats)
 from .models.hedge_mlp import NetSpec
 from .ops import layout as L
 from .ops.paths import Paths
@@ -216,6 +216,10 @@
         self.pnl_stats = backend.new_pnl_stats()
         self.pnl_paths = torch.empty(n, dtype=torch.float32, device=dev) if keep else None
         self.pnl_done = False
+        self.pnl_fold = hasattr(backend, "pnl_finish") and icfg.exercise is None and nd >= 1
+        if self.pnl_fold:
+            self.pnl_grow, self.pnl_carry, self.pnl_carry_all = pnl_fold_factors(paths.bond)
+            self.pnl_acc = torch.full((n,), float("nan"), dtype=torch.float32, device=dev)
         ex = icfg.exercise
         if ex is not None and icfg.q99:
             raise ValueError("early exercise takes one network per date: q99=True (wts_b / g_base) is not available")
@@ -309,8 +313,12 @@
         nc = self.paths.n_coarse
         start = nc - 2 if start is None else int(start)
         self.ran = list(range(start, -1, -1))
+        self.pnl_done = start == nc - 2
+        fold = self.pnl_fold and self.pnl_done
         for t in self.ran:
             first = t == nc - 2
+            pnl_kw = dict(pnl_acc=self.pnl_acc, pnl_grow=float(self.pnl_grow[t]), pnl_carry=float(self.pnl_carry[t]),
+                          pnl_first=first) if fold else {}
             data = self.date_data(t)
             if not c.carry_optimizer and c.warm_start and not first:
                 self.opt_mse.copy_(self.opt_init)
@@ -356,14 +364,16 @@
                            seed=fit_seed(c.seed, t, 1), poll_every=c.poll_every)
                 be.eval(self.w_mse, data, s_q, wts_b=self.w_q, g_base=self.gbuf, blend_c=c.cost_of_capital,
                         hold_c=self.hold_c, v_out=self.values[t], hold_out=hold_out, resid_out=resid_out,
-                        snap_a=self.snap[t, 0], snap_b=self.snap[t, 1])
+                        snap_a=self.snap[t, 0], snap_b=self.snap[t, 1], **pnl_kw)
                 if self.gvalues is not None:
                     self.eval_gram_values(t)
             else:
                 be.eval(self.w_mse, data, s_q, v_out=self.values[t], hold_out=hold_out, resid_out=resid_out,
-                        snap_a=self.snap[t, 0], exercise=self.exercise_at(t))
-        self.pnl_done = start == nc - 2
-        if self.pnl_done:
+                        snap_a=self.snap[t, 0], exercise=self.exercise_at(t), **pnl_kw)
+        if fold:
+            be.pnl_finish(self.pnl_acc, self.values[0], self.values[nc - 1], float(self.pnl_carry_all),
+                          self.pnl_stats, pnl_out=self.pnl_paths)
+        elif self.pnl_done:
             be.pnl(self.snap, self.pnl_data, self.pnl_stats, has_b=c.q99, hold_c=self.hold_c,
                    pnl_out=self.pnl_paths, exercise=c.exercise, tau_out=self.tau)
 
diff --git a/rphedge/engine/__init__.py b/rphedge/engine/__init__.py
--- a/rphedge/engine/__init__.py
+++ b/rphedge/engine/__init__.py
@@ -1,7 +1,7 @@
 from ..models.hedge_mlp import NetSpec
 from ..ops.native import MAXIN
 from .config import (DateData, Exercise, FitConfig, PnlData, TrainConfig, fit_seed, geometric_lr_schedule,
-                     keras_lr_schedule)
+                     keras_lr_schedule, pnl_fold_factors)
 from .lm_geometry import (GRAM_BLOCKS, _lm_bias_index, _lm_out_n, gram_subsample, lm_gram_geometry,
                           lm_og_wgs, lm_out_gram, lm_out_nu, lm_pass_schedule, lm_pass_wgs, lm_tpack_image, lm_tpack_len)
 from .state import (_normalise, current_weights, fit_summary, fit_template, make_opt, make_weights,
diff --git a/rphedge/engine/config.py b/rphedge/engine/config.py
--- a/rphedge/engine/config.py
+++ b/rphedge/engine/config.py
@@ -2,6 +2,7 @@
 
 from dataclasses import dataclass, field
 
+import numpy as np
 import torch
 
 from ..ops import layout as L
@@ -113,6 +114,13 @@
     payoff: torch.Tensor
 
 
+def pnl_fold_factors(bond) -> tuple:
+    b = np.asarray(bond, np.float64)
+    g = (b[1:] / b[:-1]).astype(np.float32)
+    tail = np.concatenate([np.cumprod(g[::-1].astype(np.float64))[::-1], [1.0]])
+    return g, tail[1:].astype(np.float32), np.float32(tail[0])
+
+
 @dataclass(frozen=True)
 class Exercise:
 
diff --git a/rphedge/engine/hip.py b/rphedge/engine/hip.py
--- a/rphedge/engine/hip.py
+++ b/rphedge/engine/hip.py
@@ -510,9 +510,26 @@
         assert stats.shape[0] == d.num_wgs and snap.shape[0] >= data.n_dates
         n.pnl(d, self.stream)
 
+    def pnl_finish(self, acc, w0, payoff, carry: float, stats, pnl_out=None):
+        n = self.native
+        d = n.PnlFinishDesc()
+        for t in (acc, w0, payoff):
+            assert t.dtype == torch.float32 and t.numel() == self.n_local
+        d.acc, d.w0, d.payoff = acc.data_ptr(), w0.data_ptr(), payoff.data_ptr()
+        if pnl_out is not None:
+            assert pnl_out.dtype == torch.float32 and pnl_out.numel() == self.n_local
+        d.pnl_out = n.ptr(pnl_out)
+        d.stats = stats.data_ptr()
+        d.carry = float(carry)
+        d.n_local, d.num_wgs = self.n_local, self.pnl_wgs()
+        d.nin, d.h, d.nout, d.head = self.shape
+        assert stats.shape[0] == d.num_wgs
+        n.pnl_finish(d, self.stream)
+
     def eval(self, wts, data: DateData, stats, wts_b=None, g_base=None, blend_c=0.0, hold_c=0.0,
              v_out=None, hold_out=None, resid_out=None, pred1_out=None, snap_a=None, snap_b=None,
-             n_local: int | None = None, exercise: Exercise | None = None):
+             n_local: int | None = None, exercise: Exercise | None = None, pnl_acc=None, pnl_grow: float = 1.0,
+             pnl_carry: float = 1.0, pnl_first: bool = False):
         _check_eval_data(self.spec, data)
         n = self.native
         d = n.EvalDesc()
@@ -537,4 +554,9 @@
         _set_norm(d, data)
         if exercise is not None:
             d.ex_kind, d.ex_strike = L.EX_KINDS[exercise.kind], float(exercise.strike)
+        if pnl_acc is not None:
+            if pnl_acc.dtype != torch.float32 or pnl_acc.numel() != d.n_local:
+                raise ValueError(f"eval: pnl_acc must be float32 [{d.n_local}]")
+            d.pnl_acc = pnl_acc.data_ptr()
+            d.pnl_grow, d.pnl_carry, d.pnl_first = float(pnl_grow), float(pnl_carry), 1 if pnl_first else 0
         n.eval_(d, self.stream)
diff --git a/rphedge/ops/native.py b/rphedge/ops/native.py
--- a/rphedge/ops/native.py
+++ b/rphedge/ops/native.py
@@ -49,12 +49,22 @@
         ("n_local", C.c_int), ("num_wgs", C.c_int), ("nin", C.c_int), ("h", C.c_int), ("nout", C.c_int),
         ("head", C.c_int), ("fmu", C.c_float * MAXIN), ("fisd", C.c_float * MAXIN),
         ("snap_a", VP), ("snap_b", VP), ("ex_kind", C.c_int), ("ex_strike", C.c_float),
+        ("pnl_acc", VP), ("pnl_grow", C.c_float), ("pnl_carry", C.c_float), ("pnl_first", C.c_int),
+        ("pad_pnl", C.c_int),
     ]
 
     def __init__(self, *a, **kw):
         super().__init__(*a, **kw)
         for f in range(MAXIN):
             self.fisd[f] = 1.0
+
+
+class PnlFinishDesc(C.Structure):
+    _fields_ = [
+        ("acc", VP), ("w0", VP), ("payoff", VP), ("pnl_out", VP), ("stats", VP),
+        ("carry", C.c_float), ("n_local", C.c_int), ("num_wgs", C.c_int),
+        ("nin", C.c_int), ("h", C.c_int), ("nout", C.c_int), ("head", C.c_int), ("pad0", C.c_int),
+    ]
 
 
 class PnlDesc(C.Structure):
@@ -132,6 +142,10 @@
         E.v_out.offset, E.hold_out.offset, E.resid_out.offset, E.pred1_out.offset, E.stats.offset,
         E.bond_t.offset, E.hold_c.offset, E.n_local.offset, E.head.offset, E.fmu.offset, E.fisd.offset,
         E.snap_a.offset, E.snap_b.offset, E.ex_kind.offset, E.ex_strike.offset,
+        E.pnl_acc.offset, E.pnl_grow.offset, E.pnl_carry.offset, E.pnl_first.offset,
+        C.sizeof(PnlFinishDesc), PnlFinishDesc.w0.offset, PnlFinishDesc.payoff.offset, PnlFinishDesc.pnl_out.offset,
+        PnlFinishDesc.stats.offset, PnlFinishDesc.carry.offset, PnlFinishDesc.n_local.offset,
+        PnlFinishDesc.num_wgs.offset, PnlFinishDesc.nin.offset, PnlFinishDesc.head.offset,
         C.sizeof(PnlDesc), PnlDesc.feat_ts.offset, PnlDesc.price.offset, PnlDesc.price_ts.offset,
         PnlDesc.snap.offset, PnlDesc.bond.offset, PnlDesc.pnl_out.offset, PnlDesc.stats.offset,
         PnlDesc.alpha.offset, PnlDesc.has_b.offset, PnlDesc.n_dates.offset, PnlDesc.head.offset,
@@ -183,6 +197,7 @@
         "rph_train_ticket_fit": (C.c_int, [C.POINTER(TrainDesc), C.c_int, VP]),
         "rph_eval": (C.c_int, [C.POINTER(EvalDesc), VP]),
         "rph_pnl": (C.c_int, [C.POINTER(PnlDesc), VP]),
+        "rph_pnl_finish": (C.c_int, [C.POINTER(PnlFinishDesc), VP]),
         "rph_lm_shape": (C.c_int, [C.c_int] * 4 + [C.POINTER(C.c_int)] * 3),
         "rph_lm_pass_wps": (C.c_int, [C.c_int] * 4),
         "rph_lm_eval": (C.c_int, [C.POINTER(TrainDesc), C.POINTER(LmDesc), VP, C.c_int, VP]),
@@ -193,6 +208,7 @@
                                     C.c_int, VP]),
         "rph_sobol_normal": (C.c_int, [VP, C.c_int, C.c_int, VP, VP, C.c_longlong, C.c_int, C.c_int, VP]),
         "rph_simulate": (C.c_int, [C.POINTER(SimDesc), VP]),
+        "rph_simulate_pair": (C.c_int, [C.POINTER(SimDesc), C.POINTER(SimDesc), C.POINTER(C.c_int), VP]),
         "rph_payoff": (C.c_int, [C.c_int, C.c_int, C.c_int, VP, VP, C.c_float, VP, VP, VP, VP]),
         "rph_radix_hist": (C.c_int, [VP, C.c_longlong, C.c_uint32, C.c_uint32, C.c_int, C.c_int, VP, VP]),
         "rph_ipc_alloc": (C.c_int, [C.c_longlong, C.POINTER(VP), C.c_char_p]),
@@ -291,6 +307,13 @@
     _check(lib.rph_simulate(C.byref(desc), stream_handle(stream)), "rph_simulate")
 
 
+def simulate_pair(a: SimDesc, b: SimDesc, stream=None) -> bool:
+    lib = load(required=True)
+    merged = C.c_int(0)
+    _check(lib.rph_simulate_pair(C.byref(a), C.byref(b), C.byref(merged), stream_handle(stream)), "rph_simulate_pair")
+    return bool(merged.value)
+
+
 def train_step(desc: TrainDesc, step: int, epoch: int, stream=None):
     _check(_lib.rph_train_step(C.byref(desc), int(step), int(epoch), stream_handle(stream)), "rph_train_step")
 
@@ -367,6 +390,11 @@
 def pnl(desc: PnlDesc, stream=None):
     load(required=True)
     _check(_lib.rph_pnl(C.byref(desc), stream_handle(stream)), "rph_pnl")
+
+
+def pnl_finish(desc: PnlFinishDesc, stream=None):
+    load(required=True)
+    _check(_lib.rph_pnl_finish(C.byref(desc), stream_handle(stream)), "rph_pnl_finish")
 
 
 def payoff(kind: int, s: torch.Tensor, out: torch.Tensor, strike: float, nfrac=None, wts=None, na: int = 1,
diff --git a/rphedge/ops/paths.py b/rphedge/ops/paths.py
--- a/rphedge/ops/paths.py
+++ b/rphedge/ops/paths.py
@@ -119,7 +119,8 @@
 
 def simulate_gbm(grid: Grid, n_local: int, s0: float, mu: float, sigma: float, scheme: str = "arith",
                  norm: float = 1.0, device="cuda", offset: int = 0, fp64: bool = False, seed: int = SEED_W1,
-                 stream=None, out: Paths | None = None, index_map=None, path_stat: str | None = None) -> Paths:
+                 stream=None, out: Paths | None = None, index_map=None, path_stat: str | None = None,
+                 defer: list | None = None) -> Paths:
     if path_stat not in L.PATH_STATS:
         raise ValueError(f"path_stat must be one of mean | geomean | max | min, got {path_stat!r}")
     if path_stat == "geomean" and scheme != "log":
@@ -145,7 +146,10 @@
         if path_stat is not None:
             d.path_stat = L.PATH_STATS[path_stat]
             d.out2, d.final2_out = A.data_ptr(), afin.data_ptr()
-        native.simulate(d, stream)
+        if defer is not None:
+            defer.append(d)
+        else:
+            native.simulate(d, stream)
     elif path_stat is None:
         s_np, f_np = _cpu_gbm(grid, n_local, s0, mu, sigma, scheme, offset, seed, index_map)
         S.copy_(torch.from_numpy((s_np / norm).astype(np.float32)))
@@ -169,7 +173,8 @@
                 a=0.0, b=0.0, c=0.0, kappa=0.0, theta=0.0, xi=0.0, rho=0.0, norm: float = 1.0,
                 device="cuda", offset: int = 0, fp64: bool = False, parity_nan: bool = False,
                 seed1: int = SEED_W1, seed2: int = SEED_W2, stream=None, out: Paths | None = None,
-                scheme: str = "qe", sv_tscale: float = 0.0, joint: bool | None = None, index_map=None) -> Paths:
+                scheme: str = "qe", sv_tscale: float = 0.0, joint: bool | None = None, index_map=None,
+                defer: list | None = None) -> Paths:
     if scheme not in ("qe", "euler"):
         raise ValueError(f"heston scheme must be qe | euler, got {scheme!r}")
     if model == "heston" and scheme == "qe" and not (kappa > 0 and xi > 0):
@@ -201,7 +206,10 @@
         d.sv_tscale = float(sv_tscale) if model == "sv_ref" else 0.0
         d.scheme = L.HESTON_QE if scheme == "qe" else L.HESTON_EULER
         d.out, d.out2, d.final_out = S.data_ptr(), V.data_ptr(), fin.data_ptr()
-        native.simulate(d, stream)
+        if defer is not None:
+            defer.append(d)
+        else:
+            native.simulate(d, stream)
     else:
         s_np, v_np, f_np = _cpu_sv(grid, n_local, s0, mu, v0, model, a, b, c, kappa, theta, xi, rho, offset,
                                    parity_nan, seed1, seed2, scheme=scheme,
```

Result: faster. 207.5 million (median of 6 runs) (+2.4%).
